# magenta/mt3

Measured on AMD Instinct MI355X. Metric: audio-seconds transcribed/sec (whole node), MT3-base, 1/2/4/8 MI355X, higher is better.
Workload: dtype f32; 1 GPU; BASELINE configs[2]: MT3 (model.gin) random-init, full encoder-decoder greedy decode, batch=256 synthetic 2.048 s segments per GPU, 1024 decode steps (no early exit), ids->tokens + host note decoding included; segments_per_gpu=256, segments_total=256, decode_steps=1024, decode_chains=1, decoding=greedy, parallelism=single GPU, graph_fallbacks=0, partition_fallbacks=0

## Files before the change

include/mt3_hip.h:

```cpp
#ifndef MT3_HIP_H_
#define MT3_HIP_H_

#include <stdint.h>

#ifdef __cplusplus
extern "C" {
#endif

typedef enum mt3_status {
  MT3_OK = 0,
  MT3_ERR_INVALID = -1,
  MT3_ERR_HIP = -2,
  MT3_ERR_CAPACITY = -3,
  MT3_ERR_MISSING = -4
} mt3_status;

const char* mt3_last_error(void);
int mt3_abi_version(void);

typedef struct mt3_frontend_config {
  int32_t sample_rate;
  int32_t hop_width;
  int32_t num_mel_bins;
  int32_t fft_size;
  float lo_hz;
  float hi_hz;
  int32_t table_dtype;
} mt3_frontend_config;

typedef struct mt3_frontend mt3_frontend;

int mt3_frontend_create(const mt3_frontend_config* cfg, mt3_frontend** out);
void mt3_frontend_destroy(mt3_frontend* fe);
int mt3_frontend_mel_matrix(const mt3_frontend* fe, float* h_out , int64_t* nnz);
int mt3_frontend_logmel(mt3_frontend* fe, const float* d_audio, int32_t n_segments,
                        int32_t frames_per_segment, const int32_t* h_n_frames ,
                        float* d_logmel, void* stream);
int mt3_frontend_logmel_dev(mt3_frontend* fe, const float* d_audio, int32_t n_segments,
                            int32_t frames_per_segment, const int32_t* d_n_frames ,
                            float* d_logmel, void* stream);

typedef struct mt3_resampler mt3_resampler;

int64_t mt3_resample_output_length(int64_t n_in, int32_t up, int32_t down);
int mt3_resampler_create(const double* h_taps , int64_t n_taps, int32_t up, int32_t down,
                         mt3_resampler** out);
void mt3_resampler_destroy(mt3_resampler* r);
int mt3_resampler_run(mt3_resampler* r, const float* d_in, int64_t n_in, float* d_out, int64_t out_capacity,
                      void* stream);

enum { MT3_PCM_U8 = 0, MT3_PCM_S16 = 1, MT3_PCM_S24 = 2, MT3_PCM_S32 = 3, MT3_PCM_F32 = 4, MT3_PCM_F64 = 5 };
#define MT3_PCM_MAX_CHANNELS 7

int mt3_pcm_decode(const void* d_pcm, int64_t n_frames, int32_t channels, int32_t format, float* d_out,
                   int64_t out_capacity, void* stream);
int mt3_resampler_run_pcm(mt3_resampler* r, const void* d_pcm, int64_t n_frames, int32_t channels, int32_t format,
                          float* d_out, int64_t out_capacity, void* stream);

typedef enum mt3_dtype { MT3_BF16 = 0, MT3_F32 = 1, MT3_FP8_E4M3 = 2  } mt3_dtype;

typedef struct mt3_engine_config {
  int32_t vocab_size;
  int32_t emb_dim;
  int32_t num_heads;
  int32_t head_dim;
  int32_t mlp_dim;
  int32_t num_encoder_layers;
  int32_t num_decoder_layers;
  int32_t input_depth;
  int32_t input_length;
  int32_t max_decode_len;
  int32_t max_batch;
  int32_t compute_dtype;
  int32_t decode_chains;
  int32_t kv_cache_dtype;
  int32_t dense_dtype;
  int32_t options;
} mt3_engine_config;

enum {
  MT3_OPT_SINGLE_RESIDUAL_STREAM = 1,
  MT3_OPT_ENCODER_SINGLE_RESIDUAL_STREAM = 4,
  MT3_OPT_SEPARATE_PROJECTIONS = 2,
  MT3_OPT_SEPARATE_QKV_PROJECTION = 8,
  MT3_OPT_NO_ROW_GROUPS = 16,
  MT3_OPT_ENCODER_F32_MFMA = 32,
  MT3_OPT_SPIN_WAITS = 64
};

typedef struct mt3_engine mt3_engine;

int mt3_engine_create(const mt3_engine_config* cfg, mt3_engine** out);
void mt3_engine_destroy(mt3_engine* e);
int mt3_engine_load_weight(mt3_engine* e, const char* name, const float* h_data,
                           const int64_t* shape, int32_t ndim);
int mt3_engine_finalize(mt3_engine* e);
int64_t mt3_engine_device_bytes(const mt3_engine* e);

int mt3_engine_encode(mt3_engine* e, const float* d_inputs, int32_t batch,
                      float* d_encoded_f32, void* stream);

enum {
  MT3_DECODE_NO_GRAPH = 1,
  MT3_DECODE_EARLY_EXIT = 2,
  MT3_DECODE_BEAM1 = 4,
  MT3_DECODE_SINGLE_STREAM = 8,
  MT3_DECODE_ASYNC = 16
};
#define MT3_DECODE_CHAINS(n) (((n) & 0xF) << 8)
int mt3_engine_decode(mt3_engine* e, int32_t batch, int32_t num_steps, int32_t flags,
                      int32_t* d_ids, float* d_first_logits, int32_t* h_steps_run, void* stream);
int mt3_engine_decode_wait(mt3_engine* e, int32_t* h_steps_run);

int mt3_engine_decode_beams(mt3_engine* e, int32_t batch, int32_t num_beams, int32_t num_steps, int32_t flags,
                            int32_t* d_ids, int32_t* d_all_ids, float* d_scores, int32_t* h_steps_run, void* stream);

typedef struct mt3_transcribe_stats {
  int32_t slots;
  int32_t groups;
  int32_t steps_run;
  int32_t polls;
  int32_t refills;
  int32_t starved_polls;
  int32_t encoder_chunks;
  int32_t compactions;
  int32_t used_graph;
  int32_t reserved[7];
} mt3_transcribe_stats;
int mt3_engine_transcribe(mt3_engine* e, const float* d_inputs, int32_t n_segments, int32_t num_steps, int32_t flags,
                          int32_t* d_ids, mt3_transcribe_stats* h_stats, void* stream);

int mt3_engine_decode_forced(mt3_engine* e, int32_t batch, int32_t num_steps, int32_t flags,
                             const int32_t* d_forced_ids, float* d_step_logits, int32_t* d_ids, void* stream);

int mt3_engine_score(mt3_engine* e, int32_t batch, int32_t length, const int32_t* d_targets,
                     const int32_t* d_decoder_inputs , const float* d_weights ,
                     float* d_sequence_scores, float* d_token_scores, float* d_logits, void* stream);

enum { MT3_STATUS_GRAPH_FALLBACKS = 0, MT3_STATUS_LAST_DECODE_USED_GRAPH = 1, MT3_STATUS_RESIDUAL_SPLIT = 2,
       MT3_STATUS_KV_FP8 = 3, MT3_STATUS_Q_FOLD = 4 ,
       MT3_STATUS_DENSE_FP8 = 5 ,
       MT3_STATUS_QKV_FOLD = 6 ,
       MT3_STATUS_LAST_DECODE_GROUPS = 7 ,
       MT3_STATUS_PARTITION_FALLBACKS = 8 ,
       MT3_STATUS_LAST_DECODE_COMPACTIONS = 9 ,
       MT3_STATUS_LAST_DECODE_FORKS = 10 ,
       MT3_STATUS_SCORE_CHUNKS = 11  };
int mt3_engine_status(const mt3_engine* e, int32_t what);

int mt3_ids_to_tokens(const int32_t* d_ids, int32_t batch, int32_t length, int32_t num_regular,
                      int32_t* d_tokens, void* stream);

enum { MT3_EPI_STORE = 0, MT3_EPI_RESID = 1, MT3_EPI_GEGLU = 2, MT3_EPI_POS = 3, MT3_EPI_F32 = 4, MT3_EPI_HEADS = 5 };
int mt3_op_gemm(int32_t dtype, const void* d_A, int32_t a_is_f32, int32_t norm, const void* d_Wt,
                void* d_out, int32_t M, int32_t N, int32_t K, int32_t epilogue, const float* d_aux,
                int32_t seq_len, int32_t small, void* stream);
int mt3_op_gemm_ex(int32_t dtype, const void* d_A, int32_t a_is_f32, int32_t norm, const void* d_Wt,
                   void* d_out, int32_t M, int32_t N, int32_t K, int32_t epilogue, const float* d_aux,
                   int32_t seq_len, int32_t small, const float* d_a_ss, void* d_out_ct, float* d_out_ss,
                   void* stream);
int mt3_op_residual_split(int32_t dtype, const float* d_x, void* d_x_ct, float* d_x_ss, int32_t rows, int32_t dim,
                          void* stream);
int mt3_op_encoder_attention(int32_t dtype, const void* d_qkv, void* d_out, int32_t B, int32_t T, int32_t H,
                             void* stream);
int mt3_op_decode_attention(int32_t dtype, const void* d_q, int32_t q_stride, void* d_kcache, void* d_vcache,
                            int32_t cap, const void* d_new_k, const void* d_new_v, int32_t kv_stride,
                            const int32_t* d_step, int32_t n_keys, void* d_out, int32_t B, int32_t H, void* stream);
int mt3_op_decode_attention_fp8(const void* d_q, int32_t q_stride, void* d_kcache, void* d_vcache, void* d_kv_scale,
                                int32_t cap, const void* d_new_k, const void* d_new_v, int32_t kv_stride,
                                const int32_t* d_step, int32_t n_keys, void* d_out, int32_t B, int32_t H,
                                void* stream);
int mt3_op_kv_quantize_fp8(const void* d_src, void* d_dst, void* d_scales, int32_t rows, void* stream);

int mt3_host_mx8_quantize(const float* h_w, int64_t rows, int64_t K, uint8_t* h_q, uint8_t* h_sc);
int mt3_op_mx8_quantize(const void* d_in, int32_t in_is_f32, int32_t M, int32_t K, uint8_t* d_q, uint8_t* d_sc,
                        float* d_ss, void* stream);
int mt3_op_gemm_mx8(const uint8_t* d_A, const uint8_t* d_a_sc, const uint8_t* d_W, const uint8_t* d_w_sc, void* d_out,
                    int32_t M, int32_t N, int32_t K, int32_t epilogue, int32_t seq_len, const float* d_a_ss,
                    uint8_t* d_out_q, uint8_t* d_out_sc, float* d_out_ss, void* stream);

enum { MT3_EV_SHIFT = 0, MT3_EV_PITCH = 1, MT3_EV_VELOCITY = 2, MT3_EV_TIE = 3, MT3_EV_PROGRAM = 4, MT3_EV_DRUM = 5 };
enum { MT3_SPEC_ONSETS = 0, MT3_SPEC_NOTES = 1, MT3_SPEC_TIES = 2 };

typedef struct mt3_event_range { int32_t type, min_value, max_value; } mt3_event_range;
typedef struct mt3_codec {
  double steps_per_second;
  int32_t num_ranges;
  mt3_event_range ranges[8];
} mt3_codec;
typedef struct mt3_note {
  double start_time, end_time;
  int32_t pitch, velocity, program, is_drum, instrument, reserved;
} mt3_note;

int mt3_build_codec(int32_t steps_per_second, int32_t max_shift_seconds, int32_t num_velocity_bins,
                    mt3_codec* out);
int mt3_codec_num_classes(const mt3_codec* c);
int mt3_codec_decode_event(const mt3_codec* c, int32_t index, int32_t* type, int32_t* value);
int mt3_codec_encode_event(const mt3_codec* c, int32_t type, int32_t value, int32_t* index);
int mt3_notes_decode(const mt3_codec* c, int32_t spec, int32_t n_segments, const int32_t* h_tokens,
                     const int64_t* h_seg_offsets, const double* h_start_times,
                     const int32_t* h_has_max_time, const double* h_max_times,
                     mt3_note* h_notes, int64_t notes_capacity, int64_t* n_notes,
                     int64_t* invalid_events, int64_t* dropped_events, double* total_time);

#ifdef __cplusplus
}
#endif
#endif
```

mt3_amd/_lib.py:

```python
from __future__ import annotations

import ctypes as C
import os

HERE = os.path.dirname(os.path.abspath(__file__))
LIB_PATH = os.path.join(HERE, "libmt3hip.so")

MT3_OK, MT3_ERR_INVALID, MT3_ERR_HIP, MT3_ERR_CAPACITY, MT3_ERR_MISSING = 0, -1, -2, -3, -4
MT3_BF16, MT3_F32, MT3_FP8_E4M3 = 0, 1, 2
EPI_STORE, EPI_RESID, EPI_GEGLU, EPI_POS, EPI_F32, EPI_HEADS = range(6)
DECODE_NO_GRAPH, DECODE_EARLY_EXIT, DECODE_BEAM1, DECODE_SINGLE_STREAM, DECODE_ASYNC = 1, 2, 4, 8, 16
(OPT_SINGLE_RESIDUAL_STREAM, OPT_SEPARATE_PROJECTIONS, OPT_ENCODER_SINGLE_RESIDUAL_STREAM,
 OPT_SEPARATE_QKV_PROJECTION, OPT_NO_ROW_GROUPS) = 1, 2, 4, 8, 16
OPT_ENCODER_F32_MFMA = 32
OPT_SPIN_WAITS = 64
DEBUG_SKIP_SELF_ATTN, DEBUG_SKIP_CROSS_ATTN = 1, 2
(STATUS_GRAPH_FALLBACKS, STATUS_LAST_DECODE_USED_GRAPH, STATUS_RESIDUAL_SPLIT, STATUS_KV_FP8, STATUS_Q_FOLD,
 STATUS_DENSE_FP8, STATUS_QKV_FOLD, STATUS_LAST_DECODE_GROUPS, STATUS_PARTITION_FALLBACKS,
 STATUS_LAST_DECODE_COMPACTIONS, STATUS_LAST_DECODE_FORKS, STATUS_SCORE_CHUNKS) = range(12)
(MT3_PCM_U8, MT3_PCM_S16, MT3_PCM_S24, MT3_PCM_S32, MT3_PCM_F32, MT3_PCM_F64) = range(6)
PCM_MAX_CHANNELS = 7
MAX_BEAMS = 8
EV_SHIFT, EV_PITCH, EV_VELOCITY, EV_TIE, EV_PROGRAM, EV_DRUM = range(6)
EVENT_TYPE_NAMES = ("shift", "pitch", "velocity", "tie", "program", "drum")
SPEC_ONSETS, SPEC_NOTES, SPEC_TIES = range(3)


class Mt3Error(RuntimeError):
    def __init__(self, code, msg):
        super().__init__("libmt3hip error %d: %s" % (code, msg))
        self.code = code


class FrontendConfig(C.Structure):
    _fields_ = [("sample_rate", C.c_int32), ("hop_width", C.c_int32), ("num_mel_bins", C.c_int32),
                ("fft_size", C.c_int32), ("lo_hz", C.c_float), ("hi_hz", C.c_float), ("table_dtype", C.c_int32)]


class EngineConfig(C.Structure):
    _fields_ = [(n, C.c_int32) for n in (
        "vocab_size", "emb_dim", "num_heads", "head_dim", "mlp_dim", "num_encoder_layers",
        "num_decoder_layers", "input_depth", "input_length", "max_decode_len", "max_batch", "compute_dtype",
        "decode_chains", "kv_cache_dtype", "dense_dtype", "options")]


class TranscribeStats(C.Structure):
    _fields_ = [(n, C.c_int32) for n in ("slots", "groups", "steps_run", "polls", "refills", "starved_polls",
                                         "encoder_chunks", "compactions", "used_graph")] + [("reserved", C.c_int32 * 7)]


class EventRange(C.Structure):
    _fields_ = [("type", C.c_int32), ("min_value", C.c_int32), ("max_value", C.c_int32)]


class CodecDesc(C.Structure):
    _fields_ = [("steps_per_second", C.c_double), ("num_ranges", C.c_int32), ("ranges", EventRange * 8)]


class NoteStruct(C.Structure):
    _fields_ = [("start_time", C.c_double), ("end_time", C.c_double), ("pitch", C.c_int32),
                ("velocity", C.c_int32), ("program", C.c_int32), ("is_drum", C.c_int32),
                ("instrument", C.c_int32), ("reserved", C.c_int32)]


_P = C.c_void_p
SIGNATURES = {
    "mt3_last_error": (C.c_char_p, []),
    "mt3_abi_version": (C.c_int, []),
    "mt3_frontend_create": (C.c_int, [C.POINTER(FrontendConfig), C.POINTER(_P)]),
    "mt3_frontend_destroy": (None, [_P]),
    "mt3_frontend_mel_matrix": (C.c_int, [_P, _P, C.POINTER(C.c_int64)]),
    "mt3_frontend_logmel": (C.c_int, [_P, _P, C.c_int32, C.c_int32, _P, _P, _P]),
    "mt3_frontend_logmel_dev": (C.c_int, [_P, _P, C.c_int32, C.c_int32, _P, _P, _P]),
    "mt3_resample_output_length": (C.c_int64, [C.c_int64, C.c_int32, C.c_int32]),
    "mt3_resampler_create": (C.c_int, [_P, C.c_int64, C.c_int32, C.c_int32, C.POINTER(_P)]),
    "mt3_resampler_destroy": (None, [_P]),
    "mt3_resampler_run": (C.c_int, [_P, _P, C.c_int64, _P, C.c_int64, _P]),
    "mt3_pcm_decode": (C.c_int, [_P, C.c_int64, C.c_int32, C.c_int32, _P, C.c_int64, _P]),
    "mt3_resampler_run_pcm": (C.c_int, [_P, _P, C.c_int64, C.c_int32, C.c_int32, _P, C.c_int64, _P]),
    "mt3_engine_create": (C.c_int, [C.POINTER(EngineConfig), C.POINTER(_P)]),
    "mt3_engine_destroy": (None, [_P]),
    "mt3_engine_load_weight": (C.c_int, [_P, C.c_char_p, _P, C.POINTER(C.c_int64), C.c_int32]),
    "mt3_engine_finalize": (C.c_int, [_P]),
    "mt3_engine_device_bytes": (C.c_int64, [_P]),
    "mt3_engine_encode": (C.c_int, [_P, _P, C.c_int32, _P, _P]),
    "mt3_engine_decode": (C.c_int, [_P, C.c_int32, C.c_int32, C.c_int32, _P, _P, C.POINTER(C.c_int32), _P]),
    "mt3_engine_decode_wait": (C.c_int, [_P, C.POINTER(C.c_int32)]),
    "mt3_engine_decode_beams": (C.c_int, [_P, C.c_int32, C.c_int32, C.c_int32, C.c_int32, _P, _P, _P,
                                          C.POINTER(C.c_int32), _P]),
    "mt3_engine_transcribe": (C.c_int, [_P, _P, C.c_int32, C.c_int32, C.c_int32, _P, C.POINTER(TranscribeStats), _P]),
    "mt3_engine_decode_forced": (C.c_int, [_P, C.c_int32, C.c_int32, C.c_int32, _P, _P, _P, _P]),
    "mt3_engine_score": (C.c_int, [_P, C.c_int32, C.c_int32, _P, _P, _P, _P, _P, _P, _P]),
    "mt3_engine_status": (C.c_int, [_P, C.c_int32]),
    "mt3_debug_engine_decode": (C.c_int, [_P, C.c_int32, C.c_int32, C.c_int32, C.c_int32, _P, _P]),
    "mt3_debug_engine_transcribe": (C.c_int, [_P, _P, C.c_int32, C.c_int32, C.c_int32, C.c_int32, C.c_int32, C.c_int32, _P,
                                              C.POINTER(TranscribeStats), _P]),
    "mt3_debug_engine_set_score_chunk": (C.c_int, [_P, C.c_int32]),
    "mt3_debug_engine_poison_caches": (C.c_int, [_P, C.c_int32, C.c_int32, _P]),
    "mt3_debug_engine_set_eos_schedule": (C.c_int, [_P, _P, C.c_int32]),
    "mt3_ids_to_tokens": (C.c_int, [_P, C.c_int32, C.c_int32, C.c_int32, _P, _P]),
    "mt3_op_gemm": (C.c_int, [C.c_int32, _P, C.c_int32, C.c_int32, _P, _P, C.c_int32, C.c_int32, C.c_int32,
                              C.c_int32, _P, C.c_int32, C.c_int32, _P]),
    "mt3_op_gemm_ex": (C.c_int, [C.c_int32, _P, C.c_int32, C.c_int32, _P, _P, C.c_int32, C.c_int32, C.c_int32,
                                 C.c_int32, _P, C.c_int32, C.c_int32, _P, _P, _P, _P]),
    "mt3_op_residual_split": (C.c_int, [C.c_int32, _P, _P, _P, C.c_int32, C.c_int32, _P]),
    "mt3_op_encoder_attention": (C.c_int, [C.c_int32, _P, _P, C.c_int32, C.c_int32, C.c_int32, _P]),
    "mt3_op_decode_attention": (C.c_int, [C.c_int32, _P, C.c_int32, _P, _P, C.c_int32, _P, _P, C.c_int32, _P,
                                          C.c_int32, _P, C.c_int32, C.c_int32, _P]),
    "mt3_op_decode_attention_fp8": (C.c_int, [_P, C.c_int32, _P, _P, _P, C.c_int32, _P, _P, C.c_int32, _P, C.c_int32,
                                              _P, C.c_int32, C.c_int32, _P]),
    "mt3_op_kv_quantize_fp8": (C.c_int, [_P, _P, _P, C.c_int32, _P]),
    "mt3_host_mx8_quantize": (C.c_int, [_P, C.c_int64, C.c_int64, _P, _P]),
    "mt3_op_mx8_quantize": (C.c_int, [_P, C.c_int32, C.c_int32, C.c_int32, _P, _P, _P, _P]),
    "mt3_op_gemm_mx8": (C.c_int, [_P, _P, _P, _P, _P, C.c_int32, C.c_int32, C.c_int32, C.c_int32, C.c_int32, _P, _P, _P,
                                  _P, _P]),
    "mt3_build_codec": (C.c_int, [C.c_int32, C.c_int32, C.c_int32, C.POINTER(CodecDesc)]),
    "mt3_codec_num_classes": (C.c_int, [C.POINTER(CodecDesc)]),
    "mt3_codec_decode_event": (C.c_int, [C.POINTER(CodecDesc), C.c_int32, C.POINTER(C.c_int32), C.POINTER(C.c_int32)]),
    "mt3_codec_encode_event": (C.c_int, [C.POINTER(CodecDesc), C.c_int32, C.c_int32, C.POINTER(C.c_int32)]),
    "mt3_notes_decode": (C.c_int, [C.POINTER(CodecDesc), C.c_int32, C.c_int32, _P, _P, _P, _P, _P, _P, C.c_int64,
                                   C.POINTER(C.c_int64), C.POINTER(C.c_int64), C.POINTER(C.c_int64),
                                   C.POINTER(C.c_double)]),
}

_lib = None


def load():
    global _lib
    if _lib is not None:
        return _lib
    if not os.path.exists(LIB_PATH):
        raise Mt3Error(MT3_ERR_MISSING,
                       "%s not found: build it with `python -m mt3_amd.build` "
                       "(hipcc --offload-arch=gfx950); there is no CPU fallback" % LIB_PATH)
    try:
        import torch
    except Exception:
        pass
    lib = C.CDLL(LIB_PATH)
    for name, (res, args) in SIGNATURES.items():
        fn = getattr(lib, name)
        fn.restype = res
        fn.argtypes = args
    _lib = lib
    return lib


def check(rc: int):
    if rc != MT3_OK:
        raise Mt3Error(rc, (load().mt3_last_error() or b"").decode("utf-8", "replace"))
    return rc
```

mt3_amd/csrc/engine.hip:

```cpp
#include <hip/hip_runtime.h>

#include <atomic>
#include <chrono>
#include <cmath>
#include <condition_variable>
#include <cstdlib>
#include <cstring>
#include <functional>
#include <map>
#include <mutex>
#include <new>
#include <string>
#include <thread>
#include <vector>

#include "common.h"
#include "feed.h"
#include "kernels.h"

namespace mt3k {
int launch_encoder_attention_x6(const void* qkv, void* out, int B, int T, int H, hipStream_t s);
}
#include "mx8.h"
#include "mt3_hip.h"
#include "mt3_hip_debug.h"

namespace {

constexpr int kMaxPos = 2048;
constexpr int kMaxChains = 8;
constexpr int kForksPinned = 15;

uint16_t f32_to_bf16_bits(float f) {
  uint32_t u;
  std::memcpy(&u, &f, 4);
  if ((u & 0x7fffffffu) > 0x7f800000u) return static_cast<uint16_t>((u >> 16) | 0x40);
  u += 0x7fffu + ((u >> 16) & 1u);
  return static_cast<uint16_t>(u >> 16);
}

struct HostWeight {
  std::vector<float> data;
  std::vector<int64_t> shape;
};

struct LayerDev {
  void* wqkv = nullptr;
  void* wo = nullptr;
  void* wq_x = nullptr;
  void* wkv_x = nullptr;
  void* wo_x = nullptr;
  void* wqkv_ext = nullptr;
  void* wo_ext = nullptr;
  void* w_fold = nullptr;
  void* wi = nullptr;
  void* wo_mlp = nullptr;
  void* self_k = nullptr;
  void* self_v = nullptr;
  void* cross_kv = nullptr;
  uint8_t *wqkv_q = nullptr, *wqkv_sc = nullptr, *wo_q = nullptr, *wo_sc = nullptr, *wi_q = nullptr, *wi_sc = nullptr,
          *wo_mlp_q = nullptr, *wo_mlp_sc = nullptr, *wkv_x_q = nullptr, *wkv_x_sc = nullptr;
  void *wqkv_p[3] = {}, *wo_p[3] = {}, *wi_p[3] = {}, *wo_mlp_p[3] = {}, *wkv_x_p[3] = {};
  void *wq_x_p[3] = {}, *wo_x_p[3] = {};
  float2* self_scale = nullptr;
  float2* cross_scale = nullptr;
};

constexpr int kVarBeam = 4, kVarForced = 8, kVarRetire = 16, kVarEos = 32, kVarStream = 64, kNumVariants = 128;
constexpr int kVarBeside = 128;
constexpr int kVarBeams = 256, kVarBeamsShift = 9;
constexpr int kMaxGroups = 4;
constexpr int kStageChunks = mt3feed::kStageChunks, kStageChunkCap = 64, kStageMinBatch = 8;
constexpr int kStreamPollSteps = 4;
constexpr int kThrottleWindow = 16;

struct Worker {
  std::thread th;
  std::mutex mu;
  std::condition_variable cv;
  std::function<void()> job;
  bool has_job = false, quit = false;
};

struct GroupGraph {
  int variant, batch, row0, rows, slot, max_len;
  hipGraph_t graph;
  hipGraphExec_t exec;
};

struct PendingDecode {
  bool active = false;
  int posted = 0;
  int groups = 1;
  bool beam1 = false;
  bool used_graph[kMaxGroups] = {};
  int batch = 0;
  int32_t* d_ids = nullptr;
  hipStream_t s = nullptr;
  int beams = 0;
  int num_steps = 0;
  int32_t* d_all_ids = nullptr;
  float* d_scores = nullptr;
  int rcs[kMaxGroups] = {};
  int ran[kMaxGroups] = {};
  std::string errs[kMaxGroups];
};

}

struct mt3_engine {
  mt3_engine_config cfg{};
  std::map<std::string, HostWeight> raw;
  std::vector<void*> allocs;
  int64_t device_bytes = 0;
  bool finalized = false;
  int esize = 2;
  int kv_esize = 2;
  bool kv_fp8 = false;
  void* cross_stage = nullptr;
  bool dense_fp8 = false;
  uint8_t *x_q = nullptr, *x_sc = nullptr;
  uint8_t *attn_q = nullptr, *attn_sc = nullptr;
  uint8_t *h_q = nullptr, *h_sc = nullptr;
  uint8_t *enc_q = nullptr, *enc_sc = nullptr;

  void* enc_in = nullptr;
  void* enc_in_p[3] = {};
  bool x6 = false;
  float* enc_norm = nullptr;
  float* embedding = nullptr;
  void* logits_w = nullptr;
  float* pos_table = nullptr;
  std::vector<LayerDev> enc, dec;

  float* x = nullptr;
  void* x_ct = nullptr;
  float* x_ss = nullptr;
  bool x_split = false;
  void* qkv = nullptr;
  void* attn = nullptr;
  void* hbuf = nullptr;
  void* enc_out = nullptr;
  float* y = nullptr;
  void* y_ct = nullptr;
  float* y_ss = nullptr;
  bool y_split = false;
  float* qf = nullptr;
  bool q_fold = false;
  bool qkv_fold = false;
  float* qkvf = nullptr;
  float* ew0 = nullptr;
  float* pw0 = nullptr;
  void* y_ct_alt = nullptr;
  float* y_alt = nullptr;
  void* qkv_d = nullptr;
  void* attn_d = nullptr;
  void* q_d = nullptr;
  void* h_d = nullptr;
  float* logits = nullptr;
  int* ids = nullptr;
  int* cur_tok = nullptr;
  int* done = nullptr;
  int* step = nullptr;
  int* n_done = nullptr;
  int* h_pinned = nullptr;
  int* forced = nullptr;
  std::atomic<int> graph_fallbacks{0};
  int last_used_graph = 0;
  int* slot_row = nullptr;
  int* eos_at = nullptr;
  int eos_cap = 0;
  bool eos_on = false;
  int* slot_seg = nullptr;
  int* cs_seg = nullptr;
  int* refill_plan = nullptr;
  int stream_max_len = 0;
  int stage_cap = 0;
  std::vector<void*> stage_kv;
  std::vector<float2*> stage_scale;
  float* cs_y = nullptr;
  void* cs_y_ct = nullptr;
  float* cs_y_ss = nullptr;
  float* cs_qkvf = nullptr;
  int* cs_int = nullptr;
  float* cs_beam = nullptr;
  int* cs_perm = nullptr;
  int compactions = 0;
  std::atomic<int> compactions_now{0};
  std::vector<GroupGraph> group_graphs;
  std::mutex graph_mu;
  Worker* workers[kMaxGroups] = {};
  int device = 0;
  PendingDecode pending;
  float* beam_f = nullptr;
  int* beam_len = nullptr;
  int* beam_len_row = nullptr;
  float* beam_cfg = nullptr;
  float* bk_live = nullptr;
  float* bk_fin_score = nullptr;
  int* bk_fin_step = nullptr;
  int* bk_fin_beam = nullptr;
  int* bk_fork_src = nullptr;
  int* bk_forks = nullptr;
  int* bk_par = nullptr;
  int* bk_tok = nullptr;

  hipStream_t part_stream[kMaxGroups] = {};
  hipEvent_t part_begin = nullptr;
  hipEvent_t wait_ev[kMaxGroups + 1][4] = {};
  bool spin_waits = false;
  int part_failed = 0;
  int last_groups = 1;

  int cur_batch = 0;
  hipStream_t cap_stream[8] = {};
  hipEvent_t cap_event[8] = {};
  hipGraphExec_t graph_exec[kNumVariants][9] = {};
  hipGraph_t graph[kNumVariants][9] = {};
  int graph_batch = 0;

  int score_cap = 0;
  int score_Lp = 0;
  int score_chunk_req = 0;
  int score_chunks = 0;
  bool score_planes = false;
  void* logits_p[3] = {};
  float* sc_y = nullptr;
  void* sc_y_ct = nullptr;
  float* sc_y_ss = nullptr;
  void* sc_qkv = nullptr;
  void* sc_attn = nullptr;
  void* sc_q = nullptr;
  void* sc_h = nullptr;
  float* sc_logits = nullptr;
  int* sc_tgt = nullptr;
  float* sc_tok = nullptr;

  int HD() const { return cfg.num_heads * cfg.head_dim; }
};

namespace {

float brevity_penalty(int length) { return static_cast<float>(std::pow((5.0 + length) / 6.0, 0.6)); }

int dmalloc(mt3_engine* e, void** p, size_t bytes) {
  MT3_HIP_CHECK(hipMalloc(p, bytes));
  e->allocs.push_back(*p);
  e->device_bytes += static_cast<int64_t>(bytes);
  return MT3_OK;
}

int upload_ct(mt3_engine* e, const std::vector<float>& h, void** d) {
  int rc = dmalloc(e, d, h.size() * e->esize);
  if (rc) return rc;
  if (e->cfg.compute_dtype == MT3_BF16) {
    std::vector<uint16_t> t(h.size());
    for (size_t i = 0; i < h.size(); ++i) t[i] = f32_to_bf16_bits(h[i]);
    MT3_HIP_CHECK(hipMemcpy(*d, t.data(), t.size() * 2, hipMemcpyHostToDevice));
  } else {
    MT3_HIP_CHECK(hipMemcpy(*d, h.data(), h.size() * 4, hipMemcpyHostToDevice));
  }
  return MT3_OK;
}

int upload_mx8(mt3_engine* e, const std::vector<float>& h, int64_t rows, int64_t K, uint8_t** q, uint8_t** sc) {
  if (!e->dense_fp8) return MT3_OK;
  std::vector<uint8_t> hq(h.size()), hs(static_cast<size_t>(rows) * (K / 32));
  int rc = mt3_host_mx8_quantize(h.data(), rows, K, hq.data(), hs.data());
  if (rc) return rc;
  if ((rc = dmalloc(e, reinterpret_cast<void**>(q), hq.size()))) return rc;
  if ((rc = dmalloc(e, reinterpret_cast<void**>(sc), hs.size()))) return rc;
  MT3_HIP_CHECK(hipMemcpy(*q, hq.data(), hq.size(), hipMemcpyHostToDevice));
  MT3_HIP_CHECK(hipMemcpy(*sc, hs.data(), hs.size(), hipMemcpyHostToDevice));
  return MT3_OK;
}

int upload_planes(mt3_engine* e, const std::vector<float>& h, void* (&p)[3]) {
  if (!e->x6) return MT3_OK;
  std::vector<uint16_t> pl[3];
  for (auto& v : pl) v.resize(h.size());
  for (size_t i = 0; i < h.size(); ++i) {
    auto val = [](uint16_t b) {
      const uint32_t u = static_cast<uint32_t>(b) << 16;
      float f;
      std::memcpy(&f, &u, 4);
      return f;
    };
    const uint16_t hi = f32_to_bf16_bits(h[i]);
    const float r1 = h[i] - val(hi);
    const uint16_t mi = f32_to_bf16_bits(r1);
    const float r2 = r1 - val(mi);
    pl[0][i] = hi;
    pl[1][i] = mi;
    pl[2][i] = f32_to_bf16_bits(r2);
  }
  for (int k = 0; k < 3; ++k) {
    int rc = dmalloc(e, &p[k], h.size() * 2);
    if (rc) return rc;
    MT3_HIP_CHECK(hipMemcpy(p[k], pl[k].data(), h.size() * 2, hipMemcpyHostToDevice));
  }
  return MT3_OK;
}

int upload_f32(mt3_engine* e, const std::vector<float>& h, float** d) {
  int rc = dmalloc(e, reinterpret_cast<void**>(d), h.size() * 4);
  if (rc) return rc;
  MT3_HIP_CHECK(hipMemcpy(*d, h.data(), h.size() * 4, hipMemcpyHostToDevice));
  return MT3_OK;
}

const HostWeight* find(mt3_engine* e, const std::string& name, int64_t d0, int64_t d1) {
  auto it = e->raw.find(name);
  if (it == e->raw.end()) {
    mt3::fail(MT3_ERR_MISSING, "weight not loaded: " + name);
    return nullptr;
  }
  const HostWeight& w = it->second;
  const bool ok = (d1 < 0) ? (w.shape.size() == 1 && w.shape[0] == d0)
                           : (w.shape.size() == 2 && w.shape[0] == d0 && w.shape[1] == d1);
  if (!ok) {
    mt3::fail(MT3_ERR_INVALID, "weight has the wrong shape: " + name);
    return nullptr;
  }
  return &w;
}

void put_transposed(std::vector<float>& dst, int in, int row0, const HostWeight& w, const float* scale) {
  const int out = static_cast<int>(w.shape[1]);
  for (int k = 0; k < in; ++k) {
    const float s = scale ? scale[k] : 1.f;
    const float* src = w.data.data() + static_cast<size_t>(k) * out;
    for (int n = 0; n < out; ++n) dst[static_cast<size_t>(row0 + n) * in + k] = src[n] * s;
  }
}

int build_attention(mt3_engine* e, const std::string& prefix, const float* scale, bool cross, LayerDev* L,
                    bool encoder = false) {
  const int emb = e->cfg.emb_dim, hd = e->HD();
  const HostWeight *q = find(e, prefix + "/query/kernel", emb, hd), *k = find(e, prefix + "/key/kernel", emb, hd),
                   *v = find(e, prefix + "/value/kernel", emb, hd), *o = find(e, prefix + "/out/kernel", hd, emb);
  if (!q || !k || !v || !o) return MT3_ERR_MISSING;
  int rc;
  std::vector<float> ot(static_cast<size_t>(emb) * hd);
  put_transposed(ot, hd, 0, *o, nullptr);
  if (!cross) {
    std::vector<float> t(static_cast<size_t>(3) * hd * emb);
    put_transposed(t, emb, 0, *q, scale);
    put_transposed(t, emb, hd, *k, scale);
    put_transposed(t, emb, 2 * hd, *v, scale);
    if ((rc = upload_ct(e, t, &L->wqkv))) return rc;
    if ((rc = upload_ct(e, ot, &L->wo))) return rc;
    if (encoder) {
      if ((rc = upload_planes(e, t, L->wqkv_p))) return rc;
      if ((rc = upload_planes(e, ot, L->wo_p))) return rc;
      if ((rc = upload_mx8(e, t, 3 * hd, emb, &L->wqkv_q, &L->wqkv_sc))) return rc;
      if ((rc = upload_mx8(e, ot, emb, hd, &L->wo_q, &L->wo_sc))) return rc;
    }
  } else {
    std::vector<float> tq(static_cast<size_t>(hd) * emb), tkv(static_cast<size_t>(2) * hd * emb);
    put_transposed(tq, emb, 0, *q, scale);
    put_transposed(tkv, emb, 0, *k, nullptr);
    put_transposed(tkv, emb, hd, *v, nullptr);
    if ((rc = upload_ct(e, tq, &L->wq_x))) return rc;
    if ((rc = upload_ct(e, tkv, &L->wkv_x))) return rc;
    if ((rc = upload_planes(e, tkv, L->wkv_x_p))) return rc;
    if ((rc = upload_mx8(e, tkv, 2 * hd, emb, &L->wkv_x_q, &L->wkv_x_sc))) return rc;
    if ((rc = upload_ct(e, ot, &L->wo_x))) return rc;
  }
  return MT3_OK;
}

int build_q_fold(mt3_engine* e, const std::string& P, const float* s1, const float* s2, LayerDev* L) {
  const int emb = e->cfg.emb_dim, hd = e->HD();
  const std::string S = P + "/self_attention", X = P + "/encoder_decoder_attention";
  const HostWeight *q = find(e, S + "/query/kernel", emb, hd), *k = find(e, S + "/key/kernel", emb, hd),
                   *v = find(e, S + "/value/kernel", emb, hd), *o = find(e, S + "/out/kernel", hd, emb),
                   *qx = find(e, X + "/query/kernel", emb, hd);
  if (!q || !k || !v || !o || !qx) return MT3_ERR_MISSING;
  std::vector<float> t(static_cast<size_t>(4) * hd * emb);
  put_transposed(t, emb, 0, *q, s1);
  put_transposed(t, emb, hd, *k, s1);
  put_transposed(t, emb, 2 * hd, *v, s1);
  put_transposed(t, emb, 3 * hd, *qx, s2);
  int rc;
  if ((rc = upload_ct(e, t, &L->wqkv_ext))) return rc;
  std::vector<float> u(static_cast<size_t>(emb + hd) * hd);
  put_transposed(u, hd, 0, *o, nullptr);
  std::vector<double> acc(hd);
  for (int kk = 0; kk < hd; ++kk) {
    std::fill(acc.begin(), acc.end(), 0.0);
    const float* orow = o->data.data() + static_cast<size_t>(kk) * emb;
    for (int ee = 0; ee < emb; ++ee) {
      const double w = static_cast<double>(orow[ee]) * s2[ee];
      const float* qrow = qx->data.data() + static_cast<size_t>(ee) * hd;
      for (int n = 0; n < hd; ++n) acc[n] += w * qrow[n];
    }
    for (int n = 0; n < hd; ++n) u[static_cast<size_t>(emb + n) * hd + kk] = static_cast<float>(acc[n]);
  }
  return upload_ct(e, u, &L->wo_ext);
}

mt3k::GemmArgs gemm_args(const void* A, const void* Wt, void* out, int M, int N, int K, int ldo);
const float* scale_of(mt3_engine* e, const std::string& name);

int build_qkv_fold(mt3_engine* e) {
  const mt3_engine_config& c = e->cfg;
  const int emb = c.emb_dim, hd = e->HD(), mlp = c.mlp_dim, n4 = 4 * hd, nl = c.num_decoder_layers;
  auto wext_t = [&](int l, std::vector<float>* t) -> int {
    const std::string P = "decoder/layers_" + std::to_string(l);
    const float* s1 = scale_of(e, P + "/pre_self_attention_layer_norm/scale");
    const float* s2 = scale_of(e, P + "/pre_cross_attention_layer_norm/scale");
    const HostWeight *q = find(e, P + "/self_attention/query/kernel", emb, hd),
                     *k = find(e, P + "/self_attention/key/kernel", emb, hd),
                     *v = find(e, P + "/self_attention/value/kernel", emb, hd),
                     *qx = find(e, P + "/encoder_decoder_attention/query/kernel", emb, hd);
    if (!s1 || !s2 || !q || !k || !v || !qx) return MT3_ERR_MISSING;
    t->assign(static_cast<size_t>(n4) * emb, 0.f);
    put_transposed(*t, emb, 0, *q, s1);
    put_transposed(*t, emb, hd, *k, s1);
    put_transposed(*t, emb, 2 * hd, *v, s1);
    put_transposed(*t, emb, 3 * hd, *qx, s2);
    return MT3_OK;
  };
  float *d_wext = nullptr, *d_wo = nullptr, *d_prod = nullptr;
  auto cleanup = [&]() {
    if (d_wext) (void)hipFree(d_wext);
    if (d_wo) (void)hipFree(d_wo);
    if (d_prod) (void)hipFree(d_prod);
  };
  int rc = MT3_OK;
  const int n_max = n4 > c.vocab_size ? n4 : c.vocab_size;
  hipError_t he = hipMalloc(reinterpret_cast<void**>(&d_wext), static_cast<size_t>(n_max) * emb * 4);
  if (he == hipSuccess) he = hipMalloc(reinterpret_cast<void**>(&d_wo), static_cast<size_t>(mlp) * emb * 4);
  if (he == hipSuccess) he = hipMalloc(reinterpret_cast<void**>(&d_prod), static_cast<size_t>(n_max) * mlp * 4);
  std::vector<float> wt, prod, w;
  for (int l = 0; l < nl && he == hipSuccess && rc == MT3_OK; ++l) {
    const bool last = l + 1 == nl;
    const int nx = last ? c.vocab_size : n4;
    const HostWeight* wo = find(e, "decoder/layers_" + std::to_string(l) + "/mlp/wo/kernel", mlp, emb);
    if (!wo) rc = MT3_ERR_MISSING;
    if (rc == MT3_OK && !last) rc = wext_t(l + 1, &wt);
    if (rc == MT3_OK && last) {
      const float* sn = scale_of(e, "decoder/decoder_norm/scale");
      const HostWeight* wl = find(e, "decoder/logits_dense/kernel", emb, c.vocab_size);
      if (!sn || !wl) rc = MT3_ERR_MISSING;
      else {
        wt.assign(static_cast<size_t>(nx) * emb, 0.f);
        put_transposed(wt, emb, 0, *wl, sn);
      }
    }
    if (rc != MT3_OK) break;
    he = hipMemcpy(d_wext, wt.data(), wt.size() * 4, hipMemcpyHostToDevice);
    if (he == hipSuccess) he = hipMemcpy(d_wo, wo->data.data(), wo->data.size() * 4, hipMemcpyHostToDevice);
    if (he != hipSuccess) break;
    mt3k::GemmArgs g = gemm_args(d_wext, d_wo, d_prod, nx, mlp, emb, mlp);
    rc = mt3k::launch_gemm(MT3_F32, g, false, 0, MT3_EPI_F32, false, nullptr);
    if (rc != MT3_OK) break;
    prod.resize(static_cast<size_t>(nx) * mlp);
    he = hipMemcpy(prod.data(), d_prod, prod.size() * 4, hipMemcpyDeviceToHost);
    if (he != hipSuccess) break;
    const size_t K = static_cast<size_t>(mlp) + emb;
    w.assign((static_cast<size_t>(emb) + nx) * K, 0.f);
    for (int k = 0; k < mlp; ++k)
      for (int n = 0; n < emb; ++n) w[static_cast<size_t>(n) * K + k] = wo->data[static_cast<size_t>(k) * emb + n];
    for (int n = 0; n < nx; ++n) {
      float* row = w.data() + (static_cast<size_t>(emb) + n) * K;
      std::memcpy(row, prod.data() + static_cast<size_t>(n) * mlp, static_cast<size_t>(mlp) * 4);
      std::memcpy(row + mlp, wt.data() + static_cast<size_t>(n) * emb, static_cast<size_t>(emb) * 4);
    }
    rc = upload_ct(e, w, &e->dec[l].w_fold);
  }
  if (he == hipSuccess && rc == MT3_OK) rc = wext_t(0, &wt);
  if (he == hipSuccess && rc == MT3_OK) {
    he = hipMemcpy(d_wext, wt.data(), wt.size() * 4, hipMemcpyHostToDevice);
    if (he == hipSuccess) rc = dmalloc(e, reinterpret_cast<void**>(&e->ew0), static_cast<size_t>(c.vocab_size) * n4 * 4);
    if (he == hipSuccess && rc == MT3_OK)
      rc = dmalloc(e, reinterpret_cast<void**>(&e->pw0), static_cast<size_t>(kMaxPos) * n4 * 4);
    if (he == hipSuccess && rc == MT3_OK)
      rc = mt3k::launch_gemm(MT3_F32, gemm_args(e->embedding, d_wext, e->ew0, c.vocab_size, n4, emb, n4), false, 0,
                             MT3_EPI_F32, false, nullptr);
    if (he == hipSuccess && rc == MT3_OK)
      rc = mt3k::launch_gemm(MT3_F32, gemm_args(e->pos_table, d_wext, e->pw0, kMaxPos, n4, emb, n4), false, 0,
                             MT3_EPI_F32, false, nullptr);
    if (he == hipSuccess && rc == MT3_OK) he = hipDeviceSynchronize();
  }
  cleanup();
  if (rc != MT3_OK) return rc;
  if (he != hipSuccess) return mt3::fail(MT3_ERR_HIP, std::string("qkv-fold tables: ") + hipGetErrorString(he));
  return MT3_OK;
}

int build_mlp(mt3_engine* e, const std::string& prefix, const float* scale, LayerDev* L, bool encoder = false) {
  const int emb = e->cfg.emb_dim, mlp = e->cfg.mlp_dim;
  const HostWeight *w0 = find(e, prefix + "/wi_0/kernel", emb, mlp), *w1 = find(e, prefix + "/wi_1/kernel", emb, mlp),
                   *wo = find(e, prefix + "/wo/kernel", mlp, emb);
  if (!w0 || !w1 || !wo) return MT3_ERR_MISSING;
  std::vector<float> t(static_cast<size_t>(2) * mlp * emb);
  for (int k = 0; k < emb; ++k) {
    const float s = scale[k];
    for (int n = 0; n < mlp; ++n) {
      const int q = n >> 4, r = n & 15;
      t[static_cast<size_t>(32 * q + r) * emb + k] = w0->data[static_cast<size_t>(k) * mlp + n] * s;
      t[static_cast<size_t>(32 * q + 16 + r) * emb + k] = w1->data[static_cast<size_t>(k) * mlp + n] * s;
    }
  }
  std::vector<float> ot(static_cast<size_t>(emb) * mlp);
  put_transposed(ot, mlp, 0, *wo, nullptr);
  int rc;
  if ((rc = upload_ct(e, t, &L->wi))) return rc;
  if (encoder) {
    if ((rc = upload_planes(e, t, L->wi_p))) return rc;
    if ((rc = upload_planes(e, ot, L->wo_mlp_p))) return rc;
    if ((rc = upload_mx8(e, t, 2 * mlp, emb, &L->wi_q, &L->wi_sc))) return rc;
    if ((rc = upload_mx8(e, ot, emb, mlp, &L->wo_mlp_q, &L->wo_mlp_sc))) return rc;
  }
  return upload_ct(e, ot, &L->wo_mlp);
}

const float* scale_of(mt3_engine* e, const std::string& name) {
  const HostWeight* w = find(e, name, e->cfg.emb_dim, -1);
  return w ? w->data.data() : nullptr;
}

mt3k::GemmArgs gemm_args(const void* A, const void* Wt, void* out, int M, int N, int K, int ldo) {
  mt3k::GemmArgs g{};
  g.A = A;
  g.Wt = Wt;
  g.out = out;
  g.M = M;
  g.N = N;
  g.K = K;
  g.lda = K;
  g.ldo = ldo;
  return g;
}

#define MT3_TRY(expr)           \
  do {                          \
    int _rc = (expr);           \
    if (_rc != MT3_OK) return _rc; \
  } while (0)

inline int chain_num_ops(const mt3_engine* e) { return 8 * e->cfg.num_decoder_layers + 2; }
inline bool chain_op_is_heavy(const mt3_engine* e, int op) {
  return op < 8 * e->cfg.num_decoder_layers && ((op & 7) == 1 || (op & 7) == 4);
}

mt3k::BeamKArgs beam_args(mt3_engine* e, int row0, int rows, int k) {
  mt3k::BeamKArgs b{};
  b.vocab = e->cfg.vocab_size;
  b.k = k;
  b.elems = rows / k;
  b.live = e->bk_live + row0;
  b.fin_score = e->bk_fin_score + row0;
  b.fin_step = e->bk_fin_step + row0;
  b.fin_beam = e->bk_fin_beam + row0;
  b.hist_par = e->bk_par + row0;
  b.hist_tok = e->bk_tok + row0;
  b.hist_stride = e->cfg.max_batch;
  b.slot_row = e->slot_row + row0;
  b.fork_src = e->bk_fork_src + row0;
  b.fork_count = e->bk_forks;
  b.done = e->done + row0;
  b.step = e->step + row0;
  b.cur_tok = e->cur_tok + row0;
  b.bp = e->beam_cfg;
  return b;
}

int enqueue_chain_op(mt3_engine* e, int row0, int rows, int B_total, int skip, int op, hipStream_t s, int done_slot = 0) {
  const mt3_engine_config& c = e->cfg;
  const int dt = c.compute_dtype, emb = c.emb_dim, hd = e->HD(), H = c.num_heads, T = c.input_length;
  const int Lmax = c.max_decode_len;
  const size_t es = e->esize, kes = e->kv_esize;
  const bool small = true;
  const int nl = c.num_decoder_layers;
  const bool split = e->y_split, fold = e->qkv_fold;
  const bool retire = (skip & kVarRetire) != 0;
  const size_t crow0 = retire ? 0 : static_cast<size_t>(row0);
  const int layer = op < 8 * nl ? (op >> 3) : nl - 1;
  const int cur = fold ? (layer & 1) : 0;
  const bool f32 = dt == MT3_F32;
  auto y_buf = [&](int which) -> float* {
    return ((fold && f32 && which) ? e->y_alt : e->y) + static_cast<size_t>(row0) * emb;
  };
  auto yct_buf = [&](int which) -> char* {
    if (!split) return nullptr;
    if (f32) return reinterpret_cast<char*>(y_buf(which));
    return static_cast<char*>((fold && which) ? e->y_ct_alt : e->y_ct) + static_cast<size_t>(row0) * emb * es;
  };
  float* y = y_buf(cur);
  char* y_ct = yct_buf(cur);
  char* y_copy = split && !f32 ? y_ct : nullptr;
  float* y_ss = split ? e->y_ss + static_cast<size_t>(row0) * (emb / 16) : nullptr;
  auto normed = [&](const void* Wt, void* out, int N, int ldo) {
    mt3k::GemmArgs g = gemm_args(split ? static_cast<const void*>(y_ct) : static_cast<const void*>(y), Wt, out, rows, N,
                                 emb, ldo);
    g.a_ss = y_ss;
    return g;
  };
  const int beside = ((skip & kVarBeside) || (!retire && rows < B_total)) ? 1 : 0;
  auto resid = [&](const void* A, const void* Wt, int K) {
    mt3k::GemmArgs g = gemm_args(A, Wt, y, rows, emb, K, emb);
    g.out_ct = y_copy;
    g.out_ss = y_ss;
    g.concurrent = beside;
    return g;
  };
  const int nrm = split ? 2 : 1;
  char* qkv_d = static_cast<char*>(e->qkv_d) + static_cast<size_t>(row0) * 3 * hd * es;
  char* attn_d = static_cast<char*>(e->attn_d) + static_cast<size_t>(row0) * hd * es;
  char* q_d = static_cast<char*>(e->q_d) + static_cast<size_t>(row0) * hd * es;
  char* h_d = static_cast<char*>(e->h_d) + static_cast<size_t>(row0) * c.mlp_dim * es;
  float* qkvf = fold ? e->qkvf + static_cast<size_t>(row0) * 4 * hd : nullptr;
  float* logits = e->logits + static_cast<size_t>(row0) * c.vocab_size;
  int* step = e->step + row0;
  if (op == 8 * nl) {
    if (fold) return MT3_OK;
    return mt3k::launch_gemm(dt, normed(e->logits_w, logits, c.vocab_size, c.vocab_size), !split, nrm, MT3_EPI_F32,
                             small, s);
  }
  if (op == 8 * nl + 1 && (skip & kVarBeams)) {
    mt3k::BeamKArgs b = beam_args(e, row0, rows, (skip >> kVarBeamsShift) & 15);
    b.logits = logits;
    b.n_done = e->n_done + done_slot;
    b.table = e->embedding;
    b.pos_table = e->pos_table;
    b.max_pos = kMaxPos;
    b.y_next = y_buf(0);
    b.y_ct = split && !f32 ? yct_buf(0) : nullptr;
    b.y_ss = y_ss;
    b.dim = emb;
    const mt3k::RowProj rp{e->ew0, e->pw0, qkvf, 4 * hd};
    const mt3k::LogitScale ls{fold ? y_ss : nullptr, emb / 16, emb};
    MT3_TRY(mt3k::launch_beam_step(b, rp, ls, s));
    mt3k::BeamReorderArgs r{};
    r.n_layers = nl;
    r.H = H;
    r.cap = Lmax;
    r.kv_esize = static_cast<int>(kes);
    r.slots = rows;
    for (int l = 0; l < nl; ++l) {
      r.k[l] = static_cast<char*>(e->dec[l].self_k);
      r.v[l] = static_cast<char*>(e->dec[l].self_v);
      r.scale[l] = e->kv_fp8 ? e->dec[l].self_scale : nullptr;
    }
    r.fork_src = e->bk_fork_src + row0;
    r.slot_row = e->slot_row + row0;
    r.step = step;
    r.done = e->done + row0;
    return mt3k::launch_beam_reorder(r, s);
  }
  if (op == 8 * nl + 1) {
    const mt3k::BeamState beam{e->beam_f + row0, e->beam_len + row0, e->beam_cfg, c.max_batch, e->beam_len_row + crow0};
    const mt3k::RowProj rp{e->ew0, e->pw0, qkvf, 4 * hd};
    const mt3k::LogitScale ls{fold ? y_ss : nullptr, emb / 16, emb};
    const bool streaming = (skip & kVarStream) != 0;
    const mt3k::StepRetire rt{retire ? 1 : 0, retire ? e->slot_row + row0 : nullptr,
                              (skip & kVarEos) ? e->eos_at + crow0 : nullptr, streaming ? e->slot_seg + row0 : nullptr,
                              streaming ? e->stream_max_len : 0};
    return mt3k::launch_argmax_step(logits, c.vocab_size, e->ids + crow0 * Lmax, Lmax,
                                    e->cur_tok + row0, e->done + row0, e->n_done + done_slot, step, e->embedding, e->pos_table,
                                    kMaxPos, y_buf(0), split && !f32 ? yct_buf(0) : nullptr, y_ss, emb, rows,
                                    (skip & kVarBeam) ? &beam : nullptr,
                                    (skip & kVarForced) ? e->forced + static_cast<size_t>(row0) * Lmax : nullptr, Lmax, rp, ls,
                                    rt, s);
  }
  LayerDev& L = e->dec[op >> 3];
  switch (op & 7) {
    case 0:
      if (fold) return MT3_OK;
      if (e->q_fold) {
        mt3k::GemmArgs g = normed(L.wqkv_ext, qkv_d, 4 * hd, 3 * hd);
        g.out2 = e->qf + static_cast<size_t>(row0) * hd;
        g.n_split = 3 * hd;
        return mt3k::launch_gemm(dt, g, false, 2, mt3k::kEpiStoreQ, small, s);
      }
      return mt3k::launch_gemm(dt, normed(L.wqkv, qkv_d, 3 * hd, 3 * hd), !split, nrm, MT3_EPI_STORE, small, s);
    case 1: {
      if (skip & 1) return MT3_OK;
      mt3k::DecAttnArgs a{};
      a.q = qkv_d;
      a.q_stride = 3 * hd;
      a.kcache = static_cast<char*>(L.self_k) + crow0 * H * Lmax * 64 * kes;
      a.vcache = static_cast<char*>(L.self_v) + crow0 * H * Lmax * 64 * kes;
      a.kv_scale = e->kv_fp8 ? L.self_scale + crow0 * H * Lmax : nullptr;
      if (retire) {
        a.done = e->done + row0;
        a.cache_row = e->slot_row + row0;
      }
      a.cap = Lmax;
      a.new_k = qkv_d + static_cast<size_t>(hd) * es;
      a.new_v = qkv_d + static_cast<size_t>(2 * hd) * es;
      a.kv_stride = 3 * hd;
      if (fold) {
        a.q = nullptr;
        a.q_f32 = qkvf;
        a.q_stride = a.kv_stride = 4 * hd;
        a.new_k = qkvf + hd;
        a.new_v = qkvf + 2 * hd;
        a.q_ss = y_ss;
        a.q_ss_n = emb / 16;
      }
      a.step = step;
      a.out = attn_d;
      a.B = rows;
      a.H = H;
      return mt3k::launch_decode_attention(dt, a, s);
    }
    case 2:
      if (e->q_fold) {
        mt3k::GemmArgs g = resid(attn_d, L.wo_ext, hd);
        g.N = emb + hd;
        g.out2 = fold ? qkvf + 3 * hd : e->qf + static_cast<size_t>(row0) * hd;
        g.ld2 = fold ? 4 * hd : 0;
        g.n_split = emb;
        return mt3k::launch_gemm(dt, g, false, 0, mt3k::kEpiResidQ, small, s);
      }
      return mt3k::launch_gemm(dt, resid(attn_d, L.wo, hd), false, 0, MT3_EPI_RESID, small, s);
    case 3:
      if (e->q_fold) return MT3_OK;
      return mt3k::launch_gemm(dt, normed(L.wq_x, q_d, hd, hd), !split, nrm, MT3_EPI_STORE, small, s);
    case 4: {
      if (skip & 2) return MT3_OK;
      mt3k::DecAttnArgs x{};
      x.q = q_d;
      x.q_stride = hd;
      if (e->q_fold) {
        x.q_f32 = fold ? qkvf + 3 * hd : e->qf + static_cast<size_t>(row0) * hd;
        if (fold) x.q_stride = 4 * hd;
        x.q_ss = y_ss;
        x.q_ss_n = emb / 16;
      }
      x.kcache = static_cast<char*>(L.cross_kv) + crow0 * H * T * 64 * kes;
      x.vcache = static_cast<char*>(L.cross_kv) + (static_cast<size_t>(B_total) + crow0) * H * T * 64 * kes;
      x.kv_scale = e->kv_fp8 ? L.cross_scale + crow0 * H * T : nullptr;
      if (retire) {
        x.done = e->done + row0;
        x.cache_row = e->slot_row + row0;
      }
      x.cap = T;
      x.n_keys = T;
      x.out = attn_d;
      x.B = rows;
      x.H = H;
      return mt3k::launch_decode_attention(dt, x, s);
    }
    case 5:
      return mt3k::launch_gemm(dt, resid(attn_d, L.wo_x, hd), false, 0, MT3_EPI_RESID, small, s);
    case 6: {
      mt3k::GemmArgs g = normed(L.wi, h_d, 2 * c.mlp_dim, c.mlp_dim);
      g.concurrent = beside;
      return mt3k::launch_gemm(dt, g, !split, nrm, MT3_EPI_GEGLU, small, s);
    }
    default:
      if (fold) {
        const bool last = (op >> 3) + 1 == nl;
        const int nx = last ? c.vocab_size : 4 * hd;
        mt3k::GemmArgs g = gemm_args(h_d, L.w_fold, y_buf(cur ^ 1), rows, emb + nx, c.mlp_dim + emb, emb);
        g.lda = c.mlp_dim;
        g.resid_src = y;
        g.out_ct = f32 ? nullptr : yct_buf(cur ^ 1);
        g.out_ss = y_ss;
        g.out2 = last ? logits : qkvf;
        g.ld2 = nx;
        g.n_split = emb;
        g.A2 = y_ct;
        g.lda2 = emb;
        g.k_split = c.mlp_dim;
        g.concurrent = beside;
        return mt3k::launch_gemm(dt, g, false, 0, mt3k::kEpiResidS, small, s);
      }
      return mt3k::launch_gemm(dt, resid(h_d, L.wo_mlp, c.mlp_dim), false, 0, MT3_EPI_RESID, small, s);
  }
}

int enqueue_chain_step(mt3_engine* e, int row0, int rows, int chain, int B_total, int skip, hipStream_t s,
                       int done_slot = 0) {
  (void)chain;
  for (int op = 0, n = chain_num_ops(e); op < n; ++op)
    MT3_TRY(enqueue_chain_op(e, row0, rows, B_total, skip, op, s, done_slot));
  return MT3_OK;
}

inline void chain_rows(int B, int n, int k, int* row0, int* rows) {
  const int q = B / n, r = B % n;
  *row0 = k * q + (k < r ? k : r);
  *rows = q + (k < r ? 1 : 0);
}

int chains_for(const mt3_engine* e, int B, int requested) {
  int n = requested > 0 ? requested : (e->cfg.decode_chains > 0 ? e->cfg.decode_chains : 1);
  if (n > kMaxChains) n = kMaxChains;
  while (n > 1 && B / n < 16) --n;
  return n;
}

int enqueue_decode_step(mt3_engine* e, int B, int skip, int n, hipStream_t s) {
  for (int k = 0; k < n; ++k) {
    int row0, rows;
    chain_rows(B, n, k, &row0, &rows);
    MT3_TRY(enqueue_chain_step(e, row0, rows, k, B, skip, s));
  }
  return MT3_OK;
}

void drop_graph(mt3_engine* e) {
  for (int v = 0; v < kNumVariants; ++v)
    for (int n = 0; n < 9; ++n) {
      if (e->graph_exec[v][n]) (void)hipGraphExecDestroy(e->graph_exec[v][n]);
      if (e->graph[v][n]) (void)hipGraphDestroy(e->graph[v][n]);
      e->graph_exec[v][n] = nullptr;
      e->graph[v][n] = nullptr;
    }
  e->graph_batch = 0;
}

int ensure_graph(mt3_engine* e, int B, int skip, int n) {
  if (e->graph_batch != B) drop_graph(e);
  if (e->graph_exec[skip][n]) return MT3_OK;
  for (int k = 0; k < n; ++k) {
    if (!e->cap_stream[k]) MT3_HIP_CHECK(hipStreamCreateWithFlags(&e->cap_stream[k], hipStreamNonBlocking));
    if (!e->cap_event[k]) MT3_HIP_CHECK(hipEventCreateWithFlags(&e->cap_event[k], hipEventDisableTiming));
  }
  hipStream_t origin = e->cap_stream[0];
  MT3_HIP_CHECK(hipStreamBeginCapture(origin, hipStreamCaptureModeThreadLocal));
  int rc = MT3_OK;
  hipError_t he = hipSuccess;
  if (n > 1) he = hipEventRecord(e->cap_event[0], origin);
  for (int k = 1; k < n && he == hipSuccess; ++k) he = hipStreamWaitEvent(e->cap_stream[k], e->cap_event[0], 0);
  for (int k = 0; k < n && he == hipSuccess && rc == MT3_OK; ++k) {
    int row0, rows;
    chain_rows(B, n, k, &row0, &rows);
    rc = enqueue_chain_step(e, row0, rows, k, B, skip, e->cap_stream[k]);
  }
  for (int k = 1; k < n && he == hipSuccess && rc == MT3_OK; ++k) {
    he = hipEventRecord(e->cap_event[k], e->cap_stream[k]);
    if (he == hipSuccess) he = hipStreamWaitEvent(origin, e->cap_event[k], 0);
  }
  hipGraph_t g = nullptr;
  const hipError_t end = hipStreamEndCapture(origin, &g);
  if (rc != MT3_OK || he != hipSuccess || end != hipSuccess) {
    if (g) (void)hipGraphDestroy(g);
    if (rc != MT3_OK) return rc;
    return mt3::fail(MT3_ERR_HIP, std::string("decode graph capture: ") +
                                      hipGetErrorString(he != hipSuccess ? he : end));
  }
  e->graph[skip][n] = g;
  MT3_HIP_CHECK(hipGraphInstantiate(&e->graph_exec[skip][n], g, nullptr, nullptr, 0));
  e->graph_batch = B;
  return MT3_OK;
}

}

extern "C" {

static void workers_stop(mt3_engine* e);
static void drop_group_graphs(mt3_engine* e);

int mt3_engine_create(const mt3_engine_config* cfg, mt3_engine** out) {
  if (!cfg || !out) return mt3::fail(MT3_ERR_INVALID, "mt3_engine_create: null argument");
  if (cfg->head_dim != 64) return mt3::fail(MT3_ERR_INVALID, "mt3_engine_create: head_dim must be 64");
  if (cfg->compute_dtype != MT3_BF16 && cfg->compute_dtype != MT3_F32)
    return mt3::fail(MT3_ERR_INVALID, "mt3_engine_create: compute_dtype must be MT3_BF16 or MT3_F32");
  if (cfg->input_length != 256 && cfg->input_length != 512)
    return mt3::fail(MT3_ERR_INVALID, "mt3_engine_create: input_length must be 256 (mt3) or 512 (ismir2021)");
  if (cfg->emb_dim % 128 || cfg->mlp_dim % 128 || cfg->vocab_size % 128 || cfg->input_depth % 64 ||
      (cfg->num_heads * 64) % 128)
    return mt3::fail(MT3_ERR_INVALID, "mt3_engine_create: emb/mlp/vocab/heads*64 must be multiples of 128");
  if (cfg->decode_chains < 0 || cfg->decode_chains > kMaxChains)
    return mt3::fail(MT3_ERR_INVALID, "mt3_engine_create: decode_chains must be in [0, 8]");
  if (cfg->max_batch <= 0 || cfg->max_decode_len <= 0 || cfg->max_decode_len > kMaxPos ||
      cfg->num_encoder_layers <= 0 || cfg->num_decoder_layers <= 0)
    return mt3::fail(MT3_ERR_INVALID, "mt3_engine_create: bad sizes");
  if (cfg->kv_cache_dtype != 0 && cfg->kv_cache_dtype != MT3_FP8_E4M3)
    return mt3::fail(MT3_ERR_INVALID, "mt3_engine_create: kv_cache_dtype must be 0 (= compute dtype) or MT3_FP8_E4M3");
  if (cfg->kv_cache_dtype == MT3_FP8_E4M3 && cfg->compute_dtype != MT3_BF16)
    return mt3::fail(MT3_ERR_INVALID, "mt3_engine_create: the fp8 K/V caches go with compute_dtype MT3_BF16");
  if (cfg->dense_dtype != 0 && cfg->dense_dtype != MT3_FP8_E4M3)
    return mt3::fail(MT3_ERR_INVALID, "mt3_engine_create: dense_dtype must be 0 (= compute dtype) or MT3_FP8_E4M3");
  if (cfg->dense_dtype == MT3_FP8_E4M3 && (cfg->compute_dtype != MT3_BF16 || cfg->emb_dim > 1024))
    return mt3::fail(MT3_ERR_INVALID, "mt3_engine_create: the MXFP8 dense path goes with compute_dtype MT3_BF16 and emb_dim <= 1024");
  if (cfg->options & ~(MT3_OPT_SINGLE_RESIDUAL_STREAM | MT3_OPT_SEPARATE_PROJECTIONS | MT3_OPT_ENCODER_SINGLE_RESIDUAL_STREAM |
                       MT3_OPT_SEPARATE_QKV_PROJECTION | MT3_OPT_NO_ROW_GROUPS | MT3_OPT_ENCODER_F32_MFMA | MT3_OPT_SPIN_WAITS))
    return mt3::fail(MT3_ERR_INVALID, "mt3_engine_create: unknown bit in options");
  mt3_engine* e = new (std::nothrow) mt3_engine();
  if (!e) return mt3::fail(MT3_ERR_INVALID, "out of host memory");
  e->cfg = *cfg;
  if (hipGetDevice(&e->device) != hipSuccess) {
    (void)hipGetLastError();
    e->device = 0;
  }
  e->dense_fp8 = cfg->dense_dtype == MT3_FP8_E4M3;
  e->x6 = cfg->compute_dtype == MT3_F32 && !(cfg->options & MT3_OPT_ENCODER_F32_MFMA);
  e->spin_waits = (cfg->options & MT3_OPT_SPIN_WAITS) != 0;
  e->esize = cfg->compute_dtype == MT3_BF16 ? 2 : 4;
  e->kv_fp8 = cfg->kv_cache_dtype == MT3_FP8_E4M3;
  e->kv_esize = e->kv_fp8 ? 1 : e->esize;
  *out = e;
  return MT3_OK;
}

void mt3_engine_destroy(mt3_engine* e) {
  if (!e) return;
  workers_stop(e);
  drop_graph(e);
  drop_group_graphs(e);
  for (int k = 0; k < kMaxChains; ++k) {
    if (e->cap_stream[k]) (void)hipStreamDestroy(e->cap_stream[k]);
    if (e->cap_event[k]) (void)hipEventDestroy(e->cap_event[k]);
  }
  for (int g = 0; g < kMaxGroups; ++g)
    if (e->part_stream[g]) (void)hipStreamDestroy(e->part_stream[g]);
  if (e->part_begin) (void)hipEventDestroy(e->part_begin);
  for (auto& pair : e->wait_ev)
    for (hipEvent_t ev : pair)
      if (ev) (void)hipEventDestroy(ev);
  if (e->h_pinned) (void)hipHostFree(e->h_pinned);
  for (void* p : e->allocs) (void)hipFree(p);
  delete e;
}

int mt3_engine_load_weight(mt3_engine* e, const char* name, const float* h_data, const int64_t* shape, int32_t ndim) {
  if (!e || !name || !h_data || !shape || ndim < 1 || ndim > 2)
    return mt3::fail(MT3_ERR_INVALID, "mt3_engine_load_weight: bad arguments");
  if (e->finalized) return mt3::fail(MT3_ERR_INVALID, "mt3_engine_load_weight: engine already finalized");
  HostWeight w;
  size_t n = 1;
  for (int i = 0; i < ndim; ++i) {
    if (shape[i] <= 0) return mt3::fail(MT3_ERR_INVALID, "mt3_engine_load_weight: bad shape");
    w.shape.push_back(shape[i]);
    n *= static_cast<size_t>(shape[i]);
  }
  w.data.assign(h_data, h_data + n);
  e->raw[name] = std::move(w);
  return MT3_OK;
}

int64_t mt3_engine_device_bytes(const mt3_engine* e) { return e ? e->device_bytes : 0; }

int mt3_engine_finalize(mt3_engine* e) {
  if (!e) return mt3::fail(MT3_ERR_INVALID, "mt3_engine_finalize: null engine");
  if (e->finalized) return MT3_OK;
  const mt3_engine_config& c = e->cfg;
  const int emb = c.emb_dim, hd = e->HD(), Bm = c.max_batch, T = c.input_length, L = c.max_decode_len;
  int rc;

  {
    const HostWeight* w = find(e, "encoder/continuous_inputs_projection/kernel", c.input_depth, emb);
    if (!w) return MT3_ERR_MISSING;
    std::vector<float> t(static_cast<size_t>(emb) * c.input_depth);
    put_transposed(t, c.input_depth, 0, *w, nullptr);
    if ((rc = upload_ct(e, t, &e->enc_in))) return rc;
    if ((rc = upload_planes(e, t, e->enc_in_p))) return rc;
  }
  e->enc.resize(c.num_encoder_layers);
  for (int l = 0; l < c.num_encoder_layers; ++l) {
    const std::string P = "encoder/layers_" + std::to_string(l);
    const float* s1 = scale_of(e, P + "/pre_attention_layer_norm/scale");
    const float* s2 = scale_of(e, P + "/pre_mlp_layer_norm/scale");
    if (!s1 || !s2) return MT3_ERR_MISSING;
    if ((rc = build_attention(e, P + "/attention", s1, false, &e->enc[l], true))) return rc;
    if ((rc = build_mlp(e, P + "/mlp", s2, &e->enc[l], true))) return rc;
  }
  {
    const HostWeight* w = find(e, "encoder/encoder_norm/scale", emb, -1);
    if (!w) return MT3_ERR_MISSING;
    if ((rc = upload_f32(e, w->data, &e->enc_norm))) return rc;
  }
  {
    const HostWeight* w = find(e, "decoder/token_embedder/embedding", c.vocab_size, emb);
    if (!w) return MT3_ERR_MISSING;
    if ((rc = upload_f32(e, w->data, &e->embedding))) return rc;
  }
  e->dec.resize(c.num_decoder_layers);
  const bool single_stream = (c.options & MT3_OPT_SINGLE_RESIDUAL_STREAM) != 0;
  const bool q_fold = emb % 64 == 0 && (emb <= 512 || (emb == 768 && c.compute_dtype == MT3_BF16)) && !single_stream &&
                      !(c.options & MT3_OPT_SEPARATE_PROJECTIONS);
  e->q_fold = q_fold;
  for (int l = 0; l < c.num_decoder_layers; ++l) {
    const std::string P = "decoder/layers_" + std::to_string(l);
    const float* s1 = scale_of(e, P + "/pre_self_attention_layer_norm/scale");
    const float* s2 = scale_of(e, P + "/pre_cross_attention_layer_norm/scale");
    const float* s3 = scale_of(e, P + "/pre_mlp_layer_norm/scale");
    if (!s1 || !s2 || !s3) return MT3_ERR_MISSING;
    if ((rc = build_attention(e, P + "/self_attention", s1, false, &e->dec[l]))) return rc;
    if ((rc = build_attention(e, P + "/encoder_decoder_attention", s2, true, &e->dec[l]))) return rc;
    if (q_fold && (rc = build_q_fold(e, P, s1, s2, &e->dec[l]))) return rc;
    if ((rc = build_mlp(e, P + "/mlp", s3, &e->dec[l]))) return rc;
    const size_t kvb = static_cast<size_t>(Bm) * c.num_heads * L * 64 * e->kv_esize;
    if ((rc = dmalloc(e, &e->dec[l].self_k, kvb))) return rc;
    if ((rc = dmalloc(e, &e->dec[l].self_v, kvb))) return rc;
    MT3_HIP_CHECK(hipMemset(e->dec[l].self_k, 0, kvb));
    MT3_HIP_CHECK(hipMemset(e->dec[l].self_v, 0, kvb));
    if ((rc = dmalloc(e, &e->dec[l].cross_kv, static_cast<size_t>(2) * Bm * c.num_heads * T * 64 * e->kv_esize)))
      return rc;
    if (e->kv_fp8) {
      if ((rc = dmalloc(e, reinterpret_cast<void**>(&e->dec[l].self_scale),
                        static_cast<size_t>(Bm) * c.num_heads * L * sizeof(float2))))
        return rc;
      MT3_HIP_CHECK(hipMemset(e->dec[l].self_scale, 0, static_cast<size_t>(Bm) * c.num_heads * L * sizeof(float2)));
      if ((rc = dmalloc(e, reinterpret_cast<void**>(&e->dec[l].cross_scale),
                        static_cast<size_t>(Bm) * c.num_heads * T * sizeof(float2))))
        return rc;
    }
  }
  if (e->kv_fp8 && (rc = dmalloc(e, &e->cross_stage, static_cast<size_t>(2) * Bm * c.num_heads * T * 64 * 2))) return rc;
  {
    const float* sn = scale_of(e, "decoder/decoder_norm/scale");
    const HostWeight* w = find(e, "decoder/logits_dense/kernel", emb, c.vocab_size);
    if (!sn || !w) return MT3_ERR_MISSING;
    std::vector<float> t(static_cast<size_t>(c.vocab_size) * emb);
    put_transposed(t, emb, 0, *w, sn);
    if ((rc = upload_ct(e, t, &e->logits_w))) return rc;
  }
  {
    std::vector<float> pe(static_cast<size_t>(kMaxPos) * emb);
    const int half = emb / 2;
    const double sf = -std::log(10000.0) / (half - 1);
    for (int p = 0; p < kMaxPos; ++p)
      for (int j = 0; j < half; ++j) {
        const double div = std::exp(j * sf);
        pe[static_cast<size_t>(p) * emb + j] = static_cast<float>(std::sin(p * div));
        pe[static_cast<size_t>(p) * emb + half + j] = static_cast<float>(std::cos(p * div));
      }
    if ((rc = upload_f32(e, pe, &e->pos_table))) return rc;
  }
  e->qkv_fold = q_fold && !(c.options & MT3_OPT_SEPARATE_QKV_PROJECTION) && emb % 512 == 0 && c.mlp_dim % 512 == 0;
  if (e->qkv_fold && (rc = build_qkv_fold(e))) return rc;
  const size_t M = static_cast<size_t>(Bm) * T;
  if ((rc = dmalloc(e, reinterpret_cast<void**>(&e->x), M * emb * 4))) return rc;
  e->x_split = c.compute_dtype == MT3_BF16 && emb % 64 == 0 && emb <= 1024 &&
               !(c.options & MT3_OPT_ENCODER_SINGLE_RESIDUAL_STREAM) && !e->dense_fp8;
  if (e->x_split) {
    if ((rc = dmalloc(e, &e->x_ct, M * emb * 2))) return rc;
    if ((rc = dmalloc(e, reinterpret_cast<void**>(&e->x_ss), M * (emb / 16) * 4))) return rc;
  }
  if (e->dense_fp8) {
    if (!e->x_ss && (rc = dmalloc(e, reinterpret_cast<void**>(&e->x_ss), M * (emb / 16) * 4))) return rc;
    if ((rc = dmalloc(e, reinterpret_cast<void**>(&e->x_q), M * emb))) return rc;
    if ((rc = dmalloc(e, reinterpret_cast<void**>(&e->x_sc), M * (emb / 32)))) return rc;
    if ((rc = dmalloc(e, reinterpret_cast<void**>(&e->attn_q), M * hd))) return rc;
    if ((rc = dmalloc(e, reinterpret_cast<void**>(&e->attn_sc), M * (hd / 32)))) return rc;
    if ((rc = dmalloc(e, reinterpret_cast<void**>(&e->h_q), M * c.mlp_dim))) return rc;
    if ((rc = dmalloc(e, reinterpret_cast<void**>(&e->h_sc), M * (c.mlp_dim / 32)))) return rc;
    if ((rc = dmalloc(e, reinterpret_cast<void**>(&e->enc_q), M * emb))) return rc;
    if ((rc = dmalloc(e, reinterpret_cast<void**>(&e->enc_sc), M * (emb / 32)))) return rc;
  }
  if ((rc = dmalloc(e, &e->qkv, M * 3 * hd * e->esize))) return rc;
  if ((rc = dmalloc(e, &e->attn, M * hd * e->esize))) return rc;
  if ((rc = dmalloc(e, &e->hbuf, M * c.mlp_dim * e->esize))) return rc;
  if ((rc = dmalloc(e, &e->enc_out, M * emb * e->esize))) return rc;
  if ((rc = dmalloc(e, reinterpret_cast<void**>(&e->y), static_cast<size_t>(Bm) * emb * 4))) return rc;
  e->y_split = emb % 64 == 0 && (emb <= 512 || (emb == 768 && c.compute_dtype == MT3_BF16)) && !single_stream;
  if (e->y_split) {
    if (c.compute_dtype == MT3_BF16) {
      if ((rc = dmalloc(e, &e->y_ct, static_cast<size_t>(Bm) * emb * 2))) return rc;
    } else {
      e->y_ct = e->y;
    }
    if ((rc = dmalloc(e, reinterpret_cast<void**>(&e->y_ss), static_cast<size_t>(Bm) * (emb / 16) * 4))) return rc;
  }
  if (e->q_fold && !e->y_split) e->q_fold = false;
  if (!e->q_fold) e->qkv_fold = false;
  if (e->q_fold && (rc = dmalloc(e, reinterpret_cast<void**>(&e->qf), static_cast<size_t>(Bm) * hd * 4))) return rc;
  if (e->qkv_fold) {
    if ((rc = dmalloc(e, reinterpret_cast<void**>(&e->qkvf), static_cast<size_t>(Bm) * 4 * hd * 4))) return rc;
    if (c.compute_dtype == MT3_BF16) {
      if ((rc = dmalloc(e, &e->y_ct_alt, static_cast<size_t>(Bm) * emb * 2))) return rc;
    } else if ((rc = dmalloc(e, reinterpret_cast<void**>(&e->y_alt), static_cast<size_t>(Bm) * emb * 4))) {
      return rc;
    }
  }
  if ((rc = dmalloc(e, &e->qkv_d, static_cast<size_t>(Bm) * 3 * hd * e->esize))) return rc;
  if ((rc = dmalloc(e, &e->attn_d, static_cast<size_t>(Bm) * hd * e->esize))) return rc;
  if ((rc = dmalloc(e, &e->q_d, static_cast<size_t>(Bm) * hd * e->esize))) return rc;
  if ((rc = dmalloc(e, &e->h_d, static_cast<size_t>(Bm) * c.mlp_dim * e->esize))) return rc;
  if ((rc = dmalloc(e, reinterpret_cast<void**>(&e->logits), static_cast<size_t>(Bm) * c.vocab_size * 4))) return rc;
  if ((rc = dmalloc(e, reinterpret_cast<void**>(&e->ids), static_cast<size_t>(Bm) * L * 4))) return rc;
  if ((rc = dmalloc(e, reinterpret_cast<void**>(&e->cur_tok), static_cast<size_t>(Bm) * 4))) return rc;
  if ((rc = dmalloc(e, reinterpret_cast<void**>(&e->done), static_cast<size_t>(Bm) * 4))) return rc;
  if ((rc = dmalloc(e, reinterpret_cast<void**>(&e->step), static_cast<size_t>(Bm) * 4))) return rc;
  if ((rc = dmalloc(e, reinterpret_cast<void**>(&e->n_done), 4 * kMaxChains))) return rc;
  if ((rc = dmalloc(e, reinterpret_cast<void**>(&e->forced), static_cast<size_t>(Bm) * L * 4))) return rc;
  if ((rc = dmalloc(e, reinterpret_cast<void**>(&e->slot_row), static_cast<size_t>(Bm) * 4))) return rc;
  if ((rc = dmalloc(e, reinterpret_cast<void**>(&e->eos_at), static_cast<size_t>(Bm) * 4))) return rc;
  e->eos_cap = Bm;
  if ((rc = dmalloc(e, reinterpret_cast<void**>(&e->slot_seg), static_cast<size_t>(Bm) * 4))) return rc;
  if ((rc = dmalloc(e, reinterpret_cast<void**>(&e->cs_seg), static_cast<size_t>(Bm) * 4))) return rc;
  if ((rc = dmalloc(e, reinterpret_cast<void**>(&e->refill_plan), (static_cast<size_t>(Bm) + kMaxChains) * 4))) return rc;
  if ((rc = dmalloc(e, reinterpret_cast<void**>(&e->cs_y), static_cast<size_t>(Bm) * emb * 4))) return rc;
  if (e->y_split && c.compute_dtype == MT3_BF16 && (rc = dmalloc(e, &e->cs_y_ct, static_cast<size_t>(Bm) * emb * 2))) return rc;
  if (e->y_split && (rc = dmalloc(e, reinterpret_cast<void**>(&e->cs_y_ss), static_cast<size_t>(Bm) * (emb / 16) * 4))) return rc;
  if (e->qkv_fold && (rc = dmalloc(e, reinterpret_cast<void**>(&e->cs_qkvf), static_cast<size_t>(Bm) * 4 * hd * 4))) return rc;
  if ((rc = dmalloc(e, reinterpret_cast<void**>(&e->cs_int), static_cast<size_t>(Bm) * 4 * 4))) return rc;
  if ((rc = dmalloc(e, reinterpret_cast<void**>(&e->cs_beam), static_cast<size_t>(Bm) * 2 * 4))) return rc;
  if ((rc = dmalloc(e, reinterpret_cast<void**>(&e->cs_perm), (static_cast<size_t>(Bm) + kMaxChains) * 4))) return rc;
  if ((rc = dmalloc(e, reinterpret_cast<void**>(&e->beam_f), static_cast<size_t>(2) * Bm * 4))) return rc;
  if ((rc = dmalloc(e, reinterpret_cast<void**>(&e->beam_len), static_cast<size_t>(Bm) * 4))) return rc;
  if ((rc = dmalloc(e, reinterpret_cast<void**>(&e->beam_len_row), static_cast<size_t>(Bm) * 4))) return rc;
  {
    std::vector<float> bp(static_cast<size_t>(L) + 3, 0.f);
    for (int n = 0; n <= L + 1; ++n) bp[1 + n] = brevity_penalty(n);
    if ((rc = dmalloc(e, reinterpret_cast<void**>(&e->beam_cfg), bp.size() * 4))) return rc;
    MT3_HIP_CHECK(hipMemcpy(e->beam_cfg, bp.data(), bp.size() * 4, hipMemcpyHostToDevice));
  }
  MT3_HIP_CHECK(hipHostMalloc(reinterpret_cast<void**>(&e->h_pinned), 64, hipHostMallocDefault));
  e->h_pinned[kForksPinned] = 0;
  e->raw.clear();
  e->finalized = true;
  return MT3_OK;
}

struct CrossDst {
  void* const* kv = nullptr;
  float2* const* scale = nullptr;
};

static int encode_impl(mt3_engine* e, const float* d_inputs, int32_t batch, float* d_encoded_f32, const CrossDst& dst,
                       hipStream_t s) {
  const mt3_engine_config& c = e->cfg;
  auto ckv = [&](int l) -> void* { return dst.kv ? dst.kv[l] : e->dec[l].cross_kv; };
  auto csc = [&](int l) -> float2* { return dst.scale ? dst.scale[l] : e->dec[l].cross_scale; };
  const int dt = c.compute_dtype, emb = c.emb_dim, hd = e->HD(), T = c.input_length;
  const int M = batch * T;
  const bool small = M < 2048;
  const int widest = std::max(std::max(c.input_depth, emb), std::max(hd, c.mlp_dim));
  const bool x6_fits = static_cast<size_t>(M) * widest * 4 < (1ull << 32);
  if (e->x6 && x6_fits) {
    auto x6 = [&](const void* A, void* (&W)[3], void* out, int N, int K, int ldo, bool norm, int epi, int seq) {
      mt3k::GemmArgs g = gemm_args(A, W[0], out, M, N, K, ldo);
      g.aux = e->pos_table;
      g.seq_len = seq;
      return mt3k::launch_gemm_x6(g, W[1], W[2], norm, epi, s);
    };
    MT3_TRY(x6(d_inputs, e->enc_in_p, e->x, emb, c.input_depth, emb, false, MT3_EPI_POS, T));
    for (int l = 0; l < c.num_encoder_layers; ++l) {
      LayerDev& L = e->enc[l];
      MT3_TRY(x6(e->x, L.wqkv_p, e->qkv, 3 * hd, emb, 3 * hd, true, MT3_EPI_STORE, 0));
      MT3_TRY(mt3k::launch_encoder_attention_x6(e->qkv, e->attn, batch, T, c.num_heads, s));
      MT3_TRY(x6(e->attn, L.wo_p, e->x, emb, hd, emb, false, MT3_EPI_RESID, 0));
      MT3_TRY(x6(e->x, L.wi_p, e->hbuf, 2 * c.mlp_dim, emb, c.mlp_dim, true, MT3_EPI_GEGLU, 0));
      MT3_TRY(x6(e->hbuf, L.wo_mlp_p, e->x, emb, c.mlp_dim, emb, false, MT3_EPI_RESID, 0));
    }
    MT3_TRY(mt3k::launch_rmsnorm(dt, e->x, e->enc_norm, e->enc_out, d_encoded_f32, M, emb, s));
    for (int l = 0; l < c.num_decoder_layers; ++l)
      MT3_TRY(x6(e->enc_out, e->dec[l].wkv_x_p, ckv(l), 2 * hd, emb, 2 * hd, false, MT3_EPI_HEADS, T));
    return MT3_OK;
  }
  {
    mt3k::GemmArgs g = gemm_args(d_inputs, e->enc_in, e->x, M, emb, c.input_depth, emb);
    g.aux = e->pos_table;
    g.seq_len = T;
    MT3_TRY(mt3k::launch_gemm(dt, g, true, false, MT3_EPI_POS, small, s));
  }
  if (e->dense_fp8) {
    auto mx = [&](const uint8_t* A, const uint8_t* a_sc, const uint8_t* W, const uint8_t* w_sc, int N, int K) {
      mt3k::Mx8Args g{};
      g.A = A;
      g.a_sc = a_sc;
      g.W = W;
      g.w_sc = w_sc;
      g.M = M;
      g.N = N;
      g.K = K;
      g.ldo = N;
      return g;
    };
    auto resid = [&](const uint8_t* A, const uint8_t* a_sc, const uint8_t* W, const uint8_t* w_sc, int K) {
      mt3k::Mx8Args g = mx(A, a_sc, W, w_sc, emb, K);
      g.out = e->x;
      g.out_q = e->x_q;
      g.out_sc = e->x_sc;
      g.out_ss = e->x_ss;
      return mt3k::launch_gemm_mx8(g, MT3_EPI_RESID, s);
    };
    MT3_TRY(mt3k::launch_mx8_quantize(e->x, true, M, emb, e->x_q, e->x_sc, e->x_ss, s));
    for (int l = 0; l < c.num_encoder_layers; ++l) {
      LayerDev& L = e->enc[l];
      {
        mt3k::Mx8Args g = mx(e->x_q, e->x_sc, L.wqkv_q, L.wqkv_sc, 3 * hd, emb);
        g.out = e->qkv;
        g.a_ss = e->x_ss;
        MT3_TRY(mt3k::launch_gemm_mx8(g, MT3_EPI_STORE, s));
      }
      MT3_TRY(mt3k::launch_encoder_attention(dt, e->qkv, e->attn, batch, T, c.num_heads, s));
      MT3_TRY(mt3k::launch_mx8_quantize(e->attn, false, M, hd, e->attn_q, e->attn_sc, nullptr, s));
      MT3_TRY(resid(e->attn_q, e->attn_sc, L.wo_q, L.wo_sc, hd));
      {
        mt3k::Mx8Args g = mx(e->x_q, e->x_sc, L.wi_q, L.wi_sc, 2 * c.mlp_dim, emb);
        g.ldo = c.mlp_dim;
        g.a_ss = e->x_ss;
        g.out_q = e->h_q;
        g.out_sc = e->h_sc;
        MT3_TRY(mt3k::launch_gemm_mx8(g, MT3_EPI_GEGLU, s));
      }
      MT3_TRY(resid(e->h_q, e->h_sc, L.wo_mlp_q, L.wo_mlp_sc, c.mlp_dim));
    }
    MT3_TRY(mt3k::launch_rmsnorm(dt, e->x, e->enc_norm, e->enc_out, d_encoded_f32, M, emb, s));
    MT3_TRY(mt3k::launch_mx8_quantize(e->enc_out, false, M, emb, e->enc_q, e->enc_sc, nullptr, s));
    for (int l = 0; l < c.num_decoder_layers; ++l) {
      mt3k::Mx8Args g = mx(e->enc_q, e->enc_sc, e->dec[l].wkv_x_q, e->dec[l].wkv_x_sc, 2 * hd, emb);
      g.out = e->kv_fp8 ? e->cross_stage : ckv(l);
      g.seq_len = T;
      MT3_TRY(mt3k::launch_gemm_mx8(g, MT3_EPI_HEADS, s));
      if (e->kv_fp8)
        MT3_TRY(mt3k::launch_kv_quantize_fp8(e->cross_stage, ckv(l), csc(l),
                                             batch * c.num_heads * T, s));
    }
    return MT3_OK;
  }
  const bool xs = e->x_split && !(small && !(emb <= 512 || emb == 768));
  if (xs) MT3_TRY(mt3k::launch_residual_split(e->x, e->x_ct, e->x_ss, M, emb, s));
  auto normed = [&](const void* Wt, void* out, int N, int ldo) {
    mt3k::GemmArgs g = gemm_args(xs ? static_cast<const void*>(e->x_ct) : static_cast<const void*>(e->x), Wt, out, M,
                                 N, emb, ldo);
    g.a_ss = xs ? e->x_ss : nullptr;
    return g;
  };
  auto resid = [&](const void* A, const void* Wt, int K) {
    mt3k::GemmArgs g = gemm_args(A, Wt, e->x, M, emb, K, emb);
    g.out_ct = xs ? e->x_ct : nullptr;
    g.out_ss = xs ? e->x_ss : nullptr;
    return g;
  };
  const int nrm = xs ? 2 : 1;
  for (int l = 0; l < c.num_encoder_layers; ++l) {
    LayerDev& L = e->enc[l];
    MT3_TRY(mt3k::launch_gemm(dt, normed(L.wqkv, e->qkv, 3 * hd, 3 * hd), !xs, nrm, MT3_EPI_STORE, small, s));
    MT3_TRY(mt3k::launch_encoder_attention(dt, e->qkv, e->attn, batch, T, c.num_heads, s));
    MT3_TRY(mt3k::launch_gemm(dt, resid(e->attn, L.wo, hd), false, 0, MT3_EPI_RESID, small, s));
    MT3_TRY(mt3k::launch_gemm(dt, normed(L.wi, e->hbuf, 2 * c.mlp_dim, c.mlp_dim), !xs, nrm, MT3_EPI_GEGLU, small, s));
    MT3_TRY(mt3k::launch_gemm(dt, resid(e->hbuf, L.wo_mlp, c.mlp_dim), false, 0, MT3_EPI_RESID, small, s));
  }
  MT3_TRY(mt3k::launch_rmsnorm(dt, e->x, e->enc_norm, e->enc_out, d_encoded_f32, M, emb, s));
  for (int l = 0; l < c.num_decoder_layers; ++l) {
    mt3k::GemmArgs g = gemm_args(e->enc_out, e->dec[l].wkv_x, e->kv_fp8 ? e->cross_stage : ckv(l), M,
                                 2 * hd, emb, 2 * hd);
    g.seq_len = T;
    MT3_TRY(mt3k::launch_gemm(dt, g, false, false, MT3_EPI_HEADS, small, s));
    if (e->kv_fp8)
      MT3_TRY(mt3k::launch_kv_quantize_fp8(e->cross_stage, ckv(l), csc(l),
                                           batch * c.num_heads * T, s));
  }
  return MT3_OK;
}

int mt3_engine_encode(mt3_engine* e, const float* d_inputs, int32_t batch, float* d_encoded_f32, void* stream) {
  if (!e || !e->finalized) return mt3::fail(MT3_ERR_INVALID, "mt3_engine_encode: engine not finalized");
  if (!d_inputs || batch <= 0 || batch > e->cfg.max_batch)
    return mt3::fail(MT3_ERR_INVALID, "mt3_engine_encode: batch out of range");
  if (e->pending.active)
    return mt3::fail(MT3_ERR_INVALID, "mt3_engine_encode: a decode is in flight (MT3_DECODE_ASYNC): call mt3_engine_decode_wait first");
  MT3_TRY(encode_impl(e, d_inputs, batch, d_encoded_f32, CrossDst{}, static_cast<hipStream_t>(stream)));
  e->cur_batch = batch;
  return MT3_OK;
}

static int row_groups_for(const mt3_engine_config& c, int batch, bool early_exit = false) {
  const bool f32 = c.compute_dtype != MT3_BF16;
  if (batch >= (f32 && !early_exit ? 256 : 512)) return 4;
  return batch >= 128 ? 2 : 1;
}

static int stream_row_groups_for(const mt3_engine_config& c, int slots) { return row_groups_for(c, slots); }

static void worker_main(Worker* w, int dev) {
  (void)hipSetDevice(dev);
  std::unique_lock<std::mutex> lk(w->mu);
  for (;;) {
    w->cv.wait(lk, [&] { return w->has_job || w->quit; });
    if (!w->has_job) return;
    std::function<void()> job = std::move(w->job);
    lk.unlock();
    try {
      job();
    } catch (...) {
    }
    lk.lock();
    w->has_job = false;
    w->cv.notify_all();
  }
}

static bool worker_post(mt3_engine* e, int g, std::function<void()> fn) {
  if (!e->workers[g]) {
    Worker* w = new (std::nothrow) Worker();
    if (!w) return false;
    try {
      w->th = std::thread(worker_main, w, e->device);
    } catch (...) {
      delete w;
      return false;
    }
    e->workers[g] = w;
  }
  Worker* w = e->workers[g];
  {
    std::lock_guard<std::mutex> lk(w->mu);
    w->job = std::move(fn);
    w->has_job = true;
  }
  w->cv.notify_all();
  return true;
}

static void worker_wait(mt3_engine* e, int g) {
  Worker* w = e->workers[g];
  if (!w) return;
  std::unique_lock<std::mutex> lk(w->mu);
  w->cv.wait(lk, [&] { return !w->has_job; });
}

static void workers_stop(mt3_engine* e) {
  for (int g = 0; g < kMaxGroups; ++g) {
    Worker* w = e->workers[g];
    if (!w) continue;
    {
      std::unique_lock<std::mutex> lk(w->mu);
      w->cv.wait(lk, [&] { return !w->has_job; });
      w->quit = true;
    }
    w->cv.notify_all();
    if (w->th.joinable()) w->th.join();
    delete w;
    e->workers[g] = nullptr;
  }
}

static void drop_group_graphs(mt3_engine* e) {
  for (GroupGraph& g : e->group_graphs) {
    if (g.exec) (void)hipGraphExecDestroy(g.exec);
    if (g.graph) (void)hipGraphDestroy(g.graph);
  }
  e->group_graphs.clear();
}

static hipGraphExec_t group_graph(mt3_engine* e, int variant, int batch, int row0, int rows, int slot) {
  std::lock_guard<std::mutex> lk(e->graph_mu);
  const int max_len = (variant & kVarStream) ? e->stream_max_len : 0;
  for (const GroupGraph& g : e->group_graphs)
    if (g.variant == variant && g.batch == batch && g.row0 == row0 && g.rows == rows && g.slot == slot &&
        g.max_len == max_len)
      return g.exec;
  if (!e->cap_stream[slot] && hipStreamCreateWithFlags(&e->cap_stream[slot], hipStreamNonBlocking) != hipSuccess) {
    (void)hipGetLastError();
    return nullptr;
  }
  hipStream_t cs = e->cap_stream[slot];
  if (hipStreamBeginCapture(cs, hipStreamCaptureModeThreadLocal) != hipSuccess) {
    (void)hipGetLastError();
    return nullptr;
  }
  const int rc = enqueue_chain_step(e, row0, rows, slot, batch, variant, cs, slot);
  hipGraph_t g = nullptr;
  hipGraphExec_t x = nullptr;
  const hipError_t end = hipStreamEndCapture(cs, &g);
  if (rc != MT3_OK || end != hipSuccess || hipGraphInstantiate(&x, g, nullptr, nullptr, 0) != hipSuccess) {
    if (g) (void)hipGraphDestroy(g);
    (void)hipGetLastError();
    return nullptr;
  }
  e->group_graphs.push_back(GroupGraph{variant, batch, row0, rows, slot, max_len, g, x});
  return x;
}

struct GroupRun {
  int row0, rows, batch, variant, num_steps, slot;
  bool early, use_graph;
  hipStream_t s;
  float* d_first_logits;
  float* d_step_logits;
  int ran;
  bool used_graph;
};

// ... 1063 lines not shown
```

mt3_amd/csrc/gemm.hip:

```cpp
#include <hip/hip_runtime.h>

#include <type_traits>

#include "common.h"
#include "device.h"
#include "kernels.h"

#ifndef MT3_PROF_MARK
#define MT3_PROF_MARK(i)
#endif
#ifndef MT3_PROF_DECL
#define MT3_PROF_DECL
#endif
#ifndef MT3_GLDS_PROBE
#define MT3_GLDS_PROBE 0
#endif
#ifndef MT3_GLDS_NS
#define MT3_GLDS_NS 3
#endif
#ifndef MT3_GLDS_NO_NT
#define MT3_GLDS_ST(v, p) __builtin_nontemporal_store((v), (p))
#else
#define MT3_GLDS_ST(v, p) (*(p) = (v))
#endif
#ifndef MT3_GLDS_BK
#define MT3_GLDS_BK 32
#endif
#ifndef MT3_EXP
#define MT3_EXP 0
#endif
#if MT3_EXP & 32
__device__ unsigned long long g_ph[16][8];
#undef MT3_PROF_DECL
#undef MT3_PROF_MARK
#define MT3_PROF_DECL unsigned long long ph_t0 = 0, ph_t1 = 0, ph_t2 = 0, ph_ta = 0
#define MT3_PROF_MARK(i)                                                                         \
  do {                                                                                           \
    if constexpr (BM <= 64) {                                                                    \
      if ((i) == 4) __builtin_amdgcn_s_waitcnt(0);                                               \
      if (threadIdx.x == 0) {                                                                    \
        const unsigned long long t_ = wall_clock64();                                            \
        if ((i) == 0) ph_t0 = t_;                                                                \
        else if ((i) == 1) { if (!ph_ta) ph_ta = t_; }                                           \
        else if ((i) == 2) { if (!ph_t1) ph_t1 = t_; }                                           \
        else if ((i) == 3) ph_t2 = t_;                                                           \
        else if ((i) == 4) {                                                                     \
          atomicAdd(&g_ph[EPI][0], 1ull);                                                        \
          atomicAdd(&g_ph[EPI][1], ph_t1 - ph_t0);                                               \
          atomicAdd(&g_ph[EPI][2], ph_t2 - ph_t1);                                               \
          atomicAdd(&g_ph[EPI][3], t_ - ph_t2);                                                  \
          atomicAdd(&g_ph[EPI][4], ph_ta - ph_t0);                                               \
        }                                                                                        \
      }                                                                                          \
    }                                                                                            \
  } while (0)
#endif

namespace mt3k {

template <int CPR, int NT>
__device__ __forceinline__ void tile_chunk(int tid, int p, int* row, int* chunk) {
  if constexpr ((CPR & (CPR - 1)) == 0 && NT % CPR == 0) {
    *row = tid / CPR + p * (NT / CPR);
    *chunk = tid % CPR;
  } else {
    const int c = tid + p * NT;
    *row = c / CPR;
    *chunk = c % CPR;
  }
}

template <typename CT, bool A_F32, bool NORM, int A_PASSES, int B_PASSES, int CPR, int NT>
__device__ __forceinline__ void gemm_load_tiles(u32x4 (&a_reg)[A_PASSES], u32x4 (&b_reg)[B_PASSES],
                                                float (&ss)[A_PASSES], const void* gA, const void* gW, int m0,
                                                int n0, int tid, int gM, int gLda, int gK, int k0,
                                                const void* gA2 = nullptr, int gLda2 = 0, int k1 = 0) {
  constexpr int KPL = CTraits<CT>::KPL;
  int ka = k0;
  if (gA2 != nullptr && k0 >= k1) {
    gA = gA2;
    gLda = gLda2;
    ka = k0 - k1;
  }
#pragma unroll
  for (int p = 0; p < A_PASSES; ++p) {
    int ld_row, ld_chunk;
    tile_chunk<CPR, NT>(tid, p, &ld_row, &ld_chunk);
    int row = m0 + ld_row;
    row = row < gM ? row : gM - 1;
    const size_t e = static_cast<size_t>(row) * gLda + ka + ld_chunk * KPL;
    if constexpr (A_F32) {
      const float4* src = reinterpret_cast<const float4*>(static_cast<const float*>(gA) + e);
      if constexpr (KPL == 8) {
        const float4 u = src[0], v = src[1];
        const float f[8] = {u.x, u.y, u.z, u.w, v.x, v.y, v.z, v.w};
        if constexpr (NORM) {
#pragma unroll
          for (int i = 0; i < 8; ++i) ss[p] = __builtin_fmaf(f[i], f[i], ss[p]);
        }
        a_reg[p] = pack_bf16x8(f);
      } else {
        const float4 u = src[0];
        if constexpr (NORM)
          ss[p] = __builtin_fmaf(u.w, u.w, __builtin_fmaf(u.z, u.z, __builtin_fmaf(u.y, u.y, __builtin_fmaf(u.x, u.x, ss[p]))));
        a_reg[p] = pack_f32x4(u.x, u.y, u.z, u.w);
      }
    } else {
      a_reg[p] = *reinterpret_cast<const u32x4*>(static_cast<const CT*>(gA) + e);
    }
  }
#pragma unroll
  for (int p = 0; p < B_PASSES; ++p) {
    int ld_row, ld_chunk;
    tile_chunk<CPR, NT>(tid, p, &ld_row, &ld_chunk);
    const int row = n0 + ld_row;
    const size_t e = static_cast<size_t>(row) * gK + k0 + ld_chunk * KPL;
    b_reg[p] = *reinterpret_cast<const u32x4*>(static_cast<const CT*>(gW) + e);
  }
}

struct EpiCtx {
  void* out;
  const float* aux;
  int M, N, ldo, seq;
  void* out_ct;
  float* out_ss;
  float* out2;
  int n_split, ld2;
  const float* resid_src;
};

template <typename CT, int EPI_, int FM, int FN, bool PRE, typename RowRs>
__device__ __forceinline__ void gemm_epilogue(const f32x4 (&acc)[FM][FN], int wm, int wn, int lane, int m0, int n0,
                                              const EpiCtx& c, RowRs row_rs, const float (&pre)[FM][FN][4]) {
  const int frag_row = lane & 15, frag_g = lane >> 4;
  if constexpr (EPI_ == kEpiStoreQ || EPI_ == kEpiResidQ || EPI_ == kEpiResidS) {
    if (n0 >= c.n_split) {
#pragma unroll
      for (int i = 0; i < FM; ++i)
#pragma unroll
        for (int r = 0; r < 4; ++r) {
          const int row = m0 + wm * FM * 16 + i * 16 + frag_g * 4 + r;
          if (row >= c.M) continue;
#pragma unroll
          for (int j = 0; j < FN; ++j) {
            float* o = c.out2 + static_cast<size_t>(row) * c.ld2 + (n0 - c.n_split) + wn * FN * 16 + j * 16 + frag_row;
            if constexpr (EPI_ == kEpiResidQ) *o = (PRE ? pre[i][j][r] : *o) + acc[i][j][r];
            else *o = acc[i][j][r];
          }
        }
      return;
    }
  }
  constexpr int EPI = EPI_ == kEpiStoreQ ? MT3_EPI_STORE : (EPI_ == kEpiResidQ || EPI_ == kEpiResidS) ? MT3_EPI_RESID : EPI_;
  constexpr bool PAIRED = sizeof(CT) == 2 && (EPI == MT3_EPI_STORE || EPI == MT3_EPI_GEGLU || EPI == MT3_EPI_HEADS);
  if constexpr (PAIRED) {
    const int odd = frag_row & 1;
#pragma unroll
    for (int i = 0; i < FM; ++i) {
      const int lrow0 = wm * FM * 16 + i * 16 + frag_g * 4;
#pragma unroll
      for (int j = 0; j < FN; j += (EPI == MT3_EPI_GEGLU ? 2 : 1)) {
        float mine[4], other[4];
#pragma unroll
        for (int r = 0; r < 4; ++r) {
          const float rs = row_rs(lrow0 + r);
          if constexpr (EPI == MT3_EPI_GEGLU) mine[r] = gelu_tanh_fast(acc[i][j][r] * rs) * (acc[i][j + 1][r] * rs);
          else mine[r] = acc[i][j][r] * rs;
          other[r] = lane_xor1(mine[r]);
        }
        const int col = EPI == MT3_EPI_GEGLU ? ((n0 + wn * FN * 16 + j * 16) >> 1) + frag_row
                                             : n0 + wn * FN * 16 + j * 16 + frag_row;
        const int col_even = col - odd;
#pragma unroll
        for (int h = 0; h < 2; ++h) {
          const int r = odd * 2 + h;
          const int row = m0 + lrow0 + r;
          if (row >= c.M) continue;
          const float lo = odd ? other[2 + h] : mine[h], hi = odd ? mine[2 + h] : other[h];
          const unsigned pair = pack_bf16x2(lo, hi);
          size_t dst;
          if constexpr (EPI == MT3_EPI_HEADS) {
            const int hd = c.N >> 1;
            const int kv = col_even / hd, hh = (col_even % hd) >> 6, d = col_even & 63;
            const int bb = row / c.seq, t = row % c.seq, H = hd >> 6, B = c.M / c.seq;
            dst = ((((static_cast<size_t>(kv) * B + bb) * H + hh) * c.seq) + t) * 64 + d;
          } else {
            dst = static_cast<size_t>(row) * c.ldo + col_even;
          }
          *reinterpret_cast<unsigned*>(static_cast<CT*>(c.out) + dst) = pair;
        }
      }
    }
  } else if constexpr (EPI == MT3_EPI_RESID) {
    const int odd = frag_row & 1;
#pragma unroll
    for (int i = 0; i < FM; ++i) {
      const int lrow0 = wm * FM * 16 + i * 16 + frag_g * 4;
#pragma unroll
      for (int j = 0; j < FN; ++j) {
        const int col = n0 + wn * FN * 16 + j * 16 + frag_row;
        float vnew[4], other[4], part[4];
#pragma unroll
        for (int r = 0; r < 4; ++r) {
          const int row = m0 + lrow0 + r;
          const size_t at = static_cast<size_t>(row < c.M ? row : c.M - 1) * c.ldo + col;
          vnew[r] = (PRE ? pre[i][j][r] : c.resid_src[at]) + acc[i][j][r];
          if (row < c.M) static_cast<float*>(c.out)[at] = vnew[r];
        }
        if (c.out_ss) {
#pragma unroll
          for (int r = 0; r < 4; ++r) part[r] = row16_sum(vnew[r] * vnew[r]);
#pragma unroll
          for (int r = 0; r < 4; ++r) {
            const int row = m0 + lrow0 + r;
            if (frag_row == 0 && row < c.M)
              c.out_ss[static_cast<size_t>(row) * (c.N >> 4) + ((n0 + wn * FN * 16 + j * 16) >> 4)] = part[r];
          }
        }
        if constexpr (sizeof(CT) == 2) {
          if (c.out_ct) {
#pragma unroll
            for (int r = 0; r < 4; ++r) other[r] = lane_xor1(vnew[r]);
#pragma unroll
            for (int h = 0; h < 2; ++h) {
              const int row = m0 + lrow0 + odd * 2 + h;
              if (row >= c.M) continue;
              const float lo = odd ? other[2 + h] : vnew[h], hi = odd ? vnew[2 + h] : other[h];
              *reinterpret_cast<unsigned*>(static_cast<CT*>(c.out_ct) + static_cast<size_t>(row) * c.ldo + col - odd) =
                  pack_bf16x2(lo, hi);
            }
          }
        }
      }
    }
  } else {
#pragma unroll
    for (int i = 0; i < FM; ++i) {
#pragma unroll
      for (int r = 0; r < 4; ++r) {
        const int lrow = wm * FM * 16 + i * 16 + frag_g * 4 + r;
        const int row = m0 + lrow;
        if (row >= c.M) continue;
        const float rs = row_rs(lrow);
        if constexpr (EPI == MT3_EPI_GEGLU) {
          CT* out = static_cast<CT*>(c.out);
#pragma unroll
          for (int j = 0; j < FN; j += 2) {
            const int col = n0 + wn * FN * 16 + j * 16;
            const float gate = acc[i][j][r] * rs, lin = acc[i][j + 1][r] * rs;
            out[static_cast<size_t>(row) * c.ldo + (col >> 1) + frag_row] = to_ct<CT>(gelu_tanh(gate) * lin);
          }
        } else {
#pragma unroll
          for (int j = 0; j < FN; ++j) {
            const int col = n0 + wn * FN * 16 + j * 16 + frag_row;
            const float v = acc[i][j][r] * rs;
            if constexpr (EPI == MT3_EPI_STORE) {
              static_cast<CT*>(c.out)[static_cast<size_t>(row) * c.ldo + col] = to_ct<CT>(v);
            } else if constexpr (EPI == MT3_EPI_RESID) {
              float* o = static_cast<float*>(c.out) + static_cast<size_t>(row) * c.ldo + col;
              *o = *o + v;
            } else if constexpr (EPI == MT3_EPI_POS) {
              static_cast<float*>(c.out)[static_cast<size_t>(row) * c.ldo + col] =
                  v + c.aux[static_cast<size_t>(row % c.seq) * c.N + col];
            } else if constexpr (EPI == MT3_EPI_F32) {
              static_cast<float*>(c.out)[static_cast<size_t>(row) * c.ldo + col] = v;
            } else {
              const int hd = c.N >> 1;
              const int kv = col / hd, h = (col % hd) >> 6, d = col & 63;
              const int b = row / c.seq, t = row % c.seq, H = hd >> 6, B = c.M / c.seq;
              const size_t dst = ((((static_cast<size_t>(kv) * B + b) * H + h) * c.seq) + t) * 64 + d;
              static_cast<CT*>(c.out)[dst] = to_ct<CT>(v);
            }
          }
        }
      }
    }
  }
}

template <typename CT, int BM, int BN, int BK, int WM, int WN, bool A_F32, bool NORM, int EPI, int NPV = 8>
__global__ __launch_bounds__(WM* WN * 64) void gemm_kernel(GemmArgs g) {
  constexpr int NT = WM * WN * 64;
  constexpr int KPL = CTraits<CT>::KPL;
  constexpr int KG = CTraits<CT>::KGROUP;
  constexpr int CPR = BK / KPL;
  constexpr int ROWE = BK + 2 * KPL;
  constexpr int FM = BM / (WM * 16), FN = BN / (WN * 16);
  constexpr int A_PASSES = BM * CPR / NT, B_PASSES = BN * CPR / NT;
  constexpr int ROWS_PER_PASS = NT / CPR;
  static_assert(BM * CPR % NT == 0 && BN * CPR % NT == 0, "tile/threads mismatch");
  static_assert(!NORM || (NT % CPR == 0 && (CPR & (CPR - 1)) == 0 && CPR <= 64),
                "fused norm: CPR a power of two, <= one wave, dividing NT");
  static_assert(BK % KG == 0, "BK must be a multiple of the MFMA K-group");
  static_assert(!NORM || A_F32, "NORM needs the f32 A operand");
  static_assert(EPI != MT3_EPI_GEGLU || (FN % 2 == 0), "GEGLU pairs fragments");

  __shared__ __attribute__((aligned(16))) CT As[BM * ROWE];
  __shared__ __attribute__((aligned(16))) CT Bs[BN * ROWE];
  constexpr int NP = CPR > 16 ? CPR / 16 : 1;
  __shared__ float ss_part[NORM ? BM * NP : 1];
  __shared__ float rs_x[NORM ? 1 : BM];

#if !(MT3_EXP & 64)
  asm volatile("" ::"s"(g.A), "s"(g.Wt), "s"(g.out), "s"(g.aux), "s"(g.M), "s"(g.N), "s"(g.K), "s"(g.lda), "s"(g.ldo),
               "s"(g.seq_len), "s"(g.a_ss), "s"(g.out_ct), "s"(g.out_ss), "s"(g.out2), "s"(g.n_split), "s"(g.ld2),
               "s"(g.A2), "s"(g.lda2), "s"(g.k_split), "s"(g.resid_src), "s"(g.n_major), "s"(gridDim.x));
#endif
  const void* const gA = g.A;
  const void* const gW = g.Wt;
  void* const gO = g.out;
  const float* const gAux = g.aux;
  const int gM = g.M, gN = g.N, gK = g.K, gLda = g.lda, gLdo = g.ldo, gSeq = g.seq_len;
  const float* const gAss = g.a_ss;
  void* const gOutCt = g.out_ct;
  float* const gOutSs = g.out_ss;

  MT3_PROF_DECL;
  MT3_PROF_MARK(0);
  if constexpr ((MT3_EXP & 2) == 0 && BM <= 64) __builtin_amdgcn_s_setprio(3);
  const int tid = threadIdx.x, lane = tid & 63, wave = tid >> 6;
  const int wm = wave / WN, wn = wave % WN;
  const int tiles_n = gN / BN;
  const int lid = xcd_remap(blockIdx.x, gridDim.x);
  int m0 = (lid / tiles_n) * BM, n0 = (lid % tiles_n) * BN;
  if (g.n_major) {
    const int tiles_m = gridDim.x / tiles_n;
    m0 = (lid % tiles_m) * BM;
    n0 = (lid / tiles_m) * BN;
  }

  const int ld_row = tid / CPR, ld_chunk = tid % CPR;
  float4 pv[NPV];
  const bool scale_rows = !NORM && gAss != nullptr && tid < BM;
  const int npv = gAss ? (gK >> 6) : 1;
  if constexpr (!NORM) {
    const int prow = m0 + (tid & (BM - 1)) < gM ? m0 + (tid & (BM - 1)) : gM - 1;
    const float4* p4 = gAss ? reinterpret_cast<const float4*>(gAss + static_cast<size_t>(prow) * (gK >> 4))
                            : reinterpret_cast<const float4*>(gW);
#pragma unroll
    for (int u = 0; u < NPV; ++u) pv[u] = p4[u < npv ? u : npv - 1];
  }
  constexpr bool kPre = (EPI == MT3_EPI_RESID || EPI == kEpiResidQ || EPI == kEpiResidS) && FM * FN <= 2;
  constexpr bool kSplitEpi = EPI == kEpiStoreQ || EPI == kEpiResidQ || EPI == kEpiResidS;
  const int ld2 = kSplitEpi ? (g.ld2 ? g.ld2 : gN - g.n_split) : 0;
  const bool second = kSplitEpi && n0 >= g.n_split;
  const int kend = EPI == kEpiResidS ? (second ? gK : g.k_split) : gK;
  const void* const gA2 = EPI == kEpiResidS && second ? g.A2 : nullptr;
  const int gLda2 = g.lda2, k1 = g.k_split;
  float xpre[FM][FN][4];
  const float* const gResidSrc = g.resid_src ? g.resid_src : static_cast<const float*>(gO);
  if constexpr (kPre) if (!(EPI == kEpiResidS && second)) {
    const float* src = gResidSrc;
    int ld = gLdo, c0 = n0;
    if constexpr (EPI == kEpiResidQ) {
      if (second) {
        src = g.out2;
        ld = ld2;
        c0 = n0 - g.n_split;
      }
    }
#pragma unroll
    for (int i = 0; i < FM; ++i)
#pragma unroll
      for (int j = 0; j < FN; ++j)
#pragma unroll
        for (int r = 0; r < 4; ++r) {
          const int row = m0 + wm * FM * 16 + i * 16 + (lane >> 4) * 4 + r;
          xpre[i][j][r] = src[static_cast<size_t>(row < gM ? row : gM - 1) * ld + c0 + wn * FN * 16 + j * 16 + (lane & 15)];
        }
  }
  u32x4 a_reg[A_PASSES], b_reg[B_PASSES];
  float ss[A_PASSES];
#pragma unroll
  for (int p = 0; p < A_PASSES; ++p) ss[p] = 0.f;

  f32x4 acc[FM][FN];
#pragma unroll
  for (int i = 0; i < FM; ++i)
#pragma unroll
    for (int j = 0; j < FN; ++j) acc[i][j] = f32x4{0.f, 0.f, 0.f, 0.f};

  const int frag_row = lane & 15, frag_g = lane >> 4;
  const CT* a_base = &As[(wm * FM * 16 + frag_row) * ROWE + frag_g * KPL];
  const CT* b_base = &Bs[(wn * FN * 16 + frag_row) * ROWE + frag_g * KPL];

  gemm_load_tiles<CT, A_F32, NORM, A_PASSES, B_PASSES, CPR, NT>(a_reg, b_reg, ss, gA, gW, m0, n0, tid, gM, gLda, gK, 0,
                                                                gA2, gLda2, k1);
  if constexpr (!NORM) {
    if (scale_rows) {
      float t = 0.f;
#pragma unroll
      for (int u = 0; u < NPV; ++u) {
        const float4 v = u < npv ? pv[u] : make_float4(0.f, 0.f, 0.f, 0.f);
        t = (((t + v.x) + v.y) + v.z) + v.w;
      }
      rs_x[tid] = rsqrtf(t / static_cast<float>(gK) + 1e-6f);
    }
  }
  for (int k0 = 0; k0 < kend; k0 += BK) {
    __syncthreads();
    MT3_PROF_MARK(1);
#pragma unroll
    for (int p = 0; p < A_PASSES; ++p) {
      int r, ch;
      tile_chunk<CPR, NT>(tid, p, &r, &ch);
      *reinterpret_cast<u32x4*>(&As[r * ROWE + ch * KPL]) = a_reg[p];
    }
#pragma unroll
    for (int p = 0; p < B_PASSES; ++p) {
      int r, ch;
      tile_chunk<CPR, NT>(tid, p, &r, &ch);
      *reinterpret_cast<u32x4*>(&Bs[r * ROWE + ch * KPL]) = b_reg[p];
    }
    __syncthreads();
    MT3_PROF_MARK(2);
    if (k0 + BK < kend)
      gemm_load_tiles<CT, A_F32, NORM, A_PASSES, B_PASSES, CPR, NT>(a_reg, b_reg, ss, gA, gW, m0, n0, tid, gM, gLda, gK,
                                                                    k0 + BK, gA2, gLda2, k1);
#pragma unroll
    for (int kk = 0; kk < BK / KG; ++kk) {
      u32x4 af[FM], bf[FN];
#pragma unroll
      for (int i = 0; i < FM; ++i) af[i] = *reinterpret_cast<const u32x4*>(a_base + i * 16 * ROWE + kk * KG);
#pragma unroll
      for (int j = 0; j < FN; ++j) bf[j] = *reinterpret_cast<const u32x4*>(b_base + j * 16 * ROWE + kk * KG);
#pragma unroll
      for (int i = 0; i < FM; ++i)
#pragma unroll
        for (int j = 0; j < FN; ++j) mfma_chunk<CT>(af[i], bf[j], acc[i][j]);
    }
  }
  MT3_PROF_MARK(3);

  if constexpr (NORM) {
#pragma unroll
    for (int p = 0; p < A_PASSES; ++p) {
      float v = ss[p];
      if constexpr (CPR >= 2) v += lane_xor1(v);
      if constexpr (CPR >= 4) v += __builtin_bit_cast(float, __builtin_amdgcn_update_dpp(0, __builtin_bit_cast(int, v), 0x4E, 0xF, 0xF, true));
      if constexpr (CPR >= 8) v += __builtin_bit_cast(float, __builtin_amdgcn_update_dpp(0, __builtin_bit_cast(int, v), 0x141, 0xF, 0xF, true));
      if constexpr (CPR >= 16) v += __builtin_bit_cast(float, __builtin_amdgcn_update_dpp(0, __builtin_bit_cast(int, v), 0x140, 0xF, 0xF, true));
      const bool writer = CPR >= 16 ? (ld_chunk & 15) == 0 : ld_chunk == 0;
      if (writer) ss_part[(ld_row + p * ROWS_PER_PASS) * NP + (CPR > 16 ? ld_chunk / 16 : 0)] = v;
    }
    __syncthreads();
  }
  auto row_rs = [&](int lrow) -> float {
    if constexpr (!NORM) return gAss ? rs_x[lrow] : 1.f;
    float t = ss_part[lrow * NP];
#pragma unroll
    for (int q = 1; q < NP; ++q) t += ss_part[lrow * NP + q];
    return rsqrtf(t / static_cast<float>(gK) + 1e-6f);
  };
  MT3_PROF_MARK(5);
  const EpiCtx ec{gO, gAux, gM, kSplitEpi ? g.n_split : gN, gLdo, gSeq, gOutCt, gOutSs, g.out2, g.n_split, ld2, gResidSrc};
  gemm_epilogue<CT, EPI, FM, FN, kPre>(acc, wm, wn, lane, m0, n0, ec, row_rs, xpre);
  MT3_PROF_MARK(4);
}


__device__ __forceinline__ void split3_bf16(const float (&x)[8], u32x4* h, u32x4* m, u32x4* l) {
  float hf[8], mf[8], lf[8];
#pragma unroll
  for (int i = 0; i < 8; ++i) {
    const __bf16 hi = static_cast<__bf16>(x[i]);
    const float r1 = x[i] - static_cast<float>(hi);
    const __bf16 mi = static_cast<__bf16>(r1);
    const float r2 = r1 - static_cast<float>(mi);
    hf[i] = static_cast<float>(hi);
    mf[i] = static_cast<float>(mi);
    lf[i] = r2;
  }
  *h = pack_bf16x8(hf);
  *m = pack_bf16x8(mf);
  *l = pack_bf16x8(lf);
}

template <bool NORM, int EPI, int BM_ = 128>
__global__ __launch_bounds__(256, 2) void gemm_x6_kernel(GemmArgs g, const __bf16* __restrict__ Wm,
                                                       const __bf16* __restrict__ Wl) {
  constexpr int BM = BM_, BN = 128, BK = 32, ROWE = BK + 16, FM = BM / 32, FN = 4;
  constexpr int AP = BM / 64;
  __shared__ __attribute__((aligned(16))) __bf16 As[3][BM * ROWE];
  __shared__ __attribute__((aligned(16))) __bf16 Bs[3][BN * ROWE];
  __shared__ float ss_part[NORM ? BM : 1];

  const float* const gA = static_cast<const float*>(g.A);
  const __bf16* const gW[3] = {static_cast<const __bf16*>(g.Wt), Wm, Wl};
  const int gM = g.M, gN = g.N, gK = g.K, gLda = g.lda;

  const int tid = threadIdx.x, lane = tid & 63, wave = tid >> 6;
  const int wm = wave >> 1, wn = wave & 1;
  const int tiles_n = gN / BN;
  const int lid = xcd_remap(blockIdx.x, gridDim.x);
  const int m0 = (lid / tiles_n) * BM, n0 = (lid % tiles_n) * BN;

  const int ld_chunk = (tid & 1) | ((tid >> 2) & 2);
  const int ld_row = ((tid >> 1) & 3) | ((tid >> 4) << 2);
  float4 a_st[2][AP][2];
  u32x4 w_st[2][3][2];
  typedef float f32x2 __attribute__((ext_vector_type(2)));
  f32x2 ss2[AP];
#pragma unroll
  for (int p = 0; p < AP; ++p) ss2[p] = f32x2{0.f, 0.f};
  unsigned a_offs[AP], w_offs[2];
#pragma unroll
  for (int p = 0; p < AP; ++p) {
    int row = m0 + ld_row + 64 * p;
    row = row < gM ? row : gM - 1;
    a_offs[p] = (static_cast<unsigned>(row) * static_cast<unsigned>(gLda) + ld_chunk * 8) * 4u;
  }
#pragma unroll
  for (int p = 0; p < 2; ++p) w_offs[p] = (static_cast<unsigned>(n0 + ld_row + 64 * p) * static_cast<unsigned>(gK) + ld_chunk * 8) * 2u;
  auto load = [&](int k0, auto set) {
    constexpr int S = decltype(set)::value;
    const char* const ab = reinterpret_cast<const char*>(gA) + static_cast<size_t>(k0) * 4;
#pragma unroll
    for (int p = 0; p < AP; ++p) {
      const float4* src = reinterpret_cast<const float4*>(ab + a_offs[p]);
      a_st[S][p][0] = src[0];
      a_st[S][p][1] = src[1];
    }
#pragma unroll
    for (int pl = 0; pl < 3; ++pl) {
      const char* const wb = reinterpret_cast<const char*>(gW[pl]) + static_cast<size_t>(k0) * 2;
#pragma unroll
      for (int p = 0; p < 2; ++p) w_st[S][pl][p] = *reinterpret_cast<const u32x4*>(wb + w_offs[p]);
    }
  };
  auto stage = [&](auto set) {
    constexpr int S = decltype(set)::value;
#pragma unroll
    for (int p = 0; p < AP; ++p) {
      const float f[8] = {a_st[S][p][0].x, a_st[S][p][0].y, a_st[S][p][0].z, a_st[S][p][0].w,
                          a_st[S][p][1].x, a_st[S][p][1].y, a_st[S][p][1].z, a_st[S][p][1].w};
      if constexpr (NORM) {
#pragma unroll
        for (int i = 0; i < 8; i += 2) {
          const f32x2 v = {f[i], f[i + 1]};
          ss2[p] = __builtin_elementwise_fma(v, v, ss2[p]);
        }
      }
      u32x4 h, m, l;
      split3_bf16(f, &h, &m, &l);
      const int at = (ld_row + 64 * p) * ROWE + ld_chunk * 8;
      *reinterpret_cast<u32x4*>(&As[0][at]) = h;
      *reinterpret_cast<u32x4*>(&As[1][at]) = m;
      *reinterpret_cast<u32x4*>(&As[2][at]) = l;
    }
#pragma unroll
    for (int p = 0; p < 2; ++p) {
      const int at = (ld_row + 64 * p) * ROWE + ld_chunk * 8;
#pragma unroll
      for (int pl = 0; pl < 3; ++pl) *reinterpret_cast<u32x4*>(&Bs[pl][at]) = w_st[S][pl][p];
    }
  };

  f32x4 acc[FM][FN];
#pragma unroll
  for (int i = 0; i < FM; ++i)
#pragma unroll
    for (int j = 0; j < FN; ++j) acc[i][j] = f32x4{0.f, 0.f, 0.f, 0.f};
  const int frag_row = lane & 15, frag_g = lane >> 4;
  const int a_off = (wm * (BM / 2) + frag_row) * ROWE + frag_g * 8, b_off = (wn * 64 + frag_row) * ROWE + frag_g * 8;
  auto mfma_slice = [&]() {
#pragma unroll
    for (int jh = 0; jh < FN; jh += 2) {
      u32x4 bf[3][2];
#pragma unroll
      for (int pl = 0; pl < 3; ++pl)
#pragma unroll
        for (int j = 0; j < 2; ++j) bf[pl][j] = *reinterpret_cast<const u32x4*>(&Bs[pl][b_off + (jh + j) * 16 * ROWE]);
#pragma unroll
      for (int i = 0; i < FM; ++i) {
        u32x4 af[3];
#pragma unroll
        for (int pl = 0; pl < 3; ++pl) af[pl] = *reinterpret_cast<const u32x4*>(&As[pl][a_off + i * 16 * ROWE]);
#pragma unroll
        for (int j = 0; j < 2; ++j) {
          mfma_chunk<__bf16>(af[1], bf[1][j], acc[i][jh + j]);
          mfma_chunk<__bf16>(af[0], bf[2][j], acc[i][jh + j]);
          mfma_chunk<__bf16>(af[2], bf[0][j], acc[i][jh + j]);
          mfma_chunk<__bf16>(af[0], bf[1][j], acc[i][jh + j]);
          mfma_chunk<__bf16>(af[1], bf[0][j], acc[i][jh + j]);
          mfma_chunk<__bf16>(af[0], bf[0][j], acc[i][jh + j]);
        }
      }
    }
  };
  using Set0 = std::integral_constant<int, 0>;
  using Set1 = std::integral_constant<int, 1>;

  load(0, Set0{});
  __builtin_amdgcn_sched_barrier(0);
  load(BK, Set1{});
  __builtin_amdgcn_sched_barrier(0);
  int k0 = 0;
  constexpr int kNoValuNoVmem = 0x4 | 0x8 | 0x80 | 0x100 | 0x200;
  for (; k0 + 2 * BK < gK; k0 += 2 * BK) {
    __syncthreads();
    stage(Set0{});
    __syncthreads();
    load(k0 + 2 * BK, Set0{});
    __builtin_amdgcn_sched_barrier(kNoValuNoVmem);
    mfma_slice();
    __syncthreads();
    stage(Set1{});
    __syncthreads();
    load(k0 + 3 * BK, Set1{});
    __builtin_amdgcn_sched_barrier(kNoValuNoVmem);
    mfma_slice();
  }
  __syncthreads();
  stage(Set0{});
  __syncthreads();
  mfma_slice();
  __syncthreads();
  stage(Set1{});
  __syncthreads();
  mfma_slice();
  if constexpr (NORM) {
#pragma unroll
    for (int p = 0; p < AP; ++p) {
      float v = ss2[p][0] + ss2[p][1];
      v += __builtin_bit_cast(float, __builtin_amdgcn_update_dpp(0, __builtin_bit_cast(int, v), 0xB1, 0xF, 0xF, true));
      v += __builtin_bit_cast(float, __builtin_amdgcn_update_dpp(0, __builtin_bit_cast(int, v), 0x128, 0xF, 0xF, true));
      if (ld_chunk == 0) ss_part[ld_row + 64 * p] = v;
    }
    __syncthreads();
  }
  auto row_rs = [&](int lrow) -> float {
    if constexpr (!NORM) return 1.f;
    return rsqrtf(ss_part[lrow] / static_cast<float>(gK) + 1e-6f);
  };
  const EpiCtx ec{g.out, g.aux, gM, gN, g.ldo, g.seq_len, nullptr, nullptr, nullptr, 0, 0, static_cast<const float*>(g.out)};
  const float nopre[FM][FN][4] = {};
  gemm_epilogue<float, EPI, FM, FN, false>(acc, wm, wn, lane, m0, n0, ec, row_rs, nopre);
}

int launch_gemm_x6(const GemmArgs& g, const void* Wm, const void* Wl, bool norm, int epi, hipStream_t s) {
  if (g.M <= 0 || g.N % 128 || g.K % 64 || g.K < 64 || !g.A || !g.Wt || !Wm || !Wl || !g.out)
    return mt3::fail(MT3_ERR_INVALID, "gemm_x6: bad shape or null pointer");
  if (static_cast<size_t>(g.M) * g.lda * 4 >= (1ull << 32) || static_cast<size_t>(g.N) * g.K * 2 >= (1ull << 32))
    return mt3::fail(MT3_ERR_INVALID, "gemm_x6: operand larger than 4 GB");
  if (epi == MT3_EPI_POS && (!g.aux || g.seq_len <= 0)) return mt3::fail(MT3_ERR_INVALID, "gemm_x6: POS needs aux / seq_len");
  if (epi == MT3_EPI_HEADS && (g.seq_len <= 0 || g.M % g.seq_len)) return mt3::fail(MT3_ERR_INVALID, "gemm_x6: HEADS needs M = B*T");
  const dim3 grid(((g.M + 127) / 128) * (g.N / 128)), block(256);
  const __bf16 *m = static_cast<const __bf16*>(Wm), *l = static_cast<const __bf16*>(Wl);
#define MT3_X6(NORM, EPI) hipLaunchKernelGGL((gemm_x6_kernel<NORM, EPI, 128>), grid, block, 0, s, g, m, l)
  if (norm && epi == MT3_EPI_STORE) MT3_X6(true, MT3_EPI_STORE);
  else if (norm && epi == MT3_EPI_GEGLU) MT3_X6(true, MT3_EPI_GEGLU);
  else if (!norm && epi == MT3_EPI_RESID) MT3_X6(false, MT3_EPI_RESID);
  else if (!norm && epi == MT3_EPI_POS) MT3_X6(false, MT3_EPI_POS);
  else if (!norm && epi == MT3_EPI_HEADS) MT3_X6(false, MT3_EPI_HEADS);
  else return mt3::fail(MT3_ERR_INVALID, "gemm_x6: unsupported (norm, epilogue) combination");
#undef MT3_X6
  MT3_HIP_CHECK(hipGetLastError());
  return MT3_OK;
}

template <int EPI, int NPV, int BM_ = 128>
__global__ __launch_bounds__(256) void gemm_glds_kernel(GemmArgs g) {
  using CT = __bf16;
  constexpr int BM = BM_, BN = 128, BK = MT3_GLDS_BK, FM = BM / 32, FN = 4;
  static_assert(BM == 128 || (BM == 256 && EPI != MT3_EPI_RESID && MT3_GLDS_BK == 32), "tile height");
  constexpr int ROWB = BK * 2;
  constexpr int CPROW = ROWB / 16;
  constexpr int RPP = 64 / CPROW;
  constexpr int KSH = BK == 32 ? 2 : 1;
  constexpr int STAGE_B = (BM + BN) * ROWB;
  constexpr int NS = MT3_GLDS_NS, DEPTH = NS - 1;
  constexpr int PPW = (BM + BN) / RPP / 4;
  static_assert(BK == 32 || BK == 64, "K slice");
  __shared__ __attribute__((aligned(1024))) unsigned char smem[NS * STAGE_B + BM * 4];
  float* const rs_x = reinterpret_cast<float*>(smem + NS * STAGE_B);

  const void* const gA = g.A;
  const void* const gW = g.Wt;
  const int gM = g.M, gN = g.N, gK = g.K, gLda = g.lda;
  const float* const gAss = g.a_ss;

  const int tid = threadIdx.x, lane = tid & 63, wave = tid >> 6;
  const int wm = wave >> 1, wn = wave & 1;
  const int tiles_n = gN / BN;
  const int lid = xcd_remap(blockIdx.x, gridDim.x);
  const int m0 = (lid / tiles_n) * BM, n0 = (lid % tiles_n) * BN;

  constexpr bool kMayScale = EPI != MT3_EPI_RESID;
  float4 pv[NPV];
  const bool scale_rows = kMayScale && gAss != nullptr && tid < BM;
  const int npv = gAss ? (gK >> 6) : 1;
  if constexpr (kMayScale) {
    const int prow = m0 + (tid & (BM - 1)) < gM ? m0 + (tid & (BM - 1)) : gM - 1;
    const float4* p4 = gAss ? reinterpret_cast<const float4*>(gAss + static_cast<size_t>(prow) * (gK >> 4))
                            : reinterpret_cast<const float4*>(gW);
#pragma unroll
    for (int u = 0; u < NPV; ++u) pv[u] = p4[u < npv ? u : npv - 1];
  }

  const unsigned char* src[PPW];
#pragma unroll
  for (int j = 0; j < PPW; ++j) {
    const int rr = (wave * PPW + j) * RPP + lane / CPROW;
    const bool is_a = rr < BM;
    const int r = is_a ? rr : rr - BM;
    const int chunk = (lane % CPROW) ^ ((r >> KSH) & (CPROW - 1));
    if (is_a) {
      int row = m0 + r;
      row = row < gM ? row : gM - 1;
      src[j] = static_cast<const unsigned char*>(gA) + (static_cast<size_t>(row) * gLda + chunk * 8) * 2;
    } else {
      src[j] = static_cast<const unsigned char*>(gW) + (static_cast<size_t>(n0 + r) * gK + chunk * 8) * 2;
    }
  }
  const int piece0 = wave * PPW;
  auto issue = [&](int kt, int stage) {
    const int dst0 = __builtin_amdgcn_readfirstlane(stage * STAGE_B + piece0 * 1024);
#pragma unroll
    for (int j = 0; j < PPW; ++j)
      __builtin_amdgcn_global_load_lds(
          (const __attribute__((address_space(1))) void*)(src[j] + static_cast<size_t>(kt) * ROWB),
          (__attribute__((address_space(3))) void*)(smem + dst0 + j * 1024), 16, 0, 0);
  };

  f32x4 acc[FM][FN];
#pragma unroll
  for (int i = 0; i < FM; ++i)
#pragma unroll
    for (int j = 0; j < FN; ++j) acc[i][j] = f32x4{0.f, 0.f, 0.f, 0.f};

  const int frag_row = lane & 15, frag_g = lane >> 4;
  const int key = (frag_row >> KSH) & (CPROW - 1);
  const int a_off = (wm * (BM / 2) + frag_row) * ROWB, b_off = BM * ROWB + (wn * 64 + frag_row) * ROWB;

  const int KT = gK / BK;
#pragma unroll
  for (int d = 0; d < DEPTH; ++d)
    if (d < KT) issue(d, d);
  for (int t = 0; t < KT; ++t) {
    const int ahead = KT - 1 - t < DEPTH - 1 ? KT - 1 - t : DEPTH - 1;
    if (DEPTH > 2 && ahead >= 2) {
      if constexpr (PPW == 4) asm volatile("s_waitcnt vmcnt(8)" ::: "memory");
      else if constexpr (PPW == 6) asm volatile("s_waitcnt vmcnt(12)" ::: "memory");
      else asm volatile("s_waitcnt vmcnt(16)" ::: "memory");
    } else if (DEPTH > 1 && ahead == 1) {
      if constexpr (PPW == 4) asm volatile("s_waitcnt vmcnt(4)" ::: "memory");
      else if constexpr (PPW == 6) asm volatile("s_waitcnt vmcnt(6)" ::: "memory");
      else asm volatile("s_waitcnt vmcnt(8)" ::: "memory");
    } else {
      asm volatile("s_waitcnt vmcnt(0)" ::: "memory");
    }
    __builtin_amdgcn_s_barrier();
    asm volatile("" ::: "memory");
    if (!(MT3_GLDS_PROBE & 2) && t + DEPTH < KT) issue(t + DEPTH, (t + DEPTH) % NS);
    if (MT3_GLDS_PROBE & 1) continue;
    const unsigned char* st = smem + (t % NS) * STAGE_B;
#pragma unroll
    for (int kk = 0; kk < BK / 32; ++kk) {
      const int so = ((4 * kk + frag_g) ^ key) * 16;
      u32x4 af[FM], bf[FN];
#pragma unroll
      for (int i = 0; i < FM; ++i) af[i] = *reinterpret_cast<const u32x4*>(st + a_off + i * 16 * ROWB + so);
#pragma unroll
      for (int j = 0; j < FN; ++j) bf[j] = *reinterpret_cast<const u32x4*>(st + b_off + j * 16 * ROWB + so);
#pragma unroll
      for (int i = 0; i < FM; ++i)
#pragma unroll
        for (int j = 0; j < FN; ++j) mfma_chunk<CT>(af[i], bf[j], acc[i][j]);
    }
  }
  if constexpr (kMayScale) {
    if (scale_rows) {
      float t = 0.f;
#pragma unroll
      for (int u = 0; u < NPV; ++u) {
        const float4 v = u < npv ? pv[u] : make_float4(0.f, 0.f, 0.f, 0.f);
        t = (((t + v.x) + v.y) + v.z) + v.w;
      }
      rs_x[tid] = rsqrtf(t / static_cast<float>(gK) + 1e-6f);
    }
  }
  if ((MT3_GLDS_PROBE & 4) && gM > 0) return;
  float* const tile = reinterpret_cast<float*>(smem);
  const bool has_rs = kMayScale && gAss != nullptr;
  auto tile4 = [&](int row, int col) -> float4 {
    return *reinterpret_cast<const float4*>(&tile[row * BN + (col ^ (((row >> 2) & 3) << 4))]);
  };
  f32x4 xpre[2][8];
  if constexpr (EPI == MT3_EPI_RESID) {
#pragma unroll
    for (int h = 0; h < 2; ++h)
#pragma unroll
      for (int p = 0; p < 8; ++p) {
        const int grow = m0 + h * 64 + (tid >> 5) + 8 * p;
        xpre[h][p] = *reinterpret_cast<const f32x4*>(static_cast<const float*>(g.out) +
                                                     static_cast<size_t>(grow < gM ? grow : gM - 1) * g.ldo + n0 + (tid & 31) * 4);
      }
  }
  constexpr int PW = FM / 4;
#pragma unroll 1
  for (int hw = 0; hw < 2; ++hw)
#pragma unroll
  for (int hp = 0; hp < PW; ++hp) {
    const int hm = hw * PW + hp;
    __syncthreads();
    if (wm == hw) {
#pragma unroll
      for (int i = 0; i < 4; ++i)
#pragma unroll
        for (int j = 0; j < FN; ++j)
#pragma unroll
          for (int r = 0; r < 4; ++r) {
            const int row = i * 16 + frag_g * 4 + r;
            const int col = (wn * 64 + j * 16 + frag_row) ^ (frag_g << 4);
            tile[row * BN + col] = acc[hp * 4 + i][j][r];
          }
    }
    __syncthreads();
    const int mh = m0 + hm * 64;
    if constexpr (EPI == MT3_EPI_GEGLU) {
      CT* const out = static_cast<CT*>(g.out);
      const int ldo = g.ldo, u4 = (tid & 15) * 4, q = u4 >> 4, s4 = u4 & 15;
#pragma unroll
      for (int p = 0; p < 4; ++p) {
        const int row = (tid >> 4) + 16 * p;
        if (mh + row >= gM) continue;
        const float rs = has_rs ? rs_x[hm * 64 + row] : 1.f;
        const float4 ga = tile4(row, 32 * q + s4), li = tile4(row, 32 * q + 16 + s4);
        u32x2 pk;
        pk.x = pack_bf16x2(gelu_tanh_fast(ga.x * rs) * (li.x * rs), gelu_tanh_fast(ga.y * rs) * (li.y * rs));
        pk.y = pack_bf16x2(gelu_tanh_fast(ga.z * rs) * (li.z * rs), gelu_tanh_fast(ga.w * rs) * (li.w * rs));
        MT3_GLDS_ST(pk, reinterpret_cast<u32x2*>(out + static_cast<size_t>(mh + row) * ldo + (n0 >> 1) + u4));
      }
    } else {
      const int c4 = (tid & 31) * 4;
      constexpr int kRowUnroll = EPI == MT3_EPI_RESID ? 8 : 4;
#pragma unroll kRowUnroll
      for (int p = 0; p < 8; ++p) {
        const int row = (tid >> 5) + 8 * p;
        const int grow = mh + row;
        if (grow >= gM) continue;
        const float rs = has_rs ? rs_x[hm * 64 + row] : 1.f;
        float4 v = tile4(row, c4);
        v.x *= rs, v.y *= rs, v.z *= rs, v.w *= rs;
        const int col = n0 + c4;
        if constexpr (EPI == MT3_EPI_RESID) {
          f32x4* xp = reinterpret_cast<f32x4*>(static_cast<float*>(g.out) + static_cast<size_t>(grow) * g.ldo + col);
          const f32x4 x = hw ? xpre[1][p] : xpre[0][p];
          v.x += x.x, v.y += x.y, v.z += x.z, v.w += x.w;
          *xp = f32x4{v.x, v.y, v.z, v.w};
          if (g.out_ct) {
            float t = __builtin_fmaf(v.w, v.w, __builtin_fmaf(v.z, v.z, __builtin_fmaf(v.y, v.y, v.x * v.x)));
            t = quad_sum(t);
            if ((tid & 3) == 0) g.out_ss[static_cast<size_t>(grow) * (gN >> 4) + (col >> 4)] = t;
            u32x2 pk;
            pk.x = pack_bf16x2(v.x, v.y);
            pk.y = pack_bf16x2(v.z, v.w);
            *reinterpret_cast<u32x2*>(static_cast<CT*>(g.out_ct) + static_cast<size_t>(grow) * g.ldo + col) = pk;
          }
        } else if constexpr (EPI == MT3_EPI_F32) {
          MT3_GLDS_ST((f32x4{v.x, v.y, v.z, v.w}),
                      reinterpret_cast<f32x4*>(static_cast<float*>(g.out) + static_cast<size_t>(grow) * g.ldo + col));
        } else {
          u32x2 pk;
          pk.x = pack_bf16x2(v.x, v.y);
          pk.y = pack_bf16x2(v.z, v.w);
          size_t dst;
          if constexpr (EPI == MT3_EPI_HEADS) {
            const int hd = gN >> 1, seq = g.seq_len;
            const int kv = col / hd, hh = (col % hd) >> 6, d = col & 63;
            const int bb = grow / seq, tt = grow % seq, H = hd >> 6, B = gM / seq;
            dst = ((((static_cast<size_t>(kv) * B + bb) * H + hh) * seq) + tt) * 64 + d;
          } else {
            dst = static_cast<size_t>(grow) * g.ldo + col;
          }
          MT3_GLDS_ST(pk, reinterpret_cast<u32x2*>(static_cast<CT*>(g.out) + dst));
        }
      }
    }
  }
}

template <int EPI>
static int launch_glds(const GemmArgs& g, hipStream_t s) {
  if constexpr (EPI != MT3_EPI_RESID && MT3_GLDS_BK == 32) {
    const int grid256 = ((g.M + 255) / 256) * (g.N / 128);
    if (grid256 >= 1024) {
      if (g.a_ss && g.K > 512)
        hipLaunchKernelGGL((gemm_glds_kernel<EPI, 16, 256>), dim3(grid256), dim3(256), 0, s, g);
      else
        hipLaunchKernelGGL((gemm_glds_kernel<EPI, 8, 256>), dim3(grid256), dim3(256), 0, s, g);
      MT3_HIP_CHECK(hipGetLastError());
      return MT3_OK;
    }
  }
  const int grid = ((g.M + 127) / 128) * (g.N / 128);
  if (g.a_ss && g.K > 512)
    hipLaunchKernelGGL((gemm_glds_kernel<EPI, 16>), dim3(grid), dim3(256), 0, s, g);
  else
    hipLaunchKernelGGL((gemm_glds_kernel<EPI, 8>), dim3(grid), dim3(256), 0, s, g);
  MT3_HIP_CHECK(hipGetLastError());
  return MT3_OK;
}
static bool glds_eligible(const GemmArgs& g, bool a_f32, int norm, int epi) {
  if (a_f32 || norm == 1 || g.K % 64 || g.N % 128 || g.lda % 8) return false;
  if (norm == 2 && (!g.a_ss || g.K > 1024)) return false;
  return epi == MT3_EPI_STORE || epi == MT3_EPI_RESID || epi == MT3_EPI_GEGLU || epi == MT3_EPI_HEADS ||
         epi == MT3_EPI_F32;
}

template <typename CT, int BM, int BN, int BK, int WM, int WN, bool A_F32, bool NORM, int EPI, int NPV = 8>
static int launch_cfg(const GemmArgs& g, hipStream_t s) {
  if (g.N % BN != 0 || g.K % BK != 0) return mt3::fail(MT3_ERR_INVALID, "gemm: N/K not a multiple of the tile");
  if (g.a_ss && g.K > 64 * NPV) return mt3::fail(MT3_ERR_INVALID, "gemm: K too large for this tile's partial-sum registers");
  const int grid = ((g.M + BM - 1) / BM) * (g.N / BN);
  hipLaunchKernelGGL((gemm_kernel<CT, BM, BN, BK, WM, WN, A_F32, NORM, EPI, NPV>), dim3(grid), dim3(WM * WN * 64), 0, s, g);
  MT3_HIP_CHECK(hipGetLastError());
  return MT3_OK;
}

template <typename CT, int BM, int BN, int BK, bool A_F32, bool NORM, int EPI, int NPV = 8>
static int launch_small(const GemmArgs& g, hipStream_t s) {
  return launch_cfg<CT, BM, BN, BK, 2, 2, A_F32, NORM, EPI, NPV>(g, s);
}

template <typename CT, bool A_F32, bool NORM, int EPI>
static int launch_tile(const GemmArgs& g, bool small, hipStream_t s) {
  constexpr int KG = CTraits<CT>::KGROUP;
  if (small) {
    const bool deep = g.K % (16 * KG) == 0;
    if constexpr (!NORM && !A_F32 && KG == 32 && EPI != MT3_EPI_HEADS && EPI != MT3_EPI_POS) {
      if (g.K == 24 * KG) {
        if constexpr (EPI == MT3_EPI_GEGLU) {
          if (((g.M + 31) / 32) * (g.N / 64) > 256)
            return launch_cfg<CT, 32, 64, 12 * KG, 2, 2, A_F32, NORM, EPI, 16>(g, s);
          return launch_cfg<CT, 32, 64, 24 * KG, 2, 2, A_F32, NORM, EPI, 16>(g, s);
        } else {
          if (((g.M + 31) / 32) * (g.N / 32) > 256)
            return launch_cfg<CT, 32, 32, 12 * KG, 2, 2, A_F32, NORM, EPI, 16>(g, s);
          return launch_cfg<CT, 32, 32, 24 * KG, 2, 2, A_F32, NORM, EPI, 16>(g, s);
        }
      }
    }
    if constexpr (KG == 16 && !NORM && !A_F32 &&
                  (EPI == kEpiResidS || EPI == MT3_EPI_GEGLU || EPI == kEpiResidQ || EPI == MT3_EPI_RESID)) {
      if (g.concurrent && g.M >= 256 && g.K % (8 * KG) == 0) return launch_cfg<CT, 64, 32, 8 * KG, 4, 1, A_F32, NORM, EPI>(g, s);
    }
    if constexpr (EPI == MT3_EPI_GEGLU) {
      if (deep) return launch_small<CT, 32, 64, 16 * KG, A_F32, NORM, EPI>(g, s);
      return launch_cfg<CT, 32, 64, 4 * KG, 2, 2, A_F32, NORM, EPI>(g, s);
    } else {

      if constexpr (!NORM && !A_F32 && KG == 32) {
        if (g.K == 12 * KG) return launch_cfg<CT, 32, 32, 12 * KG, 2, 2, A_F32, NORM, EPI>(g, s);
      }
      if constexpr (!NORM && !A_F32 && KG == 16) {
        if (g.K == 24 * KG) {
          const int wgs = ((g.M + 31) / 32) * (g.N / 32);
          if (wgs <= 256) return launch_cfg<CT, 32, 32, 24 * KG, 2, 2, A_F32, NORM, EPI>(g, s);
          return launch_small<CT, 32, 32, 12 * KG, A_F32, NORM, EPI>(g, s);
        }
      }
      if (deep) return launch_small<CT, 32, 32, 16 * KG, A_F32, NORM, EPI>(g, s);
      return launch_cfg<CT, 32, 32, 4 * KG, 2, 2, A_F32, NORM, EPI>(g, s);
    }
  }
  if constexpr (!NORM && !A_F32)
    if (g.a_ss && g.K > 512) return launch_cfg<CT, 128, 128, KG, 2, 2, A_F32, NORM, EPI, 16>(g, s);
  return launch_cfg<CT, 128, 128, KG, 2, 2, A_F32, NORM, EPI>(g, s);
}

template <typename CT>
static int launch_typed(const GemmArgs& g, bool a_f32, int norm, int epi, bool small, hipStream_t s) {
  if (norm == 2) {
    if (a_f32 || !g.a_ss || g.K % 64 || (small ? (g.K > 512 && g.K != 768) : g.K > 1024))
      return mt3::fail(MT3_ERR_INVALID, "gemm: norm 2 needs a compute-type A, a_ss and K = 64n <= 512 or 768 (decode-sized "
                                        "tile) / <= 1024 (encoder-sized tiles)");
    switch (epi) {
      case MT3_EPI_STORE: return launch_tile<CT, false, false, MT3_EPI_STORE>(g, small, s);
      case MT3_EPI_GEGLU: return launch_tile<CT, false, false, MT3_EPI_GEGLU>(g, small, s);
      case MT3_EPI_F32: return launch_tile<CT, false, false, MT3_EPI_F32>(g, small, s);
      case kEpiStoreQ:
        if (small) return launch_tile<CT, false, false, kEpiStoreQ>(g, small, s);
        break;
      default: break;
    }
    return mt3::fail(MT3_ERR_INVALID, "gemm: unsupported epilogue for norm 2");
  }
  if (g.a_ss) return mt3::fail(MT3_ERR_INVALID, "gemm: a_ss without norm 2");
  if (norm) {
    if (!a_f32) return mt3::fail(MT3_ERR_INVALID, "gemm: norm requires an f32 A operand");
    switch (epi) {
      case MT3_EPI_STORE: return launch_tile<CT, true, true, MT3_EPI_STORE>(g, small, s);
      case MT3_EPI_GEGLU: return launch_tile<CT, true, true, MT3_EPI_GEGLU>(g, small, s);
      case MT3_EPI_F32: return launch_tile<CT, true, true, MT3_EPI_F32>(g, small, s);
      default: break;
    }
  } else if (a_f32) {
    switch (epi) {
      case MT3_EPI_POS: return launch_tile<CT, true, false, MT3_EPI_POS>(g, small, s);
      case MT3_EPI_F32: return launch_tile<CT, true, false, MT3_EPI_F32>(g, small, s);
      case MT3_EPI_STORE: return launch_tile<CT, true, false, MT3_EPI_STORE>(g, small, s);
      default: break;
    }
  } else {
    switch (epi) {
      case MT3_EPI_RESID: return launch_tile<CT, false, false, MT3_EPI_RESID>(g, small, s);
      case kEpiResidQ:
        if (small) return launch_tile<CT, false, false, kEpiResidQ>(g, small, s);
        break;
      case kEpiResidS:
        if (small) return launch_tile<CT, false, false, kEpiResidS>(g, small, s);
        break;
      case MT3_EPI_HEADS: return launch_tile<CT, false, false, MT3_EPI_HEADS>(g, small, s);
      case MT3_EPI_STORE: return launch_tile<CT, false, false, MT3_EPI_STORE>(g, small, s);
      case MT3_EPI_F32: return launch_tile<CT, false, false, MT3_EPI_F32>(g, small, s);
      default: break;
    }
  }
  return mt3::fail(MT3_ERR_INVALID, "gemm: unsupported (a_is_f32, norm, epilogue) combination");
}

int launch_gemm(int dtype, const GemmArgs& g, bool a_f32, int norm, int epi, bool small, hipStream_t s) {
  if (g.M <= 0 || g.N <= 0 || g.K <= 0 || !g.A || !g.Wt || !g.out)
    return mt3::fail(MT3_ERR_INVALID, "gemm: bad shape or null pointer");
  if (epi == MT3_EPI_POS && (!g.aux || g.seq_len <= 0)) return mt3::fail(MT3_ERR_INVALID, "gemm: POS needs aux/seq_len");
  if ((epi == kEpiStoreQ || epi == kEpiResidQ || epi == kEpiResidS) &&
      (!g.out2 || g.n_split <= 0 || g.n_split >= g.N || g.n_split % 64))
    return mt3::fail(MT3_ERR_INVALID, "gemm: split epilogue needs out2 and 0 < n_split < N, n_split a multiple of 64");
  if (epi == kEpiResidS && (!g.A2 || g.k_split <= 0 || g.k_split >= g.K || g.k_split % 512 || (g.K - g.k_split) % 512))
    return mt3::fail(MT3_ERR_INVALID, "gemm: the two-source epilogue needs A2 and slice-aligned 0 < k_split < K");
  if (epi == MT3_EPI_HEADS && (g.seq_len <= 0 || g.M % g.seq_len != 0 || g.N % 128 != 0))
    return mt3::fail(MT3_ERR_INVALID, "gemm: HEADS needs M = B*T and N = 2*H*64");
  if (dtype == MT3_BF16 && !small && glds_eligible(g, a_f32, norm, epi)) {
    switch (epi) {
      case MT3_EPI_STORE: return launch_glds<MT3_EPI_STORE>(g, s);
      case MT3_EPI_RESID: return launch_glds<MT3_EPI_RESID>(g, s);
      case MT3_EPI_GEGLU: return launch_glds<MT3_EPI_GEGLU>(g, s);
      case MT3_EPI_HEADS: return launch_glds<MT3_EPI_HEADS>(g, s);
      default: return launch_glds<MT3_EPI_F32>(g, s);
    }
  }
  GemmArgs gg = g;
  const size_t w_bytes = static_cast<size_t>(g.N) * g.K * (dtype == MT3_BF16 ? 2 : 4);
  gg.n_major = small && w_bytes > (3u << 20) ? 1 : 0;
  if (dtype == MT3_BF16) return launch_typed<__bf16>(gg, a_f32, norm, epi, small, s);
  if (dtype == MT3_F32) return launch_typed<float>(gg, a_f32, norm, epi, small, s);
  return mt3::fail(MT3_ERR_INVALID, "gemm: unknown dtype");
}

}

extern "C" int mt3_op_gemm_ex(int32_t dtype, const void* d_A, int32_t a_is_f32, int32_t norm, const void* d_Wt,
                              void* d_out, int32_t M, int32_t N, int32_t K, int32_t epilogue, const float* d_aux,
                              int32_t seq_len, int32_t small, const float* d_a_ss, void* d_out_ct, float* d_out_ss,
                              void* stream) {
  if (norm < 0 || norm > 2) return mt3::fail(MT3_ERR_INVALID, "gemm: norm must be 0, 1 or 2");
  mt3k::GemmArgs g{};
  g.A = d_A;
  g.Wt = d_Wt;
  g.out = d_out;
  g.aux = d_aux;
  g.M = M;
  g.N = N;
  g.K = K;
  g.lda = K;
  g.ldo = epilogue == MT3_EPI_GEGLU ? N / 2 : N;
  g.seq_len = seq_len;
  g.a_ss = norm == 2 ? d_a_ss : nullptr;
  g.out_ct = d_out_ct;
  g.out_ss = d_out_ss;
  if (dtype == MT3_BF16 ? (d_out_ct != nullptr) != (d_out_ss != nullptr) : d_out_ct != nullptr)
    return mt3::fail(MT3_ERR_INVALID, "gemm: bf16: out_ct and out_ss come together; f32: out_ss alone (the rows are their "
                                      "own compute-type copy)");
  return mt3k::launch_gemm(dtype, g, a_is_f32 != 0, norm, epilogue, small != 0, static_cast<hipStream_t>(stream));
}

extern "C" int mt3_op_gemm(int32_t dtype, const void* d_A, int32_t a_is_f32, int32_t norm, const void* d_Wt,
                           void* d_out, int32_t M, int32_t N, int32_t K, int32_t epilogue, const float* d_aux,
                           int32_t seq_len, int32_t small, void* stream) {
  mt3k::GemmArgs g{};
  g.A = d_A;
  g.Wt = d_Wt;
  g.out = d_out;
  g.aux = d_aux;
  g.M = M;
  g.N = N;
  g.K = K;
  g.lda = K;
  g.ldo = epilogue == MT3_EPI_GEGLU ? N / 2 : N;
  g.seq_len = seq_len;
  return mt3k::launch_gemm(dtype, g, a_is_f32 != 0, norm != 0 ? 1 : 0, epilogue, small != 0, static_cast<hipStream_t>(stream));
}

#if MT3_EXP & 32
extern "C" int mt3_exp_gemm_phases(unsigned long long* h_out) {
  if (hipMemcpyFromSymbol(h_out, HIP_SYMBOL(g_ph), sizeof(unsigned long long) * 16 * 8) != hipSuccess) return 1;
  static const unsigned long long zeros[16 * 8] = {};
  return hipMemcpyToSymbol(HIP_SYMBOL(g_ph), zeros, sizeof(zeros)) != hipSuccess;
}
#endif
```

mt3_amd/csrc/kernels.h:

```cpp
#ifndef MT3_KERNELS_H_
#define MT3_KERNELS_H_

#include <hip/hip_runtime.h>
#include <stdint.h>

#include "mt3_hip.h"

namespace mt3k {

struct GemmArgs {
  const void* A;
  const void* Wt;
  void* out;
  const float* aux;
  int M, N, K;
  int lda, ldo;
  int seq_len;
  const float* a_ss;
  void* out_ct;
  float* out_ss;
  float* out2;
  int n_split;
  int ld2;
  const void* A2;
  int lda2;
  int k_split;
  const float* resid_src;
  int n_major;
  int concurrent;
};
constexpr int kEpiStoreQ = 6, kEpiResidQ = 7, kEpiResidS = 8;

int launch_gemm(int dtype, const GemmArgs& g, bool a_f32, int norm, int epi, bool small, hipStream_t s);

int launch_gemm_x6(const GemmArgs& g, const void* Wm, const void* Wl, bool norm, int epi, hipStream_t s);

int launch_encoder_attention(int dtype, const void* qkv, void* out, int B, int T, int H, hipStream_t s);

struct DecAttnArgs {
  const void* q;
  int q_stride;
  void* kcache;
  void* vcache;
  int cap;
  const void* new_k;
  const void* new_v;
  int kv_stride;
  const int* step;
  int n_keys;
  void* out;
  int B, H;
  float2* kv_scale;
  const float* q_f32;
  const float* q_ss;
  int q_ss_n;
  const int* done;
  const int* cache_row;
};
int launch_kv_quantize_fp8(const void* src_bf16, void* dst_fp8, void* scales, int rows, hipStream_t s);
int launch_decode_attention(int dtype, const DecAttnArgs& a, hipStream_t s);

int launch_rmsnorm(int dtype, const float* x, const float* scale, void* out_ct, float* out_f32, int rows, int dim,
                   hipStream_t s);
int launch_residual_split(const float* x, void* x_ct, float* x_ss, int rows, int dim, hipStream_t s);
struct RowProj {
  const float* ew;
  const float* pw;
  float* q_out;
  int q_n;
};
struct LogitScale {
  const float* ss;
  int n_ss;
  int dim;
};
int launch_embed(const float* table, const float* pos, const int* tok, const int* step, float* y, void* y_ct,
                 float* y_ss, int B, int dim, const RowProj& rp, hipStream_t s);
struct BeamState {
  float* f;
  int* len;
  const float* cfg;
  int rows;
  int* len_row;
};
struct StepRetire {
  int retire;
  const int* slot_row;
  const int* eos_at;
  const int* slot_seg;
  int max_len;
};
int launch_argmax_step(float* logits, int vocab, int* ids, int ids_stride, int* cur_tok, int* done,
                       int* n_done, int* step, const float* table, const float* pos_table, int max_pos,
                       float* y_next, void* y_ct, float* y_ss, int dim, int B, const BeamState* beam,
                       const int* forced, int forced_stride, const RowProj& rp, const LogitScale& ls,
                       const StepRetire& rt, hipStream_t s);
struct CompactArgs {
  int* done;
  int* slot_row;
  int* step;
  int* cur_tok;
  float* beam_f;
  int* beam_len;
  int beam_rows;
  float* y;
  void* y_ct;
  float* y_ss;
  float* qkvf;
  int emb, q_n;
  float* s_y;
  void* s_y_ct;
  float* s_y_ss;
  float* s_qkvf;
  int* s_int;
  float* s_beam;
  int* perm;
  int rows;
  int* slot_seg;
  int* s_seg;
};
int launch_compact(const CompactArgs& c, hipStream_t s);
constexpr int kRefillMaxLayers = 16;
struct RefillArgs {
  int* done;
  int* slot_row;
  int* slot_seg;
  int* step;
  int* cur_tok;
  int* n_done;
  float* beam_f;
  int* beam_len;
  int* beam_len_row;
  int beam_rows;
  float* y;
  void* y_ct;
  float* y_ss;
  int emb;
  const float* table;
  const float* pos;
  RowProj rp;
  int* ids;
  int ids_stride;
  int* out_ids;
  int* plan;
  int rows;
  int n_new;
  int first_seg;
  int n_layers;
  const char* src[kRefillMaxLayers];
  char* dst[kRefillMaxLayers];
  const char* src_sc[kRefillMaxLayers];
  char* dst_sc[kRefillMaxLayers];
  int src_batch, src_entry0, dst_batch;
  size_t row_bytes, sc_bytes;
};
int launch_refill(const RefillArgs& a, hipStream_t s);
constexpr int kBeamMaxK = 8;
constexpr float kBeamNegInf = -1.0e7f;
struct BeamKArgs {
  float* logits;
  int vocab, k, elems;
  float* live;
  float* fin_score;
  int* fin_step;
  int* fin_beam;
  int* hist_par;
  int* hist_tok;
  int hist_stride;
  int* slot_row;
  int* fork_src;
  int* fork_count;
  int* done;
  int* n_done;
  int* step;
  int* cur_tok;
  const float* bp;
  const float* table;
  const float* pos_table;
  int max_pos;
  float* y_next;
  void* y_ct;
  float* y_ss;
  int dim;
};
int launch_beam_step(const BeamKArgs& a, const RowProj& rp, const LogitScale& ls, hipStream_t s);
struct BeamReorderArgs {
  int n_layers, H, cap, kv_esize, slots;
  char* k[kRefillMaxLayers];
  char* v[kRefillMaxLayers];
  float2* scale[kRefillMaxLayers];
  const int* fork_src;
  const int* slot_row;
  const int* step;
  const int* done;
};
int launch_beam_reorder(const BeamReorderArgs& a, hipStream_t s);
int launch_beam_init(float* live, float* fin_score, int* fin_step, int* fin_beam, int slots, int k, hipStream_t s);
int launch_beam_finalize(const BeamKArgs& a, int L, int num_steps, int* ids, int* all_ids, float* scores, hipStream_t s);
int launch_iota(int* dst, int n, hipStream_t s);
int launch_set_float(float* dst, float v, hipStream_t s);
int launch_beam1_finalize(int* ids, int L, const int* beam_len, int B, hipStream_t s);
int launch_ids_to_tokens(const int* ids, int B, int L, int num_regular, int* out, hipStream_t s);

struct ScoreEmbedArgs {
  const float* table;
  const float* pos;
  const int* targets;
  const int* dec_in;
  int* tgt_pad;
  float* y;
  int rows, Lp, length, seg0, dim, vocab;
};
int launch_score_embed(const ScoreEmbedArgs& a, hipStream_t s);
struct ScoreAttnArgs {
  const void* q;
  int q_stride;
  const void* k;
  const void* v;
  int kv_stride;
  long long kv_bstride, kv_hstride;
  const int* key_tgt;
  void* out;
  int out_stride;
  int B, H, Lq, n_keys;
  int causal;
};
int launch_score_attention(int dtype, const ScoreAttnArgs& a, hipStream_t s);
struct ScoreReduceArgs {
  const float* logits;
  const int* tgt_pad;
  const float* weights;
  float* tok_pad;
  float* token_scores;
  float* seq_scores;
  int rows, Lp, length, seg0, vocab;
};
int launch_score_reduce(const ScoreReduceArgs& a, hipStream_t s);
int launch_planes(const float* w, void* hi, void* mid, void* lo, size_t n, hipStream_t s);

}
#endif
```

Baseline: 478.3 audio-s/s.

## Move next-layer QKV side product from residual-fold GEMM into GEGLU GEMM

Previously the decoder's residual/out-projection GEMM used a two-source A operand (GEGLU hidden plus residual) with a ping-pong residual buffer, so it could also emit the next layer's folded QKV/logit projection. Now that side product of the residual term goes into the wi GEGLU GEMM as extra output columns, and the wo GEMM keeps a single A source with only the MLP-fold columns. This drops the alternate y buffers, the A2/k_split loader branch and the separate resid_src pointer, which simplifies the inner load loop. In exchange the GEGLU GEMM gains padded extra columns (vocab-sized on the last layer), and the work balance between the two GEMMs shifts. A new C API entry exposes the side-output GEMM.

```diff
diff --git a/include/mt3_hip.h b/include/mt3_hip.h
--- a/include/mt3_hip.h
+++ b/include/mt3_hip.h
@@ -159,6 +159,9 @@
                    void* d_out, int32_t M, int32_t N, int32_t K, int32_t epilogue, const float* d_aux,
                    int32_t seq_len, int32_t small, const float* d_a_ss, void* d_out_ct, float* d_out_ss,
                    void* stream);
+int mt3_op_gemm_side(int32_t dtype, const void* d_A, const void* d_Wt, void* d_out, int32_t M, int32_t n_split,
+                     int32_t n_side, int32_t K, int32_t epilogue, const float* d_a_ss, void* d_out_ct, float* d_out_ss,
+                     float* d_side, int32_t concurrent, void* stream);
 int mt3_op_residual_split(int32_t dtype, const float* d_x, void* d_x_ct, float* d_x_ss, int32_t rows, int32_t dim,
                           void* stream);
 int mt3_op_encoder_attention(int32_t dtype, const void* d_qkv, void* d_out, int32_t B, int32_t T, int32_t H,
diff --git a/mt3_amd/_lib.py b/mt3_amd/_lib.py
--- a/mt3_amd/_lib.py
+++ b/mt3_amd/_lib.py
@@ -103,6 +103,8 @@
                               C.c_int32, _P, C.c_int32, C.c_int32, _P]),
     "mt3_op_gemm_ex": (C.c_int, [C.c_int32, _P, C.c_int32, C.c_int32, _P, _P, C.c_int32, C.c_int32, C.c_int32,
                                  C.c_int32, _P, C.c_int32, C.c_int32, _P, _P, _P, _P]),
+    "mt3_op_gemm_side": (C.c_int, [C.c_int32, _P, _P, _P, C.c_int32, C.c_int32, C.c_int32, C.c_int32, C.c_int32, _P, _P, _P,
+                                   _P, C.c_int32, _P]),
     "mt3_op_residual_split": (C.c_int, [C.c_int32, _P, _P, _P, C.c_int32, C.c_int32, _P]),
     "mt3_op_encoder_attention": (C.c_int, [C.c_int32, _P, _P, C.c_int32, C.c_int32, C.c_int32, _P]),
     "mt3_op_decode_attention": (C.c_int, [C.c_int32, _P, C.c_int32, _P, _P, C.c_int32, _P, _P, C.c_int32, _P,
diff --git a/mt3_amd/csrc/engine.hip b/mt3_amd/csrc/engine.hip
--- a/mt3_amd/csrc/engine.hip
+++ b/mt3_amd/csrc/engine.hip
@@ -151,8 +151,6 @@
   float* qkvf = nullptr;
   float* ew0 = nullptr;
   float* pw0 = nullptr;
-  void* y_ct_alt = nullptr;
-  float* y_alt = nullptr;
   void* qkv_d = nullptr;
   void* attn_d = nullptr;
   void* q_d = nullptr;
@@ -403,7 +401,7 @@
 mt3k::GemmArgs gemm_args(const void* A, const void* Wt, void* out, int M, int N, int K, int ldo);
 const float* scale_of(mt3_engine* e, const std::string& name);
 
-int build_qkv_fold(mt3_engine* e) {
+int build_qkv_fold(mt3_engine* e, const std::vector<std::vector<float>>& wi_host) {
   const mt3_engine_config& c = e->cfg;
   const int emb = c.emb_dim, hd = e->HD(), mlp = c.mlp_dim, n4 = 4 * hd, nl = c.num_decoder_layers;
   auto wext_t = [&](int l, std::vector<float>* t) -> int {
@@ -459,16 +457,21 @@
     prod.resize(static_cast<size_t>(nx) * mlp);
     he = hipMemcpy(prod.data(), d_prod, prod.size() * 4, hipMemcpyDeviceToHost);
     if (he != hipSuccess) break;
-    const size_t K = static_cast<size_t>(mlp) + emb;
-    w.assign((static_cast<size_t>(emb) + nx) * K, 0.f);
+    w.assign((static_cast<size_t>(emb) + nx) * mlp, 0.f);
     for (int k = 0; k < mlp; ++k)
-      for (int n = 0; n < emb; ++n) w[static_cast<size_t>(n) * K + k] = wo->data[static_cast<size_t>(k) * emb + n];
-    for (int n = 0; n < nx; ++n) {
-      float* row = w.data() + (static_cast<size_t>(emb) + n) * K;
-      std::memcpy(row, prod.data() + static_cast<size_t>(n) * mlp, static_cast<size_t>(mlp) * 4);
-      std::memcpy(row + mlp, wt.data() + static_cast<size_t>(n) * emb, static_cast<size_t>(emb) * 4);
-    }
+      for (int n = 0; n < emb; ++n) w[static_cast<size_t>(n) * mlp + k] = wo->data[static_cast<size_t>(k) * emb + n];
+    std::memcpy(w.data() + static_cast<size_t>(emb) * mlp, prod.data(), static_cast<size_t>(nx) * mlp * 4);
     rc = upload_ct(e, w, &e->dec[l].w_fold);
+    if (rc != MT3_OK) break;
+    const size_t n_wi = static_cast<size_t>(2) * mlp * emb, nx64 = (static_cast<size_t>(nx) + 63) / 64 * 64;
+    if (wi_host[l].size() != n_wi) {
+      rc = mt3::fail(MT3_ERR_INVALID, "qkv-fold: GEGLU matrix of the layer missing");
+      break;
+    }
+    w.assign(n_wi + nx64 * emb, 0.f);
+    std::memcpy(w.data(), wi_host[l].data(), n_wi * 4);
+    std::memcpy(w.data() + n_wi, wt.data(), static_cast<size_t>(nx) * emb * 4);
+    rc = upload_ct(e, w, &e->dec[l].wi);
   }
   if (he == hipSuccess && rc == MT3_OK) rc = wext_t(0, &wt);
   if (he == hipSuccess && rc == MT3_OK) {
@@ -490,7 +493,8 @@
   return MT3_OK;
 }
 
-int build_mlp(mt3_engine* e, const std::string& prefix, const float* scale, LayerDev* L, bool encoder = false) {
+int build_mlp(mt3_engine* e, const std::string& prefix, const float* scale, LayerDev* L, bool encoder = false,
+              std::vector<float>* keep_wi = nullptr) {
   const int emb = e->cfg.emb_dim, mlp = e->cfg.mlp_dim;
   const HostWeight *w0 = find(e, prefix + "/wi_0/kernel", emb, mlp), *w1 = find(e, prefix + "/wi_1/kernel", emb, mlp),
                    *wo = find(e, prefix + "/wo/kernel", mlp, emb);
@@ -507,6 +511,11 @@
   std::vector<float> ot(static_cast<size_t>(emb) * mlp);
   put_transposed(ot, mlp, 0, *wo, nullptr);
   int rc;
+  if (keep_wi) {
+    if ((rc = upload_ct(e, ot, &L->wo_mlp))) return rc;
+    keep_wi->swap(t);
+    return MT3_OK;
+  }
   if ((rc = upload_ct(e, t, &L->wi))) return rc;
   if (encoder) {
     if ((rc = upload_planes(e, t, L->wi_p))) return rc;
@@ -578,19 +587,9 @@
   const bool split = e->y_split, fold = e->qkv_fold;
   const bool retire = (skip & kVarRetire) != 0;
   const size_t crow0 = retire ? 0 : static_cast<size_t>(row0);
-  const int layer = op < 8 * nl ? (op >> 3) : nl - 1;
-  const int cur = fold ? (layer & 1) : 0;
   const bool f32 = dt == MT3_F32;
-  auto y_buf = [&](int which) -> float* {
-    return ((fold && f32 && which) ? e->y_alt : e->y) + static_cast<size_t>(row0) * emb;
-  };
-  auto yct_buf = [&](int which) -> char* {
-    if (!split) return nullptr;
-    if (f32) return reinterpret_cast<char*>(y_buf(which));
-    return static_cast<char*>((fold && which) ? e->y_ct_alt : e->y_ct) + static_cast<size_t>(row0) * emb * es;
-  };
-  float* y = y_buf(cur);
-  char* y_ct = yct_buf(cur);
+  float* y = e->y + static_cast<size_t>(row0) * emb;
+  char* y_ct = !split ? nullptr : f32 ? reinterpret_cast<char*>(y) : static_cast<char*>(e->y_ct) + static_cast<size_t>(row0) * emb * es;
   char* y_copy = split && !f32 ? y_ct : nullptr;
   float* y_ss = split ? e->y_ss + static_cast<size_t>(row0) * (emb / 16) : nullptr;
   auto normed = [&](const void* Wt, void* out, int N, int ldo) {
@@ -627,8 +626,8 @@
     b.table = e->embedding;
     b.pos_table = e->pos_table;
     b.max_pos = kMaxPos;
-    b.y_next = y_buf(0);
-    b.y_ct = split && !f32 ? yct_buf(0) : nullptr;
+    b.y_next = y;
+    b.y_ct = y_copy;
     b.y_ss = y_ss;
     b.dim = emb;
     const mt3k::RowProj rp{e->ew0, e->pw0, qkvf, 4 * hd};
@@ -661,7 +660,7 @@
                               streaming ? e->stream_max_len : 0};
     return mt3k::launch_argmax_step(logits, c.vocab_size, e->ids + crow0 * Lmax, Lmax,
                                     e->cur_tok + row0, e->done + row0, e->n_done + done_slot, step, e->embedding, e->pos_table,
-                                    kMaxPos, y_buf(0), split && !f32 ? yct_buf(0) : nullptr, y_ss, emb, rows,
+                                    kMaxPos, y, y_copy, y_ss, emb, rows,
                                     (skip & kVarBeam) ? &beam : nullptr,
                                     (skip & kVarForced) ? e->forced + static_cast<size_t>(row0) * Lmax : nullptr, Lmax, rp, ls,
                                     rt, s);
@@ -751,25 +750,27 @@
     case 6: {
       mt3k::GemmArgs g = normed(L.wi, h_d, 2 * c.mlp_dim, c.mlp_dim);
       g.concurrent = beside;
+      if (fold) {
+        const bool last = (op >> 3) + 1 == nl;
+        const int nx = last ? c.vocab_size : 4 * hd;
+        g.N = 2 * c.mlp_dim + (nx + 63) / 64 * 64;
+        g.out2 = last ? logits : qkvf;
+        g.ld2 = nx;
+        g.n_split = 2 * c.mlp_dim;
+        return mt3k::launch_gemm(dt, g, false, 2, mt3k::kEpiGegluP, small, s);
+      }
       return mt3k::launch_gemm(dt, g, !split, nrm, MT3_EPI_GEGLU, small, s);
     }
     default:
       if (fold) {
         const bool last = (op >> 3) + 1 == nl;
         const int nx = last ? c.vocab_size : 4 * hd;
-        mt3k::GemmArgs g = gemm_args(h_d, L.w_fold, y_buf(cur ^ 1), rows, emb + nx, c.mlp_dim + emb, emb);
-        g.lda = c.mlp_dim;
-        g.resid_src = y;
-        g.out_ct = f32 ? nullptr : yct_buf(cur ^ 1);
-        g.out_ss = y_ss;
+        mt3k::GemmArgs g = resid(h_d, L.w_fold, c.mlp_dim);
+        g.N = emb + nx;
         g.out2 = last ? logits : qkvf;
         g.ld2 = nx;
         g.n_split = emb;
-        g.A2 = y_ct;
-        g.lda2 = emb;
-        g.k_split = c.mlp_dim;
-        g.concurrent = beside;
-        return mt3k::launch_gemm(dt, g, false, 0, mt3k::kEpiResidS, small, s);
+        return mt3k::launch_gemm(dt, g, false, 0, mt3k::kEpiResidQ, small, s);
       }
       return mt3k::launch_gemm(dt, resid(h_d, L.wo_mlp, c.mlp_dim), false, 0, MT3_EPI_RESID, small, s);
   }
@@ -979,6 +980,9 @@
   const bool q_fold = emb % 64 == 0 && (emb <= 512 || (emb == 768 && c.compute_dtype == MT3_BF16)) && !single_stream &&
                       !(c.options & MT3_OPT_SEPARATE_PROJECTIONS);
   e->q_fold = q_fold;
+  e->qkv_fold = q_fold && !(c.options & MT3_OPT_SEPARATE_QKV_PROJECTION) && emb % 512 == 0 && c.mlp_dim % 512 == 0 &&
+                c.vocab_size % 32 == 0;
+  std::vector<std::vector<float>> dec_wi(e->qkv_fold ? c.num_decoder_layers : 0);
   for (int l = 0; l < c.num_decoder_layers; ++l) {
     const std::string P = "decoder/layers_" + std::to_string(l);
     const float* s1 = scale_of(e, P + "/pre_self_attention_layer_norm/scale");
@@ -988,7 +992,7 @@
     if ((rc = build_attention(e, P + "/self_attention", s1, false, &e->dec[l]))) return rc;
     if ((rc = build_attention(e, P + "/encoder_decoder_attention", s2, true, &e->dec[l]))) return rc;
     if (q_fold && (rc = build_q_fold(e, P, s1, s2, &e->dec[l]))) return rc;
-    if ((rc = build_mlp(e, P + "/mlp", s3, &e->dec[l]))) return rc;
+    if ((rc = build_mlp(e, P + "/mlp", s3, &e->dec[l], false, e->qkv_fold ? &dec_wi[l] : nullptr))) return rc;
     const size_t kvb = static_cast<size_t>(Bm) * c.num_heads * L * 64 * e->kv_esize;
     if ((rc = dmalloc(e, &e->dec[l].self_k, kvb))) return rc;
     if ((rc = dmalloc(e, &e->dec[l].self_v, kvb))) return rc;
@@ -1027,8 +1031,8 @@
       }
     if ((rc = upload_f32(e, pe, &e->pos_table))) return rc;
   }
-  e->qkv_fold = q_fold && !(c.options & MT3_OPT_SEPARATE_QKV_PROJECTION) && emb % 512 == 0 && c.mlp_dim % 512 == 0;
-  if (e->qkv_fold && (rc = build_qkv_fold(e))) return rc;
+  if (e->qkv_fold && (rc = build_qkv_fold(e, dec_wi))) return rc;
+  dec_wi.clear();
   const size_t M = static_cast<size_t>(Bm) * T;
   if ((rc = dmalloc(e, reinterpret_cast<void**>(&e->x), M * emb * 4))) return rc;
   e->x_split = c.compute_dtype == MT3_BF16 && emb % 64 == 0 && emb <= 1024 &&
@@ -1065,14 +1069,7 @@
   if (e->q_fold && !e->y_split) e->q_fold = false;
   if (!e->q_fold) e->qkv_fold = false;
   if (e->q_fold && (rc = dmalloc(e, reinterpret_cast<void**>(&e->qf), static_cast<size_t>(Bm) * hd * 4))) return rc;
-  if (e->qkv_fold) {
-    if ((rc = dmalloc(e, reinterpret_cast<void**>(&e->qkvf), static_cast<size_t>(Bm) * 4 * hd * 4))) return rc;
-    if (c.compute_dtype == MT3_BF16) {
-      if ((rc = dmalloc(e, &e->y_ct_alt, static_cast<size_t>(Bm) * emb * 2))) return rc;
-    } else if ((rc = dmalloc(e, reinterpret_cast<void**>(&e->y_alt), static_cast<size_t>(Bm) * emb * 4))) {
-      return rc;
-    }
-  }
+  if (e->qkv_fold && (rc = dmalloc(e, reinterpret_cast<void**>(&e->qkvf), static_cast<size_t>(Bm) * 4 * hd * 4))) return rc;
   if ((rc = dmalloc(e, &e->qkv_d, static_cast<size_t>(Bm) * 3 * hd * e->esize))) return rc;
   if ((rc = dmalloc(e, &e->attn_d, static_cast<size_t>(Bm) * hd * e->esize))) return rc;
   if ((rc = dmalloc(e, &e->q_d, static_cast<size_t>(Bm) * hd * e->esize))) return rc;
diff --git a/mt3_amd/csrc/gemm.hip b/mt3_amd/csrc/gemm.hip
--- a/mt3_amd/csrc/gemm.hip
+++ b/mt3_amd/csrc/gemm.hip
@@ -73,22 +73,15 @@
 template <typename CT, bool A_F32, bool NORM, int A_PASSES, int B_PASSES, int CPR, int NT>
 __device__ __forceinline__ void gemm_load_tiles(u32x4 (&a_reg)[A_PASSES], u32x4 (&b_reg)[B_PASSES],
                                                 float (&ss)[A_PASSES], const void* gA, const void* gW, int m0,
-                                                int n0, int tid, int gM, int gLda, int gK, int k0,
-                                                const void* gA2 = nullptr, int gLda2 = 0, int k1 = 0) {
+                                                int n0, int tid, int gM, int gLda, int gK, int k0) {
   constexpr int KPL = CTraits<CT>::KPL;
-  int ka = k0;
-  if (gA2 != nullptr && k0 >= k1) {
-    gA = gA2;
-    gLda = gLda2;
-    ka = k0 - k1;
-  }
 #pragma unroll
   for (int p = 0; p < A_PASSES; ++p) {
     int ld_row, ld_chunk;
     tile_chunk<CPR, NT>(tid, p, &ld_row, &ld_chunk);
     int row = m0 + ld_row;
     row = row < gM ? row : gM - 1;
-    const size_t e = static_cast<size_t>(row) * gLda + ka + ld_chunk * KPL;
+    const size_t e = static_cast<size_t>(row) * gLda + k0 + ld_chunk * KPL;
     if constexpr (A_F32) {
       const float4* src = reinterpret_cast<const float4*>(static_cast<const float*>(gA) + e);
       if constexpr (KPL == 8) {
@@ -127,14 +120,13 @@
   float* out_ss;
   float* out2;
   int n_split, ld2;
-  const float* resid_src;
 };
 
 template <typename CT, int EPI_, int FM, int FN, bool PRE, typename RowRs>
 __device__ __forceinline__ void gemm_epilogue(const f32x4 (&acc)[FM][FN], int wm, int wn, int lane, int m0, int n0,
                                               const EpiCtx& c, RowRs row_rs, const float (&pre)[FM][FN][4]) {
   const int frag_row = lane & 15, frag_g = lane >> 4;
-  if constexpr (EPI_ == kEpiStoreQ || EPI_ == kEpiResidQ || EPI_ == kEpiResidS) {
+  if constexpr (EPI_ == kEpiStoreQ || EPI_ == kEpiResidQ || EPI_ == kEpiGegluP) {
     if (n0 >= c.n_split) {
 #pragma unroll
       for (int i = 0; i < FM; ++i)
@@ -144,15 +136,18 @@
           if (row >= c.M) continue;
 #pragma unroll
           for (int j = 0; j < FN; ++j) {
-            float* o = c.out2 + static_cast<size_t>(row) * c.ld2 + (n0 - c.n_split) + wn * FN * 16 + j * 16 + frag_row;
+            const int col2 = (n0 - c.n_split) + wn * FN * 16 + j * 16 + frag_row;
+            float* o = c.out2 + static_cast<size_t>(row) * c.ld2 + col2;
             if constexpr (EPI_ == kEpiResidQ) *o = (PRE ? pre[i][j][r] : *o) + acc[i][j][r];
-            else *o = acc[i][j][r];
+            else if constexpr (EPI_ == kEpiGegluP) {
+              if (col2 < c.ld2) *o = acc[i][j][r];
+            } else *o = acc[i][j][r];
           }
         }
       return;
     }
   }
-  constexpr int EPI = EPI_ == kEpiStoreQ ? MT3_EPI_STORE : (EPI_ == kEpiResidQ || EPI_ == kEpiResidS) ? MT3_EPI_RESID : EPI_;
+  constexpr int EPI = EPI_ == kEpiStoreQ ? MT3_EPI_STORE : EPI_ == kEpiResidQ ? MT3_EPI_RESID : EPI_ == kEpiGegluP ? MT3_EPI_GEGLU : EPI_;
   constexpr bool PAIRED = sizeof(CT) == 2 && (EPI == MT3_EPI_STORE || EPI == MT3_EPI_GEGLU || EPI == MT3_EPI_HEADS);
   if constexpr (PAIRED) {
     const int odd = frag_row & 1;
@@ -205,7 +200,7 @@
         for (int r = 0; r < 4; ++r) {
           const int row = m0 + lrow0 + r;
           const size_t at = static_cast<size_t>(row < c.M ? row : c.M - 1) * c.ldo + col;
-          vnew[r] = (PRE ? pre[i][j][r] : c.resid_src[at]) + acc[i][j][r];
+          vnew[r] = (PRE ? pre[i][j][r] : static_cast<const float*>(c.out)[at]) + acc[i][j][r];
           if (row < c.M) static_cast<float*>(c.out)[at] = vnew[r];
         }
         if (c.out_ss) {
@@ -295,7 +290,7 @@
                 "fused norm: CPR a power of two, <= one wave, dividing NT");
   static_assert(BK % KG == 0, "BK must be a multiple of the MFMA K-group");
   static_assert(!NORM || A_F32, "NORM needs the f32 A operand");
-  static_assert(EPI != MT3_EPI_GEGLU || (FN % 2 == 0), "GEGLU pairs fragments");
+  static_assert((EPI != MT3_EPI_GEGLU && EPI != kEpiGegluP) || (FN % 2 == 0), "GEGLU pairs fragments");
 
   __shared__ __attribute__((aligned(16))) CT As[BM * ROWE];
   __shared__ __attribute__((aligned(16))) CT Bs[BN * ROWE];
@@ -306,7 +301,7 @@
 #if !(MT3_EXP & 64)
   asm volatile("" ::"s"(g.A), "s"(g.Wt), "s"(g.out), "s"(g.aux), "s"(g.M), "s"(g.N), "s"(g.K), "s"(g.lda), "s"(g.ldo),
                "s"(g.seq_len), "s"(g.a_ss), "s"(g.out_ct), "s"(g.out_ss), "s"(g.out2), "s"(g.n_split), "s"(g.ld2),
-               "s"(g.A2), "s"(g.lda2), "s"(g.k_split), "s"(g.resid_src), "s"(g.n_major), "s"(gridDim.x));
+               "s"(g.n_major), "s"(gridDim.x));
 #endif
   const void* const gA = g.A;
   const void* const gW = g.Wt;
@@ -342,17 +337,14 @@
 #pragma unroll
     for (int u = 0; u < NPV; ++u) pv[u] = p4[u < npv ? u : npv - 1];
   }
-  constexpr bool kPre = (EPI == MT3_EPI_RESID || EPI == kEpiResidQ || EPI == kEpiResidS) && FM * FN <= 2;
-  constexpr bool kSplitEpi = EPI == kEpiStoreQ || EPI == kEpiResidQ || EPI == kEpiResidS;
+  constexpr bool kPre = (EPI == MT3_EPI_RESID || EPI == kEpiResidQ) && FM * FN <= 2;
+  constexpr bool kSplitEpi = EPI == kEpiStoreQ || EPI == kEpiResidQ || EPI == kEpiGegluP;
   const int ld2 = kSplitEpi ? (g.ld2 ? g.ld2 : gN - g.n_split) : 0;
   const bool second = kSplitEpi && n0 >= g.n_split;
-  const int kend = EPI == kEpiResidS ? (second ? gK : g.k_split) : gK;
-  const void* const gA2 = EPI == kEpiResidS && second ? g.A2 : nullptr;
-  const int gLda2 = g.lda2, k1 = g.k_split;
+  const int kend = gK;
   float xpre[FM][FN][4];
-  const float* const gResidSrc = g.resid_src ? g.resid_src : static_cast<const float*>(gO);
-  if constexpr (kPre) if (!(EPI == kEpiResidS && second)) {
-    const float* src = gResidSrc;
+  if constexpr (kPre) {
+    const float* src = static_cast<const float*>(gO);
     int ld = gLdo, c0 = n0;
     if constexpr (EPI == kEpiResidQ) {
       if (second) {
@@ -386,8 +378,7 @@
   const CT* a_base = &As[(wm * FM * 16 + frag_row) * ROWE + frag_g * KPL];
   const CT* b_base = &Bs[(wn * FN * 16 + frag_row) * ROWE + frag_g * KPL];
 
-  gemm_load_tiles<CT, A_F32, NORM, A_PASSES, B_PASSES, CPR, NT>(a_reg, b_reg, ss, gA, gW, m0, n0, tid, gM, gLda, gK, 0,
-                                                                gA2, gLda2, k1);
+  gemm_load_tiles<CT, A_F32, NORM, A_PASSES, B_PASSES, CPR, NT>(a_reg, b_reg, ss, gA, gW, m0, n0, tid, gM, gLda, gK, 0);
   if constexpr (!NORM) {
     if (scale_rows) {
       float t = 0.f;
@@ -418,7 +409,7 @@
     MT3_PROF_MARK(2);
     if (k0 + BK < kend)
       gemm_load_tiles<CT, A_F32, NORM, A_PASSES, B_PASSES, CPR, NT>(a_reg, b_reg, ss, gA, gW, m0, n0, tid, gM, gLda, gK,
-                                                                    k0 + BK, gA2, gLda2, k1);
+                                                                    k0 + BK);
 #pragma unroll
     for (int kk = 0; kk < BK / KG; ++kk) {
       u32x4 af[FM], bf[FN];
@@ -455,7 +446,7 @@
     return rsqrtf(t / static_cast<float>(gK) + 1e-6f);
   };
   MT3_PROF_MARK(5);
-  const EpiCtx ec{gO, gAux, gM, kSplitEpi ? g.n_split : gN, gLdo, gSeq, gOutCt, gOutSs, g.out2, g.n_split, ld2, gResidSrc};
+  const EpiCtx ec{gO, gAux, gM, kSplitEpi ? g.n_split : gN, gLdo, gSeq, gOutCt, gOutSs, g.out2, g.n_split, ld2};
   gemm_epilogue<CT, EPI, FM, FN, kPre>(acc, wm, wn, lane, m0, n0, ec, row_rs, xpre);
   MT3_PROF_MARK(4);
 }
@@ -635,7 +626,7 @@
     if constexpr (!NORM) return 1.f;
     return rsqrtf(ss_part[lrow] / static_cast<float>(gK) + 1e-6f);
   };
-  const EpiCtx ec{g.out, g.aux, gM, gN, g.ldo, g.seq_len, nullptr, nullptr, nullptr, 0, 0, static_cast<const float*>(g.out)};
+  const EpiCtx ec{g.out, g.aux, gM, gN, g.ldo, g.seq_len, nullptr, nullptr, nullptr, 0, 0};
   const float nopre[FM][FN][4] = {};
   gemm_epilogue<float, EPI, FM, FN, false>(acc, wm, wn, lane, m0, n0, ec, row_rs, nopre);
 }
@@ -915,6 +906,7 @@
 static int launch_cfg(const GemmArgs& g, hipStream_t s) {
   if (g.N % BN != 0 || g.K % BK != 0) return mt3::fail(MT3_ERR_INVALID, "gemm: N/K not a multiple of the tile");
   if (g.a_ss && g.K > 64 * NPV) return mt3::fail(MT3_ERR_INVALID, "gemm: K too large for this tile's partial-sum registers");
+  if (g.a_ss && (g.K < 64 || g.K % 64)) return mt3::fail(MT3_ERR_INVALID, "gemm: a_ss needs K = 64n >= 64");
   const int grid = ((g.M + BM - 1) / BM) * (g.N / BN);
   hipLaunchKernelGGL((gemm_kernel<CT, BM, BN, BK, WM, WN, A_F32, NORM, EPI, NPV>), dim3(grid), dim3(WM * WN * 64), 0, s, g);
   MT3_HIP_CHECK(hipGetLastError());
@@ -929,11 +921,12 @@
 template <typename CT, bool A_F32, bool NORM, int EPI>
 static int launch_tile(const GemmArgs& g, bool small, hipStream_t s) {
   constexpr int KG = CTraits<CT>::KGROUP;
+  constexpr bool kGeglu = EPI == MT3_EPI_GEGLU || EPI == kEpiGegluP;
   if (small) {
     const bool deep = g.K % (16 * KG) == 0;
     if constexpr (!NORM && !A_F32 && KG == 32 && EPI != MT3_EPI_HEADS && EPI != MT3_EPI_POS) {
       if (g.K == 24 * KG) {
-        if constexpr (EPI == MT3_EPI_GEGLU) {
+        if constexpr (kGeglu) {
           if (((g.M + 31) / 32) * (g.N / 64) > 256)
             return launch_cfg<CT, 32, 64, 12 * KG, 2, 2, A_F32, NORM, EPI, 16>(g, s);
           return launch_cfg<CT, 32, 64, 24 * KG, 2, 2, A_F32, NORM, EPI, 16>(g, s);
@@ -945,10 +938,10 @@
       }
     }
     if constexpr (KG == 16 && !NORM && !A_F32 &&
-                  (EPI == kEpiResidS || EPI == MT3_EPI_GEGLU || EPI == kEpiResidQ || EPI == MT3_EPI_RESID)) {
+                  (kGeglu || EPI == kEpiResidQ || EPI == MT3_EPI_RESID)) {
       if (g.concurrent && g.M >= 256 && g.K % (8 * KG) == 0) return launch_cfg<CT, 64, 32, 8 * KG, 4, 1, A_F32, NORM, EPI>(g, s);
     }
-    if constexpr (EPI == MT3_EPI_GEGLU) {
+    if constexpr (kGeglu) {
       if (deep) return launch_small<CT, 32, 64, 16 * KG, A_F32, NORM, EPI>(g, s);
       return launch_cfg<CT, 32, 64, 4 * KG, 2, 2, A_F32, NORM, EPI>(g, s);
     } else {
@@ -985,6 +978,9 @@
       case kEpiStoreQ:
         if (small) return launch_tile<CT, false, false, kEpiStoreQ>(g, small, s);
         break;
+      case kEpiGegluP:
+        if (small) return launch_tile<CT, false, false, kEpiGegluP>(g, small, s);
+        break;
       default: break;
     }
     return mt3::fail(MT3_ERR_INVALID, "gemm: unsupported epilogue for norm 2");
@@ -1011,9 +1007,6 @@
       case kEpiResidQ:
         if (small) return launch_tile<CT, false, false, kEpiResidQ>(g, small, s);
         break;
-      case kEpiResidS:
-        if (small) return launch_tile<CT, false, false, kEpiResidS>(g, small, s);
-        break;
       case MT3_EPI_HEADS: return launch_tile<CT, false, false, MT3_EPI_HEADS>(g, small, s);
       case MT3_EPI_STORE: return launch_tile<CT, false, false, MT3_EPI_STORE>(g, small, s);
       case MT3_EPI_F32: return launch_tile<CT, false, false, MT3_EPI_F32>(g, small, s);
@@ -1027,11 +1020,11 @@
   if (g.M <= 0 || g.N <= 0 || g.K <= 0 || !g.A || !g.Wt || !g.out)
     return mt3::fail(MT3_ERR_INVALID, "gemm: bad shape or null pointer");
   if (epi == MT3_EPI_POS && (!g.aux || g.seq_len <= 0)) return mt3::fail(MT3_ERR_INVALID, "gemm: POS needs aux/seq_len");
-  if ((epi == kEpiStoreQ || epi == kEpiResidQ || epi == kEpiResidS) &&
+  if ((epi == kEpiStoreQ || epi == kEpiResidQ || epi == kEpiGegluP) &&
       (!g.out2 || g.n_split <= 0 || g.n_split >= g.N || g.n_split % 64))
     return mt3::fail(MT3_ERR_INVALID, "gemm: split epilogue needs out2 and 0 < n_split < N, n_split a multiple of 64");
-  if (epi == kEpiResidS && (!g.A2 || g.k_split <= 0 || g.k_split >= g.K || g.k_split % 512 || (g.K - g.k_split) % 512))
-    return mt3::fail(MT3_ERR_INVALID, "gemm: the two-source epilogue needs A2 and slice-aligned 0 < k_split < K");
+  if (epi == kEpiGegluP && (g.ld2 < 0 || g.ld2 > g.N - g.n_split || (g.N - g.n_split) % 64))
+    return mt3::fail(MT3_ERR_INVALID, "gemm: the GEGLU side product needs N - n_split = 64n >= ld2");
   if (epi == MT3_EPI_HEADS && (g.seq_len <= 0 || g.M % g.seq_len != 0 || g.N % 128 != 0))
     return mt3::fail(MT3_ERR_INVALID, "gemm: HEADS needs M = B*T and N = 2*H*64");
   if (dtype == MT3_BF16 && !small && glds_eligible(g, a_f32, norm, epi)) {
@@ -1095,6 +1088,37 @@
   return mt3k::launch_gemm(dtype, g, a_is_f32 != 0, norm != 0 ? 1 : 0, epilogue, small != 0, static_cast<hipStream_t>(stream));
 }
 
+extern "C" int mt3_op_gemm_side(int32_t dtype, const void* d_A, const void* d_Wt, void* d_out, int32_t M, int32_t n_split,
+                                int32_t n_side, int32_t K, int32_t epilogue, const float* d_a_ss, void* d_out_ct,
+                                float* d_out_ss, float* d_side, int32_t concurrent, void* stream) {
+  if (epilogue != MT3_EPI_GEGLU && epilogue != MT3_EPI_RESID)
+    return mt3::fail(MT3_ERR_INVALID, "gemm_side: epilogue must be MT3_EPI_GEGLU or MT3_EPI_RESID");
+  if (n_side <= 0) return mt3::fail(MT3_ERR_INVALID, "gemm_side: n_side must be positive");
+  const bool geglu = epilogue == MT3_EPI_GEGLU;
+  if (geglu ? (d_a_ss == nullptr || d_out_ct != nullptr || d_out_ss != nullptr)
+            : (d_a_ss != nullptr || (dtype == MT3_BF16 ? (d_out_ct != nullptr) != (d_out_ss != nullptr) : d_out_ct != nullptr)))
+    return mt3::fail(MT3_ERR_INVALID, "gemm_side: GEGLU takes a_ss and no out_ct / out_ss; RESID takes no a_ss (bf16: out_ct "
+                                      "and out_ss together, f32: out_ss alone)");
+  mt3k::GemmArgs g{};
+  g.A = d_A;
+  g.Wt = d_Wt;
+  g.out = d_out;
+  g.M = M;
+  g.N = n_split + (geglu ? (n_side + 63) / 64 * 64 : n_side);
+  g.K = K;
+  g.lda = K;
+  g.ldo = geglu ? n_split / 2 : n_split;
+  g.a_ss = d_a_ss;
+  g.out_ct = d_out_ct;
+  g.out_ss = d_out_ss;
+  g.out2 = d_side;
+  g.n_split = n_split;
+  g.ld2 = n_side;
+  g.concurrent = concurrent != 0;
+  return mt3k::launch_gemm(dtype, g, false, geglu ? 2 : 0, geglu ? mt3k::kEpiGegluP : mt3k::kEpiResidQ, true,
+                           static_cast<hipStream_t>(stream));
+}
+
 #if MT3_EXP & 32
 extern "C" int mt3_exp_gemm_phases(unsigned long long* h_out) {
   if (hipMemcpyFromSymbol(h_out, HIP_SYMBOL(g_ph), sizeof(unsigned long long) * 16 * 8) != hipSuccess) return 1;
diff --git a/mt3_amd/csrc/kernels.h b/mt3_amd/csrc/kernels.h
--- a/mt3_amd/csrc/kernels.h
+++ b/mt3_amd/csrc/kernels.h
@@ -22,14 +22,10 @@
   float* out2;
   int n_split;
   int ld2;
-  const void* A2;
-  int lda2;
-  int k_split;
-  const float* resid_src;
   int n_major;
   int concurrent;
 };
-constexpr int kEpiStoreQ = 6, kEpiResidQ = 7, kEpiResidS = 8;
+constexpr int kEpiStoreQ = 6, kEpiResidQ = 7, kEpiGegluP = 9;
 
 int launch_gemm(int dtype, const GemmArgs& g, bool a_f32, int norm, int epi, bool small, hipStream_t s);
 
```

After: 491.1 audio-s/s (median of 6 runs). +2.7%, better.
